# jinPrelude/simple-es

Measured on AMD Instinct MI355X. Metric: env-steps/sec (whole node), CartPole openai_es pop=4096 at 1/2/4/8 GPUs, higher is better.
Workload: dtype f32

## Files before the change

include/ses.h:

```cpp
#ifndef SES_H_
#define SES_H_

#include <stdint.h>

#ifdef __cplusplus
extern "C" {
#endif

#define SES_OK 0
#define SES_ERR_INVALID_ARG (-1)
#define SES_ERR_UNSUPPORTED (-2)
#define SES_ERR_HIP (-3)
#define SES_ERR_NO_DEVICE (-4)
#define SES_ERR_COMM (-5)

#define SES_HIDDEN 32

#define SES_ENV_NONE (-1)
#define SES_ENV_CARTPOLE 0
#define SES_ENV_LUNARLANDER 1
#define SES_ENV_SIMPLE_SPREAD 2
#define SES_ENV_BIPEDALWALKER 3
#define SES_ENV_ACROBOT 4
#define SES_ENV_MOUNTAINCAR 5
#define SES_ENV_PENDULUM 6
#define SES_ENV_MOUNTAINCAR_CONT 7

#define SES_MODE_EPISODIC 0
#define SES_MODE_FIXED_LENGTH 1

typedef struct ses_handle ses_handle;

typedef struct ses_config {
    int32_t env_id;
    int32_t num_state;
    int32_t num_action;
    int32_t discrete_action;
    int32_t gru;
    int32_t pomdp;
    int32_t max_step;
    int32_t eval_ep_num;
    int32_t device;
    int32_t lanes_per_env;
    int32_t n_agents;
    int32_t physics64;
} ses_config;

int ses_create(const ses_config *cfg, void *stream, ses_handle **out);
int ses_destroy(ses_handle *h);
int ses_sync(ses_handle *h);
int ses_set_tuning(ses_handle *h, const char *name, int32_t value);
int ses_launch_counts(ses_handle *h, int64_t *pair_rollouts, int64_t *perturb_rollouts, int64_t *apply_perturb);
int ses_set_stamp(ses_handle *h, uint64_t *dst);
const char *ses_last_error(void);
const char *ses_version(void);
int ses_param_count(int32_t num_state, int32_t num_action, int32_t gru);
int ses_device_count(void);

int ses_perturb(ses_handle *h, const float *parents, const int32_t *parent_idx, const int32_t *row_ids,
                float sigma, uint64_t seed, uint64_t gen, int64_t first_row, int32_t n_rows, float *theta);
int ses_noise(ses_handle *h, uint64_t seed, uint64_t gen, int64_t first_row, int32_t n_rows, float *eps);
int ses_perturb_host_noise(ses_handle *h, const float *parents, const int32_t *parent_idx,
                           const double *eps64, double sigma, int32_t n_rows, float *theta,
                           float *eps_store);
int ses_init_states_uniform(ses_handle *h, uint64_t seed, uint64_t gen, int64_t first_row, int32_t n_rows,
                            int32_t shared, int32_t width, float lo, float hi, float *out);
int ses_init_states_uniform_gens(ses_handle *h, uint64_t seed, uint64_t gen0, int32_t gens, int64_t first_row,
                                 int32_t n_rows, int32_t shared, int32_t width, float lo, float hi, float *out);

int ses_policy_forward(ses_handle *h, const float *theta, const float *obs, float *hidden, int32_t n,
                       float *logits, float *act, int32_t *action);

int ses_env_step(ses_handle *h, int32_t n, int32_t mode, float *x, float *xd, float *th, float *thd,
                 const int32_t *action, float *ret, uint32_t *status);

int ses_env_state_bytes(ses_handle *h);
int ses_env_obs_width(ses_handle *h);
int ses_env_reset(ses_handle *h, const float *init, int32_t n, void *state, float *obs);
int ses_env_step_generic(ses_handle *h, void *state, const void *action, int32_t n, float *obs, float *reward,
                         int32_t *done);

int ses_env_step_shape(ses_handle *h, int32_t *block, int32_t *lds_bytes, int32_t *waves_per_cu, int32_t *lds_per_cu);

int ses_stream_probe(ses_handle *h, int32_t n, float *x, float *xd, float *th, float *thd, const int32_t *action,
                     float *ret, uint32_t *status);

int ses_rollout(ses_handle *h, const float *theta, const float *init, int32_t init_per_offspring,
                int32_t n_rows, int32_t mode, float *fitness, double *ep_return, int32_t *ep_steps);

int ses_rank_center(ses_handle *h, const float *fitness, int32_t n, int32_t *rank, double *weights, float *best);

int ses_openai_generation(ses_handle *h, const float *fitness, int32_t n, uint64_t seed, uint64_t gen, double lr,
                          double sigma, double adam_a, const float *mu_in, const float *m_in, const float *v_in,
                          float *mu_out, float *m_out, float *v_out, float next_sigma, uint64_t next_gen,
                          int64_t first_row, int32_t n_rows, float *theta_next, float *best);
int ses_openai_sharded_ok(ses_handle *h, ses_handle *comm, int32_t n, int32_t per_rank, int32_t world);
int ses_openai_generation_sharded(ses_handle *h, ses_handle *comm, const float *fitness, int32_t n, uint64_t seed, uint64_t gen,
                                  double lr, double sigma, double adam_a, const float *mu_in, const float *m_in,
                                  const float *v_in, float *mu_out, float *m_out, float *v_out, float next_sigma,
                                  uint64_t next_gen, int64_t first_row, int32_t n_rows, int32_t per_rank, int32_t world,
                                  float *theta_next, float *best);
int ses_es_update_philox(ses_handle *h, const double *weights, int32_t n, int32_t skip_row0, uint64_t seed,
                         uint64_t gen, double lr, double sigma, double adam_a, float *mu, float *m, float *v,
                         float *grad_out);
int ses_es_update_stored(ses_handle *h, const double *weights, int32_t n, const float *eps_store, double lr,
                         double sigma, double adam_a, float *mu, float *m, float *v, float *grad_out);

int ses_perturb_mirrored(ses_handle *h, const float *mu, const float *scale, float sigma, uint64_t seed, uint64_t gen,
                         int64_t first_row, int32_t n_rows, float *theta);
int ses_pgpe_generation(ses_handle *h, const float *fitness, int32_t n, uint64_t seed, uint64_t gen, double sigma, double adam_a,
                        double sigma_learning_rate, double sigma_max_change, float scale_lo, float scale_hi, const float *mu_in,
                        const float *m_in, const float *v_in, const float *scale_in, float *mu_out, float *m_out, float *v_out,
                        float *scale_out, float next_sigma, uint64_t next_gen, int64_t first_row, int32_t n_rows,
                        float *theta_next, float *best, float *gmu_out, float *gs_out);

typedef struct ses_sepcma_params {
    int32_t mu, reserved;
    double mueff, c_sigma, d_sigma, c_c, c_1, c_mu, chi;
    float scale_lo, scale_hi, step_lo, step_hi;
} ses_sepcma_params;
int ses_perturb_sepcma(ses_handle *h, const float *mu, const float *C, const float *step, float sigma, uint64_t seed, uint64_t gen,
                       int64_t first_row, int32_t n_rows, float *theta);
int ses_sepcma_generation(ses_handle *h, const float *fitness, int32_t n, uint64_t seed, uint64_t gen, double sigma, double hsig_scale,
                          const ses_sepcma_params *p, const float *weights, const float *mu_in, const float *C_in,
                          const float *ps_in, const float *pc_in, const float *step_in, float *mu_out, float *C_out, float *ps_out,
                          float *pc_out, float *step_out, float next_sigma, uint64_t next_gen, int64_t first_row, int32_t n_rows,
                          float *theta_next, float *best, float *sz_out, float *szz_out, double *norm2_out);

#define SES_LMMA_MAX_MEMORY 32
#define SES_LMMA_MAX_P 16384
typedef struct ses_lmma_params {
    int32_t mu, m;
    double mueff, c_sigma, d_sigma, chi;
    float step_lo, step_hi;
    float cd[SES_LMMA_MAX_MEMORY], ad[SES_LMMA_MAX_MEMORY], ac[SES_LMMA_MAX_MEMORY], bc[SES_LMMA_MAX_MEMORY];
} ses_lmma_params;
int ses_perturb_lmma(ses_handle *h, const float *mu, const float *M, const float *step, const ses_lmma_params *p, int32_t m_active,
                     float sigma, uint64_t seed, uint64_t gen, int64_t first_row, int32_t n_rows, float *theta, float *dots_out);
int ses_lmma_generation(ses_handle *h, const float *fitness, int32_t n, uint64_t seed, uint64_t gen, double sigma,
                        const ses_lmma_params *p, const float *weights, int32_t m_active, int32_t m_active_next, const float *mu_in,
                        const float *ps_in, const float *M_in, const float *step_in, float *mu_out, float *ps_out, float *M_out,
                        float *step_out, float next_sigma, uint64_t next_gen, int64_t first_row, int32_t n_rows, float *theta_next,
                        float *best, float *sz_out, float *sd_out, float *sdots_out, double *norm2_out, float *dots_next_out);

int ses_elite_ids(ses_handle *h, const int32_t *rank, int32_t n, int32_t k, int32_t *elite_ids);
int ses_elite_select(ses_handle *h, const int32_t *rank, int32_t n, int32_t k, const int32_t *parent_map,
                     int32_t *alias_state, int32_t *elite_ids, int32_t *elite_parent_idx, int32_t *alias_first);
int ses_elite_mean(ses_handle *h, const float *rows, const int32_t *alias_first, int32_t k, float *mean);
int ses_gather_rows(ses_handle *h, const float *src, const int32_t *ids, int32_t n_ids, float *dst);

#define SES_STRATEGY_OPENAI_ES 0
#define SES_STRATEGY_SIMPLE_EVOLUTION 1
#define SES_STRATEGY_SIMPLE_GENETIC 2
#define SES_STRATEGY_PGPE 3
#define SES_STRATEGY_SEP_CMA_ES 4
#define SES_STRATEGY_LM_MA_ES 5
typedef struct ses_gen_state {
    int32_t strategy, n, elite_num, mode, shared_init, init_width;
    float init_lo, init_hi;
    uint64_t seed, env_seed;
    double learning_rate, sigma_decay;
    double sigma, pop_sigma;
    uint64_t pop_gen;
    int64_t adam_t;
    int32_t cur, world;
    float *theta[2];
    float *parents[2];
    float *adam_m[2];
    float *adam_v[2];
    int32_t *parent_map;
    int32_t *alias_state;
    float *fitness;
    float *init;
    int32_t *work_i32;
    float *work_f32;
    int64_t first_row;
    int32_t n_local, per_rank;
    ses_handle *comm;
    float *fit_local;
    float *scale[2];
    double sigma_learning_rate, sigma_max_change;
    float scale_lo, scale_hi;
    float *cma_C[2];
    float *cma_ps[2];
    float *cma_pc[2];
    float *cma_step[2];
    const float *cma_weights;
    ses_sepcma_params cma;
    float *lm_ps[2];
    float *lm_M[2];
    float *lm_step[2];
    const float *lm_weights;
    ses_lmma_params lm;
} ses_gen_state;
int ses_run_generations(ses_handle *h, ses_gen_state *st, int32_t k, float *best, uint64_t *stamps);

#define SES_COMM_ID_BYTES 128
int ses_comm_unique_id(void *id);
int ses_comm_init(ses_handle *h, int32_t rank, int32_t world, const void *id);
int ses_comm_info(ses_handle *h, int32_t *rank, int32_t *world, int32_t *rccl_version);
int ses_comm_destroy(ses_handle *h);
int ses_allgather_fitness(ses_handle *h, const float *local, int32_t n_per_rank, float *all);
#define SES_COMM_P2P_HANDLE_BYTES 64
int ses_comm_p2p_export(ses_handle *h, int32_t rank, int32_t world, int32_t max_per_rank, void *handle);
int ses_comm_p2p_attach(ses_handle *h, const void *handles);
int ses_comm_p2p_attach_local(ses_handle *h, ses_handle *const *peers);
int ses_stream_create_exclusive(int32_t device, void **stream);
int ses_stream_destroy(void *stream);
int ses_comm_p2p_info(ses_handle *h, int32_t *world, int32_t *max_per_rank, int32_t *exchanges);
int ses_comm_p2p_counts(ses_handle *h, int32_t *flag_exchanges, int32_t *granule_exchanges);
int ses_comm_p2p_status(ses_handle *h, uint32_t *timed_out_mask);
int ses_comm_p2p_reset_status(ses_handle *h);
int ses_comm_p2p_detach(ses_handle *h);

#ifdef __cplusplus
}
#endif
#endif
```

simple-es_amd/csrc/ses_core.hip:

```cpp
#include <cstring>
#include <string>

#include "ses_internal.h"

namespace ses {

static thread_local char g_err[512] = "";

int set_error(int code, const char *fmt, ...)
{
    va_list ap;
    va_start(ap, fmt);
    vsnprintf(g_err, sizeof g_err, fmt, ap);
    va_end(ap);
    return code;
}

int ensure_episode_scratch(ses_handle *h, size_t episodes)
{
    if (episodes <= h->ep_cap) return SES_OK;
    if (h->ep_return || h->ep_steps) SES_HIP_TRY(hipStreamSynchronize(h->stream));
    if (h->ep_return) SES_HIP_TRY(hipFree(h->ep_return));
    if (h->ep_steps) SES_HIP_TRY(hipFree(h->ep_steps));
    h->ep_return = nullptr;
    h->ep_steps = nullptr;
    h->ep_cap = 0;
    SES_HIP_TRY(hipMalloc(&h->ep_return, episodes * sizeof(double)));
    SES_HIP_TRY(hipMalloc(&h->ep_steps, episodes * sizeof(int32_t)));
    h->ep_cap = episodes;
    return SES_OK;
}

int ensure_reduce_scratch(ses_handle *h, size_t bytes)
{
    if (bytes <= h->red_cap) return SES_OK;
    size_t want = bytes < (1u << 20) ? (1u << 20) : bytes * 2;
    if (h->red_scratch) {
        SES_HIP_TRY(hipStreamSynchronize(h->stream));
        SES_HIP_TRY(hipFree(h->red_scratch));
    }
    h->red_scratch = nullptr;
    h->red_cap = 0;
    h->rank_zeroed = nullptr;
    h->counter_armed = nullptr;
    SES_HIP_TRY(hipMalloc(&h->red_scratch, want));
    h->red_cap = want;
    return SES_OK;
}

}

extern "C" {

const char *ses_last_error(void) { return ses::g_err; }

const char *ses_version(void) { return "ses-hip 0.1 (gfx950)"; }

int ses_param_count(int32_t S, int32_t A, int32_t gru)
{
    int p = SES_HIDDEN * S + SES_HIDDEN + A * SES_HIDDEN + A;
    if (gru) p += 2 * (3 * SES_HIDDEN * SES_HIDDEN) + 2 * (3 * SES_HIDDEN);
    return p;
}

int ses_device_count(void)
{
    int n = 0;
    hipError_t e = hipGetDeviceCount(&n);
    if (e != hipSuccess) return ses::set_error(SES_ERR_NO_DEVICE, "hipGetDeviceCount: %s", hipGetErrorString(e));
    return n;
}

int ses_create(const ses_config *cfg, void *stream, ses_handle **out)
{
    SES_REQUIRE(cfg && out, "ses_create: null argument");
    SES_REQUIRE(cfg->env_id == SES_ENV_CARTPOLE || cfg->env_id == SES_ENV_NONE || cfg->env_id == SES_ENV_SIMPLE_SPREAD ||
                    cfg->env_id == SES_ENV_LUNARLANDER || cfg->env_id == SES_ENV_BIPEDALWALKER || ses::is_classic_env(cfg->env_id),
                "ses_create: unknown env_id %d", cfg->env_id);
    SES_REQUIRE(cfg->num_state >= 1 && cfg->num_state <= 32, "ses_create: num_state %d out of range", cfg->num_state);
    SES_REQUIRE(cfg->num_action >= 1 && cfg->num_action <= 8, "ses_create: num_action %d out of range", cfg->num_action);
    SES_REQUIRE(cfg->eval_ep_num >= 1, "ses_create: eval_ep_num must be >= 1");
    SES_REQUIRE(cfg->max_step >= 1 && cfg->max_step < (1 << 30), "ses_create: max_step must be in [1, 2^30)");
    SES_REQUIRE(cfg->lanes_per_env == 0 || cfg->lanes_per_env == 1 || cfg->lanes_per_env == 2 ||
                    cfg->lanes_per_env == 4 || cfg->lanes_per_env == 8 || cfg->lanes_per_env == 16 || cfg->lanes_per_env == 32,
                "ses_create: lanes_per_env must be 0, 1, 2, 4, 8, 16 or 32");
    if (cfg->env_id == SES_ENV_CARTPOLE)
        SES_REQUIRE(cfg->num_state == 4 && cfg->num_action == 2 && cfg->discrete_action,
                    "ses_create: CartPole needs num_state=4 num_action=2 discrete_action=1");
    if (cfg->env_id == SES_ENV_LUNARLANDER)
        SES_REQUIRE(cfg->num_state == 8 && cfg->num_action == 4,
                    "ses_create: LunarLander needs num_state=8 num_action=4 (discrete_action=0: LunarLanderContinuous-v2, 1: LunarLander-v2)");
    if (cfg->env_id == SES_ENV_BIPEDALWALKER)
        SES_REQUIRE(cfg->num_state == 24 && cfg->num_action == 4 && !cfg->discrete_action && !cfg->gru && !cfg->pomdp,
                    "ses_create: BipedalWalker needs num_state=24 num_action=4 discrete_action=0 gru=0 pomdp=0");
    if (cfg->env_id == SES_ENV_SIMPLE_SPREAD)
        SES_REQUIRE((cfg->n_agents == 2 || cfg->n_agents == 3) && cfg->num_state == 6 * cfg->n_agents &&
                        cfg->num_action == 5 && cfg->discrete_action && (cfg->gru == 0 || cfg->gru == 1),
                    "ses_create: simple_spread needs n_agents in {2,3}, num_state=6*n_agents, num_action=5, "
                    "discrete_action=1, gru in {0,1}");
    static const struct {
        int env_id;
        const char *name;
        int S, A, discrete;
    } classic[] = {{SES_ENV_ACROBOT, "Acrobot-v1", 6, 3, 1}, {SES_ENV_MOUNTAINCAR, "MountainCar-v0", 2, 3, 1},
                   {SES_ENV_PENDULUM, "Pendulum-v1", 3, 1, 0}, {SES_ENV_MOUNTAINCAR_CONT, "MountainCarContinuous-v0", 2, 1, 0}};
    for (const auto &e : classic)
        if (cfg->env_id == e.env_id)
            SES_REQUIRE(cfg->num_state == e.S && cfg->num_action == e.A && (cfg->discrete_action != 0) == e.discrete &&
                            (cfg->gru == 0 || cfg->gru == 1) && !cfg->pomdp && !cfg->physics64,
                        "ses_create: %s needs num_state=%d num_action=%d discrete_action=%d gru in {0,1} pomdp=0 physics64=0 "
                        "(its physics is float64 regardless)",
                        e.name, e.S, e.A, e.discrete);
    SES_REQUIRE(cfg->physics64 == 0 || (cfg->physics64 == 1 && cfg->env_id == SES_ENV_CARTPOLE),
                "ses_create: physics64 is a CartPole rollout option");
    int ndev = ses_device_count();
    if (ndev <= 0) return ses::set_error(SES_ERR_NO_DEVICE, "ses_create: no HIP device visible");
    SES_REQUIRE(cfg->device >= 0 && cfg->device < ndev, "ses_create: device %d not in [0,%d)", cfg->device, ndev);
    SES_HIP_TRY(hipSetDevice(cfg->device));
    ses_handle *h = new ses_handle();
    std::memset(h, 0, sizeof *h);
    h->cfg = *cfg;
    h->stream = (hipStream_t)stream;
    h->P = ses_param_count(cfg->num_state, cfg->num_action, cfg->gru);
    h->obs_mask = 0u;
    if (cfg->pomdp && cfg->env_id == SES_ENV_CARTPOLE) h->obs_mask = 0xAu;
    if (cfg->pomdp && cfg->env_id == SES_ENV_LUNARLANDER) h->obs_mask = 0x2Cu;
    h->tune_rollout_block = 64;
    h->tune_gru_mfma_min_e = 12;
    h->tune_gru_mfma4_min_e = 7;
    h->tune_gru_ep_parallel_max = 4096;
    h->tune_gru_sequential = 0;
    h->tune_rollout_mix = 1;
    h->tune_rollout_waves8 = 1024;
    h->tune_rollout_packed = -1;
    h->tune_rollout_heavy_packed = -1;
    h->tune_rollout_mix_8_16 = 1;
    h->tune_rollout_handover_step = 1 << 30;
    h->tune_rollout_heavy_prio_steps = 1 << 30;
    h->tune_lander_per_wave = 0;
    h->tune_box2d_lpe = 0;
    h->tune_box2d_epw = 0;
    h->tune_env_step_block = 64;
    h->tune_env_step_lds = -1;
    h->tune_env_step_waves = 7;
    h->env_step_key[0] = -2;
    {
        int lds = 0;
        const hipError_t e = hipDeviceGetAttribute(&lds, hipDeviceAttributeMaxSharedMemoryPerMultiprocessor, cfg->device);
        if (e != hipSuccess) {
            delete h;
            return ses::set_error(SES_ERR_HIP, "ses_create: hipDeviceGetAttribute: %s", hipGetErrorString(e));
        }
        h->lds_per_cu = lds;
    }
    h->tune_openai_sharded_tail = 1;
    h->tune_openai_sharded_min_rows = 8192;
    h->tune_openai_granules = 1;
    h->tune_comm_granules_enabled = 1;
    h->tune_fused_fitness = 1;
    h->tune_fused_mean = 1;
    h->tune_fused_elite = 1;
    h->tune_fused_apply_perturb = 1;
    h->tune_fused_perturb_rollout = 1;
    h->tune_pgpe_fused_apply_perturb = 1;
    h->tune_spread_gru_wave_per_batch = -1;
    h->tune_comm_granules = 0;
    h->tune_es_final_max_chunks = 0;
    h->tune_es_tail_wide = 1;
    *out = h;
    return SES_OK;
}

int ses_set_tuning(ses_handle *h, const char *name, int32_t value)
{
    SES_REQUIRE(h && name, "ses_set_tuning: null argument");
    struct Knob {
        const char *name;
        int ses_handle::*field;
        int lo, hi;
    };
    static const Knob knobs[] = {{"rollout_block", &ses_handle::tune_rollout_block, 64, 256},
                                 {"gru_mfma_min_e", &ses_handle::tune_gru_mfma_min_e, 1, 1 << 30},
                                 {"gru_mfma4_min_e", &ses_handle::tune_gru_mfma4_min_e, 0, 8},
                                 {"gru_ep_parallel_max", &ses_handle::tune_gru_ep_parallel_max, 0, 1 << 30},
                                 {"gru_sequential", &ses_handle::tune_gru_sequential, 0, 1},
                                 {"rollout_mix", &ses_handle::tune_rollout_mix, 0, 1},
                                 {"rollout_waves8", &ses_handle::tune_rollout_waves8, 1, 1 << 20},
                                 {"rollout_mix_light", &ses_handle::tune_rollout_mix_light, 0, 16},
                                 {"rollout_lpe32_max_envs", &ses_handle::tune_rollout_lpe32_max, 0, 1 << 30},
                                 {"rollout_packed", &ses_handle::tune_rollout_packed, -1, 1},
                                 {"rollout_heavy_packed", &ses_handle::tune_rollout_heavy_packed, -1, 1},
                                 {"rollout_mix_8_16", &ses_handle::tune_rollout_mix_8_16, 0, 1},
                                 {"rollout_handover_step", &ses_handle::tune_rollout_handover_step, 0, 1 << 30},
                                 {"rollout_heavy_prio_steps", &ses_handle::tune_rollout_heavy_prio_steps, 0, 1 << 30},
                                 {"lander_offspring_per_wave", &ses_handle::tune_lander_per_wave, 0, 4},
                                 {"box2d_lanes_per_env", &ses_handle::tune_box2d_lpe, 0, 64},
                                 {"box2d_envs_per_wave", &ses_handle::tune_box2d_epw, 0, 64},
                                 {"pendulum_generic_step", &ses_handle::tune_pendulum_generic, 0, 1},
                                 {"env_step_block", &ses_handle::tune_env_step_block, 64, 256},
                                 {"env_step_lds_bytes", &ses_handle::tune_env_step_lds, -1, 65536},
                                 {"env_step_waves_per_cu", &ses_handle::tune_env_step_waves, 1, 32},
                                 {"es_final_max_chunks", &ses_handle::tune_es_final_max_chunks, 0, 1 << 20},
                                 {"es_tail_wide", &ses_handle::tune_es_tail_wide, 0, 1},
                                 {"comm_force_rccl", &ses_handle::tune_comm_force_rccl, 0, 1},
                                 {"comm_p2p_timeout_ms", &ses_handle::tune_comm_p2p_timeout_ms, 0, 1 << 30},
                                 {"comm_p2p_keep_going", &ses_handle::tune_comm_p2p_keep_going, 0, 1},
                                 {"openai_sharded_tail", &ses_handle::tune_openai_sharded_tail, 0, 1},
                                 {"openai_sharded_min_rows", &ses_handle::tune_openai_sharded_min_rows, 0, 1 << 30},
                                 {"openai_granule_exchange", &ses_handle::tune_openai_granules, 0, 1},
                                 {"comm_granule_allgather", &ses_handle::tune_comm_granules, 0, 1},
                                 {"comm_granules_enabled", &ses_handle::tune_comm_granules_enabled, 0, 1},
                                 {"fused_fitness_exchange", &ses_handle::tune_fused_fitness, 0, 1},
                                 {"fused_episode_mean", &ses_handle::tune_fused_mean, 0, 1},
                                 {"fused_elite_tail", &ses_handle::tune_fused_elite, 0, 1},
                                 {"fused_apply_perturb", &ses_handle::tune_fused_apply_perturb, 0, 1},
                                 {"fused_perturb_rollout", &ses_handle::tune_fused_perturb_rollout, 0, 1},
                                 {"pgpe_fused_apply_perturb", &ses_handle::tune_pgpe_fused_apply_perturb, 0, 1},
                                 {"spread_gru_wave_per_batch", &ses_handle::tune_spread_gru_wave_per_batch, -1, 1}};
    for (const Knob &k : knobs) {
        if (std::strcmp(k.name, name) == 0) {
            SES_REQUIRE(value >= k.lo && value <= k.hi, "ses_set_tuning: %s = %d outside [%d, %d]", name, value, k.lo, k.hi);
            SES_REQUIRE(k.field != &ses_handle::tune_rollout_block || value == 64 || value == 256,
                        "ses_set_tuning: rollout_block must be 64 or 256");
            SES_REQUIRE(k.field != &ses_handle::tune_env_step_block || value == 64 || value == 128 || value == 256,
                        "ses_set_tuning: env_step_block must be 64, 128 or 256");
            SES_REQUIRE(k.field != &ses_handle::tune_lander_per_wave || value != 3,
                        "ses_set_tuning: lander_offspring_per_wave must be 0, 1, 2 or 4");
            SES_REQUIRE(k.field != &ses_handle::tune_box2d_lpe || (value & (value - 1)) == 0,
                        "ses_set_tuning: box2d_lanes_per_env must be 0 or a power of two up to 64");
            SES_REQUIRE(k.field != &ses_handle::tune_rollout_mix_light || value == 0 || value == 8 || value == 16,
                        "ses_set_tuning: rollout_mix_light must be 0, 8 or 16");
            h->*(k.field) = value;
            if (k.field == &ses_handle::tune_comm_p2p_timeout_ms) ses::comm_p2p_set_timeout(h);
            return SES_OK;
        }
    }
    return ses::set_error(SES_ERR_INVALID_ARG, "ses_set_tuning: unknown knob '%s'", name);
}

int ses_launch_counts(ses_handle *h, int64_t *pair_rollouts, int64_t *perturb_rollouts, int64_t *apply_perturb)
{
    SES_REQUIRE(h, "ses_launch_counts: null handle");
    if (pair_rollouts) *pair_rollouts = h->count_pair_rollouts;
    if (perturb_rollouts) *perturb_rollouts = h->count_perturb_rollouts;
    if (apply_perturb) *apply_perturb = h->count_apply_perturb;
    return SES_OK;
}

int ses_set_stamp(ses_handle *h, uint64_t *dst)
{
    SES_REQUIRE(h, "ses_set_stamp: null handle");
    h->stamp = (unsigned long long *)dst;
    return SES_OK;
}

int ses_destroy(ses_handle *h)
{
    if (!h) return SES_OK;
    (void)hipSetDevice(h->cfg.device);
    (void)ses::comm_release(h);
    if (h->ep_return) (void)hipFree(h->ep_return);
    if (h->ep_steps) (void)hipFree(h->ep_steps);
    if (h->red_scratch) (void)hipFree(h->red_scratch);
    if (h->gen_init) (void)hipFree(h->gen_init);
    delete h;
    return SES_OK;
}

int ses_sync(ses_handle *h)
{
    SES_REQUIRE(h, "ses_sync: null handle");
    SES_HIP_TRY(hipStreamSynchronize(h->stream));
    return SES_OK;
}

}
```

simple-es_amd/csrc/ses_internal.h:

```cpp
#pragma once
#include <hip/hip_runtime.h>

#include <cstdarg>
#include <cstdio>
#include <type_traits>

#include "../../include/ses.h"

namespace ses {
struct P2pGranuleView;
struct PerturbUpdate {
    const float *partial;
    int chunks, P4;
    float update_factor;
    double adam_a;
    const float *mu_in, *m_in, *v_in;
    float *mu_out, *m_out, *v_out;
    float sigma;
    uint64_t seed, gen;
    long long first_row;
    int n_rows, P, quads;
    float *theta;
    unsigned long long *stamp;
    int32_t *rank_to_clear;
    int n_clear;
};
}
struct ses_handle {
    ses_config cfg;
    hipStream_t stream;
    int P;
    uint32_t obs_mask;
    double *ep_return;
    int32_t *ep_steps;
    size_t ep_cap;
    void *red_scratch;
    size_t red_cap;
    float *gen_init;
    size_t gen_init_cap;
    void *comm;
    int comm_rank, comm_world;
    struct ses_p2p *p2p;
    int tune_rollout_block;
    int tune_gru_mfma_min_e;
    int tune_gru_mfma4_min_e;
    int tune_gru_ep_parallel_max;
    int tune_gru_sequential;
    int tune_rollout_mix;
    int tune_rollout_waves8;
    int tune_rollout_mix_light;
    int tune_rollout_lpe32_max;
    int tune_rollout_mix_8_16;
    int tune_rollout_handover_step;
    int tune_rollout_heavy_prio_steps;
    int tune_rollout_packed;
    int tune_rollout_heavy_packed;
    unsigned long long *stamp;
    int32_t *rank_zeroed;
    int rank_zeroed_n;
    unsigned int *counter_armed;
    int tune_comm_force_rccl;
    int tune_es_final_max_chunks;
    int tune_es_tail_wide;
    int tune_box2d_lpe;
    int tune_env_step_block;
    int tune_env_step_lds;
    int tune_env_step_waves;
    const ses::P2pGranuleView *fit_gv;
    const float *fit_own;
    int fit_per_rank;
    int skip_mean;
    const double *mean_src;
    unsigned long long *mean_stamp;
    int tune_fused_elite;
    int tune_fused_apply_perturb;
    int tune_fused_mean;
    int lds_per_cu;
    int env_step_key[3];
    int env_step_lds_resolved;
    int env_step_wpc;
    int tune_box2d_epw;
    int tune_lander_per_wave;
    int tune_comm_p2p_timeout_ms;
    int tune_comm_p2p_keep_going;
    int tune_fused_fitness;
    int tune_comm_granules_enabled;
    int tune_comm_granules;
    int tune_openai_granules;
    int tune_openai_sharded_tail;
    int tune_openai_sharded_min_rows;
    int tune_fused_perturb_rollout;
    int defer_perturb, defer_mode;
    int perturb_pending;
    ses::PerturbUpdate pending;
    long long count_pair_rollouts;
    long long count_perturb_rollouts;
    long long count_apply_perturb;
    int tune_pendulum_generic;
    int tune_pgpe_fused_apply_perturb;
    int tune_spread_gru_wave_per_batch;
};

namespace ses {

__device__ __forceinline__ unsigned long long real_time() { return wall_clock64(); }

int set_error(int code, const char *fmt, ...);

#define SES_HIP_TRY(expr)                                                                          \
    do {                                                                                           \
        hipError_t e_ = (expr);                                                                    \
        if (e_ != hipSuccess)                                                                      \
            return ::ses::set_error(SES_ERR_HIP, "%s failed: %s (%s:%d)", #expr, hipGetErrorString(e_), \
                                    __FILE__, __LINE__);                                           \
    } while (0)

#define SES_REQUIRE(cond, ...)                                             \
    do {                                                                   \
        if (!(cond)) return ::ses::set_error(SES_ERR_INVALID_ARG, __VA_ARGS__); \
    } while (0)

inline int ceil_div(long long a, long long b) { return (int)((a + b - 1) / b); }

template <int L>
using lanes_c = std::integral_constant<int, L>;

template <class F>
inline void with_fixed_length(int mode, F &&f)
{
    if (mode == SES_MODE_FIXED_LENGTH) f(std::true_type{});
    else f(std::false_type{});
}

template <int... Ls, class F>
inline bool with_lanes(int lanes, F &&f)
{
    return (... || (lanes == Ls && (f(lanes_c<Ls>{}), true)));
}

template <int S_, int A_>
struct PolicyShape {
    static constexpr int S = S_, A = A_;
};
template <class... Shapes, class F>
inline bool with_policy_shape(int S, int A, F &&f)
{
    return (... || (S == Shapes::S && A == Shapes::A && (f(Shapes{}), true)));
}

struct RolloutArgs {
    const float *theta, *init;
    int per;
    int n_rows, E, P, max_step;
    uint32_t obs_mask;
    double *epr;
    int32_t *ep_steps;
    long long episodes() const { return (long long)n_rows * E; }
};

template <class K, class... X>
inline void launch_rollout_kernel(const ses_handle *h, K kernel, dim3 grid, dim3 block, const RolloutArgs &a, X... extra)
{
    hipLaunchKernelGGL(kernel, grid, block, 0, h->stream, a.theta, a.init, a.per, a.n_rows, a.E, a.P, a.max_step, a.obs_mask,
                       extra..., a.epr, a.ep_steps);
}

constexpr int P2P_GRANULE_MAX_WORLD = 16;
struct P2pGranuleView {
    unsigned long long *dst[P2P_GRANULE_MAX_WORLD];
    const unsigned long long *src;
    int section;
    int rank, world;
    uint32_t seq;
    unsigned long long timeout_ticks;
    uint32_t *err, *err_seen;
};
int comm_p2p_granules_begin(ses_handle *comm, int granules, P2pGranuleView *view);

#if defined(__HIPCC__)
__device__ __forceinline__ void granule_store(unsigned long long *dst, uint32_t seq, uint32_t value_bits)
{
    __hip_atomic_store(dst, ((unsigned long long)value_bits << 32) | (unsigned long long)seq, __ATOMIC_RELAXED, __HIP_MEMORY_SCOPE_SYSTEM);
}

__device__ __forceinline__ uint32_t granule_wait(const unsigned long long *src, const P2pGranuleView &v, int from)
{
    const unsigned long long t0 = real_time();
    unsigned long long limit = v.timeout_ticks;
    bool known_late = false;
    for (;;) {
        const unsigned long long g = __hip_atomic_load(src, __ATOMIC_RELAXED, __HIP_MEMORY_SCOPE_SYSTEM);
        const uint32_t tag = (uint32_t)g;
        if (tag == v.seq) return (uint32_t)(g >> 32);
        if (!known_late) {
            known_late = true;
            const uint32_t seen = __hip_atomic_load(v.err_seen, __ATOMIC_RELAXED, __HIP_MEMORY_SCOPE_AGENT);
            if (((seen >> (from & 31)) & 1u) && limit > 200000ull) limit = 200000ull;
        }
        if ((int32_t)(tag - v.seq) > 0 || real_time() - t0 > limit) {
            atomicOr_system(v.err, 1u << (from & 31));
            atomicOr(v.err_seen, 1u << (from & 31));
            return 0x7FC00000u;
        }
        __builtin_amdgcn_s_sleep(2);
    }
}

#endif

int openai_fused_fitness_ok(const ses_handle *h, int32_t n, int32_t per_rank, int32_t n_ranked);
int elite_tail_small(ses_handle *h, const double *ep_return, int32_t n, int32_t k, const int32_t *parent_map, int32_t *alias_state,
                     int32_t *rank, float *fitness, float *best, int32_t *ids, int32_t *pidx, int32_t *alias,
                     unsigned long long *stamp, const float *parents, float sigma, uint64_t seed, uint64_t gen, float *mean_out);

inline bool is_classic_env(int env_id)
{
    return env_id == SES_ENV_ACROBOT || env_id == SES_ENV_MOUNTAINCAR || env_id == SES_ENV_PENDULUM || env_id == SES_ENV_MOUNTAINCAR_CONT;
}
int classic_env_state_bytes(const ses_handle *h);
int classic_env_obs_width(const ses_handle *h);
int classic_env_reset(ses_handle *h, const float *init, int n, void *state, float *obs);
int classic_env_step(ses_handle *h, void *state, const void *action, int n, float *obs, float *reward, int32_t *done);
int classic_lanes_per_env(const ses_handle *h, long long episodes);
int classic_rollout(const ses_handle *h, const RolloutArgs &a, int mode);
inline bool is_classic_policy_shape(int S, int A) { return (A == 3 && (S == 6 || S == 2)) || (A == 1 && (S == 3 || S == 2)); }
int classic_policy_forward(ses_handle *h, const float *theta, const float *obs, float *hidden, int n, float *logits, float *act,
                           int32_t *action);

int spread_gru_rollout(const ses_handle *h, const RolloutArgs &a);
inline bool is_spread_policy_shape(int S, int A) { return A == 5 && (S == 12 || S == 18); }
int spread_gru_policy_forward(ses_handle *h, const float *theta, const float *obs, float *hidden, int n, float *logits, float *act,
                              int32_t *action);

enum class GruForm { Sequential, EpisodeParallel, Mfma4, Mfma, LockstepMulti4, LockstepMulti2, Lockstep };

int lander_discrete_rollout(const ses_handle *h, const RolloutArgs &a, GruForm form, int lpe, int epw);
int lander_discrete_env_step(ses_handle *h, void *state, const int32_t *action, int n, float *obs, float *reward, int32_t *done);

bool cartpole_perturb_rollout_ok(const ses_handle *h, int n_rows, int mode);
int flush_pending_perturb(ses_handle *h);

int ensure_episode_scratch(ses_handle *h, size_t episodes);
int ensure_reduce_scratch(ses_handle *h, size_t bytes);
int comm_release(ses_handle *h);
void comm_p2p_set_timeout(ses_handle *h);


}
```

simple-es_amd/csrc/ses_perturb_prologue.h:

```cpp
#pragma once
#include "ses_internal.h"
#include "ses_rng.h"

namespace ses {

__device__ __forceinline__ void adam_apply(float g, double adam_a, float &mu, float &m, float &v)
{
    const float b1 = 0.99f, b2 = 0.999f;
    const float omb1 = (float)(1.0 - 0.99), omb2 = (float)(1.0 - 0.999);
    const float mn = (b1 * m) + (omb1 * g);
    const float vn = (b2 * v) + (omb2 * (g * g));
    const double num = (-adam_a) * (double)mn;
    const float den = __builtin_sqrtf(vn) + 1e-08f;
    const double step = num / (double)den;
    m = mn;
    v = vn;
    mu = (float)((double)mu + step);
}

constexpr int UPDATE_PRELOAD = 4;
struct UpdateOperands {
    float part[UPDATE_PRELOAD];
    float mu, m, v;
};
__device__ __forceinline__ UpdateOperands es_update_load(const PerturbUpdate &u, int p)
{
    UpdateOperands o;
#pragma unroll
    for (int c = 0; c < UPDATE_PRELOAD; ++c) o.part[c] = c < u.chunks ? u.partial[(size_t)c * u.P4 + p] : 0.0f;
    o.mu = u.mu_in[p]; o.m = u.m_in[p]; o.v = u.v_in[p];
    return o;
}
__device__ __forceinline__ void es_update_finish(const PerturbUpdate &u, int p, UpdateOperands &o)
{
    float sum = o.part[0];
#pragma unroll
    for (int c = 1; c < UPDATE_PRELOAD; ++c)
        if (c < u.chunks) sum = sum + o.part[c];
    for (int c = UPDATE_PRELOAD; c < u.chunks; ++c) sum = sum + u.partial[(size_t)c * u.P4 + p];
    const float g = sum * u.update_factor;
    adam_apply(g, u.adam_a, o.mu, o.m, o.v);
}

__device__ __forceinline__ void perturb_update_mean(const PerturbUpdate &u, float *mu_new, UpdateOperands *first = nullptr)
{
    const int block = (int)blockDim.x;
    const long long t = (long long)blockIdx.x * block + threadIdx.x;
    if (u.stamp && t == 0) *u.stamp = real_time();
    for (int p = threadIdx.x; p < u.P; p += block) {
        UpdateOperands o = (first && p == (int)threadIdx.x) ? *first : es_update_load(u, p);
        es_update_finish(u, p, o);
        mu_new[p] = o.mu;
        if (blockIdx.x == 0) { u.mu_out[p] = o.mu; u.m_out[p] = o.m; u.v_out[p] = o.v; }
    }
    for (long long i = t; i < u.n_clear; i += (long long)gridDim.x * block) u.rank_to_clear[i] = 0;
}

__device__ __forceinline__ int perturb_row_quad(const PerturbUpdate &u, const float *mu_new, int i, int q, float (&out)[4])
{
    const int lim = u.P - 4 * q < 4 ? u.P - 4 * q : 4;
    const long long row = u.first_row + i;
    if (row == 0) {
        for (int l = 0; l < lim; ++l) out[l] = mu_new[4 * q + l];
        return lim;
    }
    float z[4];
    normal4(u.seed, u.gen, (uint32_t)row, (uint32_t)q, z);
    for (int l = 0; l < lim; ++l) out[l] = fma_(u.sigma, z[l], mu_new[4 * q + l]);
    return lim;
}

struct RowSpan {
    int row0, rows;
};
__device__ __forceinline__ RowSpan rows_of_envs(int env0, int env1, int E)
{
    if (env1 <= env0) return RowSpan{0, 0};
    const int r0 = env0 / E;
    return RowSpan{r0, (env1 - 1) / E - r0 + 1};
}
inline int max_rows_of_envs(int n, int E) { return n <= 1 ? n : (n - 2) / E + 2; }

constexpr int PERTURB_BATCH = 3;
struct PerturbItems {
    float z[PERTURB_BATCH][4];
    int i[PERTURB_BATCH], q[PERTURB_BATCH], s[PERTURB_BATCH];
};
template <int K>
__device__ __forceinline__ void perturb_draw(const PerturbUpdate &u, RowSpan a, RowSpan b, int base, int items, PerturbItems &it)
{
#pragma unroll
    for (int k = 0; k < K; ++k) {
        int w = base + k * (int)blockDim.x + (int)threadIdx.x;
        w = w < items ? w : items - 1;
        const int s = w / u.quads;
        it.s[k] = s;
        it.q[k] = w - s * u.quads;
        it.i[k] = s < a.rows ? a.row0 + s : b.row0 + (s - a.rows);
        normal4(u.seed, u.gen, (uint32_t)(u.first_row + it.i[k]), (uint32_t)it.q[k], it.z[k]);
    }
}
__device__ __forceinline__ int perturb_batch_count(int base, int items)
{
    const int left = items - (base + ((int)threadIdx.x & ~63));
    const int n = left <= 0 ? 0 : (left + (int)blockDim.x - 1) / (int)blockDim.x;
    return __builtin_amdgcn_readfirstlane(n < PERTURB_BATCH ? n : PERTURB_BATCH);
}
__device__ __forceinline__ void perturb_draw_n(const PerturbUpdate &u, RowSpan a, RowSpan b, int base, int items, int n, PerturbItems &it)
{
    if (n >= 3) perturb_draw<3>(u, a, b, base, items, it);
    else if (n == 2) perturb_draw<2>(u, a, b, base, items, it);
    else if (n == 1) perturb_draw<1>(u, a, b, base, items, it);
}
__device__ __forceinline__ void perturb_store(const PerturbUpdate &u, const float *mu_new, float *lds_rows, int base, int items, int n,
                                              const PerturbItems &it)
{
#pragma unroll
    for (int k = 0; k < PERTURB_BATCH; ++k) {
        if (k >= n || base + k * (int)blockDim.x + (int)threadIdx.x >= items) continue;
        const int q = it.q[k];
        const int lim = u.P - 4 * q < 4 ? u.P - 4 * q : 4;
        const bool mean_row = u.first_row + it.i[k] == 0;
        float *dst = u.theta + (size_t)it.i[k] * u.P + 4 * q, *row = lds_rows + (size_t)it.s[k] * u.P + 4 * q;
        for (int l = 0; l < lim; ++l) {
            const float m = mu_new[4 * q + l];
            const float v = mean_row ? m : fma_(u.sigma, it.z[k][l], m);
            dst[l] = v;
            row[l] = v;
        }
    }
}

__device__ __forceinline__ void perturb_prologue(const PerturbUpdate &u, RowSpan a, RowSpan b, float *mu_new, float *lds_rows,
                                                 TanhEntry *tanh_lds)
{
    const int tid = (int)threadIdx.x, block = (int)blockDim.x;
    const int items = (a.rows + b.rows) * u.quads;
    UpdateOperands first{};
    if (tid < u.P) first = es_update_load(u, tid);
    const float4 *tanh_src = reinterpret_cast<const float4 *>(&SES_TANH_TABLE[0][0]);
    float4 tv{};
    if (tanh_lds && tid < SES_TANH_N) tv = tanh_src[tid];
    PerturbItems it;
    int n = perturb_batch_count(0, items);
    perturb_draw_n(u, a, b, 0, items, n, it);
    if (tanh_lds) {
        if (tid < SES_TANH_N) tanh_lds[tid] = TanhEntry{tv.x, tv.y, tv.z, tv.w};
        for (int i = tid + block; i < SES_TANH_N; i += block) {
            const float4 v = tanh_src[i];
            tanh_lds[i] = TanhEntry{v.x, v.y, v.z, v.w};
        }
    }
    perturb_update_mean(u, mu_new, &first);
    __syncthreads();
    perturb_store(u, mu_new, lds_rows, 0, items, n, it);
    for (int base = PERTURB_BATCH * block; base < items; base += PERTURB_BATCH * block) {
        n = perturb_batch_count(base, items);
        perturb_draw_n(u, a, b, base, items, n, it);
        perturb_store(u, mu_new, lds_rows, base, items, n, it);
    }
    __syncthreads();
}

}
```

simple-es_amd/csrc/ses_policy.h:

```cpp
#pragma once
#include <hip/hip_runtime.h>

#include "ses_math.h"

namespace ses {

constexpr int H = 32;

template <int CTRL>
__device__ __forceinline__ float dpp_mov(float v)
{
    return __builtin_bit_cast(float, __builtin_amdgcn_update_dpp(0, __builtin_bit_cast(int, v), CTRL, 0xF, 0xF, true));
}
constexpr int DPP_QUAD_XOR1 = 0xB1;
constexpr int DPP_QUAD_XOR2 = 0x4E;
constexpr int DPP_ROW_HALF_MIRROR = 0x141;
constexpr int DPP_ROW_ROR8 = 0x128;
constexpr int DPP_ROW_ROR12 = 0x12C;
constexpr int DPP_QUAD_00_22 = 0xA0;
constexpr int DPP_ROW_BCAST1 = 0x151;
constexpr int DPP_ROW_NEWBCAST15 = 0x15F;
constexpr int DPP_ROW_ROR4 = 0x124;
constexpr int DPP_QUAD_BCAST0 = 0x00;
constexpr int DPP_QUAD_BCAST1 = 0x55;
constexpr int DPP_QUAD_BCAST2 = 0xAA;
constexpr int DPP_QUAD_BCAST3 = 0xFF;

template <int LPE>
__device__ __forceinline__ float lanes_sum(float v)
{
    if constexpr (LPE >= 2) v = v + dpp_mov<DPP_QUAD_XOR1>(v);
    if constexpr (LPE >= 4) v = v + dpp_mov<DPP_QUAD_XOR2>(v);
    if constexpr (LPE >= 8) v = v + dpp_mov<DPP_ROW_HALF_MIRROR>(v);
    return v;
}

template <int S, int A, int LPE>
struct MlpSlice {
    static constexpr int U = H / LPE;
    static constexpr int G = U / 4;
    static_assert(U % 4 == 0 || U == 2 || U == 1, "a lane owns whole fc2 groups, or a lane pair / quad owns one");
    static constexpr int W2N = U <= 2 ? 4 : U;
    float w1[U][S];
    float b1[U];
    float w2[A][W2N];
    float b2[A];

    __device__ __forceinline__ void load(const float *__restrict__ theta, int sub)
    {
        const int j0 = sub * U;
        const float *pw1 = theta;
        const float *pb1 = theta + H * S;
        const float *pw2 = pb1 + H;
        const float *pb2 = pw2 + A * H;
#pragma unroll
        for (int u = 0; u < U; ++u) {
#pragma unroll
            for (int k = 0; k < S; ++k) w1[u][k] = SES_TANH_H_INV * pw1[(j0 + u) * S + k];
            b1[u] = SES_TANH_H_INV * pb1[j0 + u];
        }
#pragma unroll
        for (int a = 0; a < A; ++a) {
            if constexpr (U == 1) {
#pragma unroll
                for (int u = 0; u < 4; ++u) w2[a][u] = pw2[a * H + (j0 & ~3) + u];
            } else if constexpr (U == 2) {
#pragma unroll
                for (int u = 0; u < 2; ++u) {
                    w2[a][u] = pw2[a * H + j0 + u];
                    w2[a][2 + u] = pw2[a * H + (j0 & ~3) + u];
                }
            } else {
#pragma unroll
                for (int u = 0; u < U; ++u) w2[a][u] = pw2[a * H + j0 + u];
            }
            b2[a] = pb2[a];
        }
    }

    struct Pending {
        float pre[U], frac[U];
        TanhEntry ent[U];
    };

    __device__ __forceinline__ void begin(const TanhEntry *tab, const float (&obs)[S], Pending &pd) const
    {
        int32_t idx[U];
#pragma unroll
        for (int u = 0; u < U; ++u) {
            float acc = b1[u];
#pragma unroll
            for (int k = 0; k < S; ++k) acc = fma_(w1[u][k], obs[k], acc);
            pd.pre[u] = acc;
            idx[u] = tanh_index_scaled(acc, pd.frac[u]);
        }
        __builtin_amdgcn_sched_barrier(0);
#pragma unroll
        for (int u = 0; u < U; ++u) pd.ent[u] = tab[idx[u]];
    }

    __device__ __forceinline__ void finish(const Pending &pd, float (&logits)[A]) const
    {
        float a[U];
#pragma unroll
        for (int u = 0; u < U; ++u) a[u] = tanh_eval(pd.ent[u], pd.frac[u], pd.pre[u]);
        if constexpr (U == 1) {
#pragma unroll
            for (int o = 0; o < A; ++o) {
                float q = dpp_mov<DPP_QUAD_BCAST0>(a[0]) * w2[o][0];
                q = fma_(dpp_mov<DPP_QUAD_BCAST1>(a[0]), w2[o][1], q);
                q = fma_(dpp_mov<DPP_QUAD_BCAST2>(a[0]), w2[o][2], q);
                q = fma_(dpp_mov<DPP_QUAD_BCAST3>(a[0]), w2[o][3], q);
                q = q + dpp_mov<DPP_ROW_ROR4>(q);
                q = q + dpp_mov<DPP_ROW_ROR8>(q);
                float lo = q, hi = q;
                asm volatile("s_nop 1\n\tv_permlane16_swap_b32 %0, %1\n\ts_nop 1" : "+v"(lo), "+v"(hi));
                q = lo + hi;
                logits[o] = dpp_mov<DPP_ROW_NEWBCAST15>(q + b2[o]);
            }
            return;
        }
        if constexpr (U == 2) {
#pragma unroll
            for (int o = 0; o < A; ++o) {
                float q = dpp_mov<DPP_QUAD_00_22>(a[0]) * w2[o][2];
                q = fma_(dpp_mov<DPP_QUAD_00_22>(a[1]), w2[o][3], q);
                q = fma_(w2[o][0], a[0], q);
                q = fma_(w2[o][1], a[1], q);
                q = q + dpp_mov<DPP_QUAD_XOR2>(q);
                q = q + dpp_mov<DPP_ROW_ROR12>(q);
                q = q + dpp_mov<DPP_ROW_ROR8>(q);
                logits[o] = dpp_mov<DPP_ROW_BCAST1>(q + b2[o]);
            }
            return;
        }
#pragma unroll
        for (int o = 0; o < A; ++o) {
            float p[G > 0 ? G : 1];
#pragma unroll
            for (int g = 0; g < G; ++g) {
                float acc = w2[o][4 * g] * a[4 * g];
                acc = fma_(w2[o][4 * g + 1], a[4 * g + 1], acc);
                acc = fma_(w2[o][4 * g + 2], a[4 * g + 2], acc);
                acc = fma_(w2[o][4 * g + 3], a[4 * g + 3], acc);
                p[g] = acc;
            }
            float s;
            if constexpr (G == 8) {
                s = ((p[0] + p[1]) + (p[2] + p[3])) + ((p[4] + p[5]) + (p[6] + p[7]));
            } else if constexpr (G == 4) {
                s = (p[0] + p[1]) + (p[2] + p[3]);
            } else if constexpr (G == 2) {
                s = p[0] + p[1];
            } else {
                s = p[0];
            }
            logits[o] = lanes_sum<LPE>(s) + b2[o];
        }
    }

    __device__ __forceinline__ void forward(const TanhEntry *tab, const float (&obs)[S], float (&logits)[A]) const
    {
        Pending pd;
        begin(tab, obs, pd);
        finish(pd, logits);
    }
};

template <int S, int A, int LPE>
__device__ __forceinline__ void mlp_forward_streamed(const float *__restrict__ theta, int sub, const TanhEntry *tab,
                                                     const float (&obs)[S], float (&logits)[A])
{
    constexpr int U = H / LPE, G = U / 4;
    static_assert(U % 4 == 0, "a lane owns whole fc2 groups");
    const int j0 = sub * U;
    const float *pw1 = theta;
    const float *pb1 = theta + H * S;
    const float *pw2 = pb1 + H;
    const float *pb2 = pw2 + A * H;
    float p[A][G];
#pragma unroll
    for (int g = 0; g < G; ++g) {
        float a[4];
#pragma unroll
        for (int u = 0; u < 4; ++u) {
            const int j = j0 + 4 * g + u;
            float acc = SES_TANH_H_INV * pb1[j];
#pragma unroll
            for (int k = 0; k < S; ++k) acc = fma_(SES_TANH_H_INV * pw1[j * S + k], obs[k], acc);
            float frac;
            const int32_t idx = tanh_index_scaled(acc, frac);
            a[u] = tanh_eval(tab[idx], frac, acc);
        }
#pragma unroll
        for (int o = 0; o < A; ++o) {
            const float *w = pw2 + o * H + j0 + 4 * g;
            float acc = w[0] * a[0];
            acc = fma_(w[1], a[1], acc);
            acc = fma_(w[2], a[2], acc);
            acc = fma_(w[3], a[3], acc);
            p[o][g] = acc;
        }
        __builtin_amdgcn_sched_barrier(0);
    }
#pragma unroll
    for (int o = 0; o < A; ++o) {
        float s;
        if constexpr (G == 8) {
            s = ((p[o][0] + p[o][1]) + (p[o][2] + p[o][3])) + ((p[o][4] + p[o][5]) + (p[o][6] + p[o][7]));
        } else if constexpr (G == 4) {
            s = (p[o][0] + p[o][1]) + (p[o][2] + p[o][3]);
        } else if constexpr (G == 2) {
            s = p[o][0] + p[o][1];
        } else {
            s = p[o][0];
        }
        logits[o] = lanes_sum<LPE>(s) + pb2[o];
    }
}

__device__ __forceinline__ void stage_tanh_table(TanhEntry *lds)
{
    const float4 *src = reinterpret_cast<const float4 *>(&SES_TANH_TABLE[0][0]);
    for (int i = threadIdx.x; i < SES_TANH_N; i += blockDim.x) {
        const float4 v = src[i];
        lds[i] = TanhEntry{v.x, v.y, v.z, v.w};
    }
    __syncthreads();
}

__device__ __forceinline__ int add_mask_bit(int v, unsigned long long mask)
{
    asm("v_addc_co_u32_e64 %0, vcc, %0, 0, %1" : "+v"(v) : "s"(mask) : "vcc");
    return v;
}

template <int A>
__device__ __forceinline__ int argmax_first(const float (&logits)[A])
{
    int best = 0;
    float bv = logits[0];
#pragma unroll
    for (int k = 1; k < A; ++k) {
        const bool gt = logits[k] > bv;
        best = gt ? k : best;
        bv = gt ? logits[k] : bv;
    }
    return best;
}

}
```

simple-es_amd/csrc/ses_policy_pk.h:

```cpp
#pragma once
#include "ses_cartpole.h"
#include "ses_policy.h"

namespace ses {

typedef float pk2 __attribute__((ext_vector_type(2)));

__device__ __forceinline__ pk2 pk_fma(pk2 a, pk2 b, pk2 c) { return __builtin_elementwise_fma(a, b, c); }
__device__ __forceinline__ pk2 pk_splat(float v) { return pk2{v, v}; }

template <int LPE>
struct MlpSlicePk {
    static constexpr int S = 4, A = 2;
    static constexpr int U = H / LPE;
    static constexpr int UP = U / 2;
    static constexpr int G = U / 4;
    static_assert(U == 2 || U == 4 || U == 8, "4, 8 or 16 lanes per env");
    pk2 w1[UP][S];
    pk2 b1[UP];
    pk2 w2[U];
    pk2 w2e[2];
    pk2 b2;

    __device__ __forceinline__ void load(const float *__restrict__ theta, int sub)
    {
        const int j0 = sub * U;
        const float *pw1 = theta, *pb1 = theta + H * S, *pw2 = pb1 + H, *pb2 = pw2 + A * H;
#pragma unroll
        for (int p = 0; p < UP; ++p) {
#pragma unroll
            for (int k = 0; k < S; ++k)
                w1[p][k] = pk2{SES_TANH_H_INV * pw1[(j0 + 2 * p) * S + k], SES_TANH_H_INV * pw1[(j0 + 2 * p + 1) * S + k]};
            b1[p] = pk2{SES_TANH_H_INV * pb1[j0 + 2 * p], SES_TANH_H_INV * pb1[j0 + 2 * p + 1]};
        }
#pragma unroll
        for (int u = 0; u < U; ++u) w2[u] = pk2{pw2[j0 + u], pw2[H + j0 + u]};
#pragma unroll
        for (int u = 0; u < 2; ++u) w2e[u] = pk2{pw2[(j0 & ~3) + u], pw2[H + (j0 & ~3) + u]};
        b2 = pk2{pb2[0], pb2[1]};
    }

    struct Pending {
        float pre[U], frac[U];
        TanhEntry ent[U];
    };

    __device__ __forceinline__ void begin(const TanhEntry *tab, const float (&obs)[S], Pending &pd) const
    {
        int32_t idx[U];
        pk2 acc[UP];
#pragma unroll
        for (int p = 0; p < UP; ++p) acc[p] = b1[p];
#pragma unroll
        for (int k = 0; k < S; ++k) {
#pragma unroll
            for (int p = 0; p < UP; ++p) acc[p] = pk_fma(w1[p][k], pk_splat(obs[k]), acc[p]);
        }
#pragma unroll
        for (int p = 0; p < UP; ++p) {
            pd.pre[2 * p] = acc[p].x;
            pd.pre[2 * p + 1] = acc[p].y;
            idx[2 * p] = tanh_index_scaled(acc[p].x, pd.frac[2 * p]);
            idx[2 * p + 1] = tanh_index_scaled(acc[p].y, pd.frac[2 * p + 1]);
        }
        __builtin_amdgcn_sched_barrier(0);
#pragma unroll
        for (int u = 0; u < U; ++u) pd.ent[u] = tab[idx[u]];
    }

    __device__ __forceinline__ pk2 finish(const Pending &pd) const
    {
        float a[U];
        if constexpr (U == 8) {
            constexpr int order[8] = {2, 0, 1, 5, 3, 4, 7, 6};
#pragma unroll
            for (int i = 0; i < 8; ++i) a[order[i]] = tanh_eval(pd.ent[order[i]], pd.frac[order[i]], pd.pre[order[i]]);
        } else {
#pragma unroll
            for (int u = 0; u < U; ++u) a[u] = tanh_eval(pd.ent[u], pd.frac[u], pd.pre[u]);
        }
        pk2 q;
        if constexpr (U == 2) {
            const float e0 = dpp_mov<DPP_QUAD_00_22>(a[0]), e1 = dpp_mov<DPP_QUAD_00_22>(a[1]);
            q = w2e[0] * pk_splat(e0);
            q = pk_fma(w2e[1], pk_splat(e1), q);
            q = pk_fma(w2[0], pk_splat(a[0]), q);
            q = pk_fma(w2[1], pk_splat(a[1]), q);
            float q0 = q.x, q1 = q.y;
            q0 = q0 + dpp_mov<DPP_QUAD_XOR2>(q0);
            q1 = q1 + dpp_mov<DPP_QUAD_XOR2>(q1);
            q0 = q0 + dpp_mov<DPP_ROW_ROR12>(q0);
            q1 = q1 + dpp_mov<DPP_ROW_ROR12>(q1);
            q0 = q0 + dpp_mov<DPP_ROW_ROR8>(q0);
            q1 = q1 + dpp_mov<DPP_ROW_ROR8>(q1);
            const pk2 lg = pk2{q0, q1} + b2;
            return pk2{dpp_mov<DPP_ROW_BCAST1>(lg.x), dpp_mov<DPP_ROW_BCAST1>(lg.y)};
        } else {
            pk2 p[G];
#pragma unroll
            for (int g = 0; g < G; ++g) {
                p[g] = w2[4 * g] * pk_splat(a[4 * g]);
                p[g] = pk_fma(w2[4 * g + 1], pk_splat(a[4 * g + 1]), p[g]);
                p[g] = pk_fma(w2[4 * g + 2], pk_splat(a[4 * g + 2]), p[g]);
                p[g] = pk_fma(w2[4 * g + 3], pk_splat(a[4 * g + 3]), p[g]);
            }
            if constexpr (G == 2) q = p[0] + p[1];
            else q = p[0];
            const float q0 = lanes_sum<LPE>(q.x), q1 = lanes_sum<LPE>(q.y);
            return pk2{q0, q1} + b2;
        }
    }
};

struct CartPoleSimPk {
    pk2 P, V;
    __device__ __forceinline__ void init(const float *s0)
    {
        P = pk2{s0[0], s0[2]};
        V = pk2{s0[1], s0[3]};
    }
};

template <int LPE, bool FIXED_LENGTH, bool MASKED>
__device__ __forceinline__ void rollout_cartpole_mlp_loop_pk(const TanhEntry *tanh_tab, const MlpSlicePk<LPE> &net,
                                                             CartPoleSimPk &sim, int max_step, uint32_t obs_mask, int &steps,
                                                             unsigned long long &alive_mask)
{
    pk2 P = sim.P;
    pk2 V = sim.V;
    const float th_clamp = register_constant(CP_TH_CLAMP), lim_clamp = register_constant(CP_CLAMP);
    const pk2 tau2 = pk_splat(register_constant(CP_TAU));
    const pk2 k0 = {register_constant(2.443315711809948e-5f), register_constant(-1.9515295891e-4f)};
    const pk2 k1 = {register_constant(-1.388731625493765e-3f), register_constant(8.3321608736e-3f)};
    const pk2 k2 = {register_constant(4.166664568298827e-2f), register_constant(-1.6666654611e-1f)};
    asm volatile("" ::"v"(net.b2));
    bool alive = true;
    for (int t = 0; t < max_step; ++t) {
        if constexpr (!FIXED_LENGTH) {
            if (__ballot(alive) == 0ull) break;
        }
        float obs[4] = {P.x, V.x, P.y, V.y};
        if constexpr (MASKED) {
#pragma unroll
            for (int k = 0; k < 4; ++k) obs[k] = ((obs_mask >> k) & 1u) ? 0.0f : obs[k];
        }
        typename MlpSlicePk<LPE>::Pending pending;
        net.begin(tanh_tab, obs, pending);
        const float th = P.y, thd = V.y;
        const float z = th * th;
        const pk2 zz = pk_splat(z);
        pk2 pz = pk_fma(k0, zz, k1);
        pz = pk_fma(pz, zz, k2);
        pz = pz * zz;
        CartPolePre pre;
        pre.sn = fma_(pz.y, th, th);
        pre.cs = fma_(pz.x, z, fma_(-0.5f, z, 1.0f));
        pre.q = CP_PML_OVER_MASS * (thd * thd);
        pre.gsn = CP_GRAVITY * pre.sn;
        pre.den = fma_(CP_DEN_C1, pre.cs * pre.cs, CP_DEN_C0);
        {
            const float r0 = __builtin_amdgcn_rcpf(pre.den);
            pre.rden = fma_(fma_(-pre.den, r0, 1.0f), r0, r0);
        }
        const pk2 lg = net.finish(pending);
        const bool one = lg.y > lg.x;
        const float fom = one ? CP_FORCE_OVER_MASS : -CP_FORCE_OVER_MASS;
        const float temp = fma_(pre.q, pre.sn, fom);
        const float num = fma_(-pre.cs, temp, pre.gsn);
        const float thacc = cartpole_quotient(num, pre);
        const float xacc = fma_(-CP_PML_OVER_MASS * thacc, pre.cs, temp);
        const pk2 Pn = pk_fma(tau2, V, P);
        const pk2 Vn = pk_fma(tau2, pk2{xacc, thacc}, V);
        const float nx = clamp_sym_reg(Pn.x, lim_clamp);
        const float nth = __builtin_amdgcn_fmed3f(Pn.y, -th_clamp, th_clamp);
        const float nxd = clamp_sym_reg(Vn.x, lim_clamp);
        const float nthd = clamp_sym_reg(Vn.y, lim_clamp);
        if constexpr (FIXED_LENGTH) {
            P = pk2{nx, nth};
            V = pk2{nxd, nthd};
            steps = add_mask_bit(steps, alive_mask);
            alive_mask &= ~(__builtin_amdgcn_ballot_w64(__builtin_fabsf(nx) > CP_X_LIMIT) |
                            __builtin_amdgcn_ballot_w64(__builtin_fabsf(nth) > CP_THETA_LIMIT));
        } else {
            const bool term = (nx < -CP_X_LIMIT) || (nx > CP_X_LIMIT) || (nth < -CP_THETA_LIMIT) || (nth > CP_THETA_LIMIT);
            P = pk2{alive ? nx : P.x, alive ? nth : P.y};
            V = pk2{alive ? nxd : V.x, alive ? nthd : V.y};
            steps += (int)alive;
            alive = alive & !term;
        }
    }
    sim.P = P;
    sim.V = V;
}

}
```

simple-es_amd/csrc/ses_rollout.hip:

```cpp
#include "ses_cartpole.h"
#include "ses_gru.h"
#include "ses_gru_lockstep.h"
#include "ses_gru_mfma.h"
#include "ses_gru_mfma4.h"
#include "ses_lander.h"
#include "ses_walker.h"
#include "ses_internal.h"
#include "ses_policy.h"
#include "ses_policy_pk.h"
#include "ses_policy_forward.h"
#include "ses_rollout_bodies.h"
#include "ses_perturb_prologue.h"
#include "ses_spread.h"

namespace ses {

template <bool PHYS64>
struct CartPoleSim;

template <>
struct CartPoleSim<false> {
    CartPoleState st;
    CartPolePre pre;
    float th_clamp, lim_clamp;
    __device__ __forceinline__ void init(const float *s0)
    {
        st = CartPoleState{s0[0], s0[1], s0[2], s0[3]};
        th_clamp = register_constant(CP_TH_CLAMP);
        lim_clamp = register_constant(CP_CLAMP);
    }
    __device__ __forceinline__ void observe(float (&o)[4]) const { o[0] = st.x; o[1] = st.xd; o[2] = st.th; o[3] = st.thd; }
    __device__ __forceinline__ bool small_angle() const { return __builtin_fabsf(st.th) <= SINCOS_SMALL_MAX; }
    template <bool SMALL>
    __device__ __forceinline__ void prepare()
    {
        pre = SMALL ? cartpole_pre_small(st) : cartpole_pre(st);
    }
    __device__ __forceinline__ unsigned long long terminal_mask() const
    {
        return __builtin_amdgcn_ballot_w64(__builtin_fabsf(st.x) > CP_X_LIMIT) |
               __builtin_amdgcn_ballot_w64(__builtin_fabsf(st.th) > CP_THETA_LIMIT);
    }
    __device__ __forceinline__ bool advance(int action, bool keep_old)
    {
        CartPoleState ns = st;
        const bool term = cartpole_post(ns, pre, action, th_clamp, lim_clamp);
        st.x = keep_old ? st.x : ns.x;
        st.xd = keep_old ? st.xd : ns.xd;
        st.th = keep_old ? st.th : ns.th;
        st.thd = keep_old ? st.thd : ns.thd;
        return term;
    }
};

template <>
struct CartPoleSim<true> {
    CartPoleState64 st;
    __device__ __forceinline__ void init(const float *s0) { st = CartPoleState64{s0[0], s0[1], s0[2], s0[3]}; }
    __device__ __forceinline__ void observe(float (&o)[4]) const
    {
        o[0] = (float)st.x; o[1] = (float)st.xd; o[2] = (float)st.th; o[3] = (float)st.thd;
    }
    __device__ __forceinline__ bool small_angle() const { return false; }
    template <bool SMALL>
    __device__ __forceinline__ void prepare() {}
    __device__ __forceinline__ unsigned long long terminal_mask() const
    {
        const double thr = 12 * 2 * 3.141592653589793 / 360;
        return __builtin_amdgcn_ballot_w64(__builtin_fabs(st.x) > 2.4) |
               __builtin_amdgcn_ballot_w64(__builtin_fabs(st.th) > thr);
    }
    __device__ __forceinline__ bool advance(int action, bool keep_old)
    {
        CartPoleState64 ns = st;
        const bool term = cartpole_step64(ns, action);
        st.x = keep_old ? st.x : ns.x;
        st.xd = keep_old ? st.xd : ns.xd;
        st.th = keep_old ? st.th : ns.th;
        st.thd = keep_old ? st.thd : ns.thd;
        return term;
    }
};

template <int LPE, bool FIXED_LENGTH, bool PHYS64, bool MASKED, bool SMALL>
__device__ __forceinline__ void rollout_cartpole_mlp_loop(const TanhEntry *tanh_tab, const MlpSlice<4, 2, LPE> &net,
                                                          CartPoleSim<PHYS64> &sim, int max_step, uint32_t obs_mask,
                                                          int &steps, unsigned long long &alive_mask)
{
    bool alive = true;
    for (int t = 0; t < max_step; ++t) {
        if constexpr (!FIXED_LENGTH) {
            if (__ballot(alive) == 0ull) break;
        }
        float obs[4];
        sim.observe(obs);
        if constexpr (MASKED) {
#pragma unroll
            for (int k = 0; k < 4; ++k) obs[k] = ((obs_mask >> k) & 1u) ? 0.0f : obs[k];
        }
        float logits[2];
        typename MlpSlice<4, 2, LPE>::Pending pending;
        net.begin(tanh_tab, obs, pending);
        sim.template prepare<SMALL>();
        net.finish(pending, logits);
        const int action = argmax_first<2>(logits);
        const bool term = sim.advance(action, FIXED_LENGTH ? false : !alive);
        if constexpr (FIXED_LENGTH) {
            steps = add_mask_bit(steps, alive_mask);
            alive_mask &= ~sim.terminal_mask();
        } else {
            steps += (int)alive;
            alive = alive & !term;
        }
    }
}

template <int LPE, bool FIXED_LENGTH, bool PHYS64>
__device__ __forceinline__ void rollout_cartpole_mlp_run(const TanhEntry *tanh_tab, const MlpSlice<4, 2, LPE> &net,
                                                         CartPoleSim<PHYS64> &sim, int n_steps, uint32_t obs_mask, bool small,
                                                         int &steps, unsigned long long &alive_mask)
{
    if (obs_mask == 0u && small)
        rollout_cartpole_mlp_loop<LPE, FIXED_LENGTH, PHYS64, false, true>(tanh_tab, net, sim, n_steps, obs_mask, steps, alive_mask);
    else if (small)
        rollout_cartpole_mlp_loop<LPE, FIXED_LENGTH, PHYS64, true, true>(tanh_tab, net, sim, n_steps, obs_mask, steps, alive_mask);
    else
        rollout_cartpole_mlp_loop<LPE, FIXED_LENGTH, PHYS64, true, false>(tanh_tab, net, sim, n_steps, obs_mask, steps, alive_mask);
}

template <int LPE, bool FIXED_LENGTH, bool PHYS64 = false, bool PK = false>
__device__ __forceinline__ void rollout_cartpole_mlp_body(const TanhEntry *tanh_tab, long long lane_index, int env0,
                                                          const float *__restrict__ theta,
                                                          const float *__restrict__ init, int init_per_offspring,
                                                          int n_env, int E, int P, int max_step, uint32_t obs_mask,
                                                          double *__restrict__ ep_return,
                                                          int32_t *__restrict__ ep_steps, int row_base = 0)
{
    static_assert(!PK || (!PHYS64 && (LPE == 8 || LPE == 16)), "the packed step exists for 8 / 16 lanes per env, fp32 dynamics");
    int env = env0 + (int)(lane_index / LPE);
    const int sub = (int)(lane_index % LPE);
    const bool valid = env < n_env;
    env = valid ? env : n_env - 1;
    const int row = env / E;
    const int ep = env - row * E;
    const float *s0 = init + ((size_t)(init_per_offspring ? row : 0) * E + ep) * 4;
    int steps = 0;
    const bool small = !PHYS64 && __ballot(!(__builtin_fabsf(s0[2]) <= SINCOS_SMALL_MAX)) == 0ull;
    bool done = false;
    if constexpr (PK) {
        if (small) {
            MlpSlicePk<LPE> netp;
            netp.load(theta + (size_t)(row - row_base) * P, sub);
            CartPoleSimPk simp;
            simp.init(s0);
            unsigned long long alive_mask = ~0ull;
            if (obs_mask == 0u)
                rollout_cartpole_mlp_loop_pk<LPE, FIXED_LENGTH, false>(tanh_tab, netp, simp, max_step, obs_mask, steps, alive_mask);
            else
                rollout_cartpole_mlp_loop_pk<LPE, FIXED_LENGTH, true>(tanh_tab, netp, simp, max_step, obs_mask, steps, alive_mask);
            done = true;
        }
    }
    if (!done) {
        MlpSlice<4, 2, LPE> net;
        net.load(theta + (size_t)(row - row_base) * P, sub);
        CartPoleSim<PHYS64> sim;
        sim.init(s0);
        unsigned long long alive_mask = ~0ull;
        rollout_cartpole_mlp_run<LPE, FIXED_LENGTH, PHYS64>(tanh_tab, net, sim, max_step, obs_mask, small, steps, alive_mask);
    }
    if (valid && sub == 0) {
        if (ep_return) ep_return[env] = (double)steps;
        if (ep_steps) ep_steps[env] = steps;
    }
}

template <int LPE, bool FIXED_LENGTH, int BLOCK, bool PHYS64 = false, bool PK = false>
__global__ __launch_bounds__(BLOCK) void k_rollout_cartpole_mlp(const float *__restrict__ theta,
                                                             const float *__restrict__ init, int init_per_offspring,
                                                             int n_rows, int E, int P, int max_step,
                                                             uint32_t obs_mask, double *__restrict__ ep_return,
                                                             int32_t *__restrict__ ep_steps)
{
    __shared__ TanhEntry tanh_tab[SES_TANH_N];
    stage_tanh_table(tanh_tab);
    rollout_cartpole_mlp_body<LPE, FIXED_LENGTH, PHYS64, PK>(tanh_tab, (long long)blockIdx.x * BLOCK + threadIdx.x, 0, theta, init,
                                                 init_per_offspring, n_rows * E, E, P, max_step, obs_mask, ep_return,
                                                 ep_steps);
}

template <bool FIXED_LENGTH, int LIGHT, int REST = 4>
__global__ __launch_bounds__(64) void k_rollout_cartpole_mlp_mix(const float *__restrict__ theta,
                                                                 const float *__restrict__ init,
                                                                 int init_per_offspring, int n_rows, int E, int P,
                                                                 int max_step, uint32_t obs_mask, int waves_light,
                                                                 double *__restrict__ ep_return,
                                                                 int32_t *__restrict__ ep_steps)
{
    constexpr int EPW = 64 / LIGHT;
    __shared__ TanhEntry tanh_tab[SES_TANH_N];
    stage_tanh_table(tanh_tab);
    const int n_env = n_rows * E;
    if ((int)blockIdx.x < waves_light) {
        rollout_cartpole_mlp_body<LIGHT, FIXED_LENGTH>(tanh_tab, (long long)blockIdx.x * 64 + threadIdx.x, 0, theta, init,
                                                       init_per_offspring, n_env < waves_light * EPW ? n_env : waves_light * EPW,
                                                       E, P, max_step, obs_mask, ep_return, ep_steps);
    } else {
        rollout_cartpole_mlp_body<REST, FIXED_LENGTH>(tanh_tab, (long long)(blockIdx.x - waves_light) * 64 + threadIdx.x,
                                                      waves_light * EPW, theta, init, init_per_offspring, n_env, E, P, max_step,
                                                      obs_mask, ep_return, ep_steps);
    }
}

constexpr int HANDOVER_PAIRS = 4;
struct HandoverSlot {
    float x, xd, th, thd;
    int steps, alive;
};
template <bool FIXED_LENGTH, bool OWN_ROWS, bool HEAVY_PK>
__device__ __forceinline__ void rollout_cartpole_mlp_pairs(
    const TanhEntry *tanh_tab, HandoverSlot (*slots)[64 / 4], int *small_of, const float *__restrict__ theta,
    const float *__restrict__ init, int init_per_offspring, int n_rows, int E, int P, int max_step, uint32_t obs_mask,
    int waves_light, int waves_heavy, int handover, int prio_steps, double *__restrict__ ep_return,
    int32_t *__restrict__ ep_steps, const float *rows_l = nullptr, int row0_l = 0, const float *rows_h = nullptr, int row0_h = 0)
{
    static_assert(FIXED_LENGTH, "the hand-over needs every env to run max_step steps");
    constexpr int LIGHT = 16, HEAVY = 4, SPLIT = 8;
    constexpr int EPW_L = 64 / LIGHT, EPW_H = 64 / HEAVY, EPW_S = 64 / SPLIT;
    static_assert(EPW_H == 2 * EPW_S, "the heavy wave's envs are split evenly");
    using Slot = HandoverSlot;
    const int wave = (int)threadIdx.x / 64, lane = (int)threadIdx.x % 64;
    const int slot = wave % HANDOVER_PAIRS;
    const int pair = (int)blockIdx.x * HANDOVER_PAIRS + slot;
    const bool heavy = wave >= HANDOVER_PAIRS;
    const int n_env = n_rows * E;
    const int n_light = n_env < waves_light * EPW_L ? n_env : waves_light * EPW_L;
    const int env0_h = waves_light * EPW_L + pair * EPW_H;
    const bool has_heavy = pair < waves_heavy && env0_h < n_env;
    const bool split = handover < max_step;
    const int n_heavy = split ? handover : max_step;
    if (!heavy) {
        if (pair * EPW_L < n_light)
            rollout_cartpole_mlp_body<LIGHT, FIXED_LENGTH>(tanh_tab, (long long)pair * 64 + lane, 0, OWN_ROWS ? rows_l : theta, init,
                                                           init_per_offspring, n_light, E, P, max_step, obs_mask, ep_return,
                                                           ep_steps, OWN_ROWS ? row0_l : 0);
    } else if (has_heavy) {
        int env = env0_h + lane / HEAVY;
        const int sub = lane % HEAVY;
        const bool valid = env < n_env;
        env = valid ? env : n_env - 1;
        const int row = env / E;
        const int ep = env - row * E;
        const float *s0 = init + ((size_t)(init_per_offspring ? row : 0) * E + ep) * 4;
        const bool small = __ballot(!(__builtin_fabsf(s0[2]) <= SINCOS_SMALL_MAX)) == 0ull;
        const float *const row_theta = OWN_ROWS ? rows_h + (size_t)(row - row0_h) * P : theta + (size_t)row * P;
        CartPoleSim<false> sim;
        sim.init(s0);
        int steps = 0;
        unsigned long long alive_mask = ~0ull;
        const int n1 = prio_steps < n_heavy ? prio_steps : n_heavy;
        bool done = false;
        if constexpr (HEAVY_PK) if (small) {
            MlpSlicePk<HEAVY> netp;
            netp.load(row_theta, sub);
            CartPoleSimPk simp;
            simp.init(s0);
#pragma unroll 1
            for (int seg = 0; seg < 2; ++seg) {
                if (seg == 0) __builtin_amdgcn_s_setprio(1);
                else __builtin_amdgcn_s_setprio(0);
                const int n_seg = seg == 0 ? n1 : n_heavy - n1;
                if (obs_mask == 0u)
                    rollout_cartpole_mlp_loop_pk<HEAVY, FIXED_LENGTH, false>(tanh_tab, netp, simp, n_seg, obs_mask, steps, alive_mask);
                else
                    rollout_cartpole_mlp_loop_pk<HEAVY, FIXED_LENGTH, true>(tanh_tab, netp, simp, n_seg, obs_mask, steps, alive_mask);
            }
            sim.st = CartPoleState{simp.P.x, simp.V.x, simp.P.y, simp.V.y};
            done = true;
        }
        if (!done) {
            MlpSlice<4, 2, HEAVY> net;
            net.load(row_theta, sub);
#pragma unroll 1
            for (int seg = 0; seg < 2; ++seg) {
                if (seg == 0) __builtin_amdgcn_s_setprio(1);
                else __builtin_amdgcn_s_setprio(0);
                rollout_cartpole_mlp_run<HEAVY, FIXED_LENGTH, false>(tanh_tab, net, sim, seg == 0 ? n1 : n_heavy - n1, obs_mask,
                                                                     small, steps, alive_mask);
            }
        }
        if (!split) {
            if (valid && sub == 0) {
                if (ep_return) ep_return[env] = (double)steps;
                if (ep_steps) ep_steps[env] = steps;
            }
        } else if (sub == 0) {
            slots[slot][lane / HEAVY] = Slot{sim.st.x, sim.st.xd, sim.st.th, sim.st.thd, steps, (int)((alive_mask >> lane) & 1ull)};
            if (lane == 0) small_of[slot] = small ? 1 : 0;
        }
    }
    if (!split) return;
    __syncthreads();
    if (!has_heavy) return;
    const int k = (heavy ? 0 : EPW_S) + lane / SPLIT;
    const int sub = lane % SPLIT;
    int env = env0_h + k;
    const bool valid = env < n_env;
    env = valid ? env : n_env - 1;
    const int row = env / E;
    const Slot st = slots[slot][k];
    const bool small = small_of[slot] != 0;
    MlpSlice<4, 2, SPLIT> net;
    net.load(OWN_ROWS ? rows_h + (size_t)(row - row0_h) * P : theta + (size_t)row * P, sub);
    const float s1[4] = {st.x, st.xd, st.th, st.thd};
    CartPoleSim<false> sim;
    sim.init(s1);
    int steps = st.steps;
    unsigned long long alive_mask = __ballot(st.alive != 0);
    rollout_cartpole_mlp_run<SPLIT, FIXED_LENGTH, false>(tanh_tab, net, sim, max_step - handover, obs_mask, small, steps,
                                                         alive_mask);
    if (valid && sub == 0) {
        if (ep_return) ep_return[env] = (double)steps;
        if (ep_steps) ep_steps[env] = steps;
    }
}

template <bool FIXED_LENGTH, bool HEAVY_PK = false>
__global__ __launch_bounds__(64 * 2 * HANDOVER_PAIRS) void k_rollout_cartpole_mlp_handover(
    const float *__restrict__ theta, const float *__restrict__ init, int init_per_offspring, int n_rows, int E, int P,
    int max_step, uint32_t obs_mask, int waves_light, int waves_heavy, int handover, int prio_steps,
    double *__restrict__ ep_return, int32_t *__restrict__ ep_steps)
{
    __shared__ TanhEntry tanh_tab[SES_TANH_N];
    __shared__ HandoverSlot slots[HANDOVER_PAIRS][64 / 4];
    __shared__ int small_of[HANDOVER_PAIRS];
    stage_tanh_table(tanh_tab);
    rollout_cartpole_mlp_pairs<FIXED_LENGTH, false, HEAVY_PK>(tanh_tab, slots, small_of, theta, init, init_per_offspring, n_rows, E, P,
                                                              max_step, obs_mask, waves_light, waves_heavy, handover, prio_steps,
                                                              ep_return, ep_steps);
}

template <bool FIXED_LENGTH, bool HEAVY_PK = false>
__global__ __launch_bounds__(64 * 2 * HANDOVER_PAIRS) void k_rollout_cartpole_mlp_handover_perturb(
    const float *__restrict__ init, int init_per_offspring, int n_rows, int E, int P, int max_step, uint32_t obs_mask,
    int waves_light, int waves_heavy, int handover, int prio_steps, double *__restrict__ ep_return,
    int32_t *__restrict__ ep_steps, PerturbUpdate u)
{
    __shared__ TanhEntry tanh_tab[SES_TANH_N];
    __shared__ HandoverSlot slots[HANDOVER_PAIRS][64 / 4];
    __shared__ int small_of[HANDOVER_PAIRS];
    extern __shared__ float own_rows_lds[];
    constexpr int ENVS_L = HANDOVER_PAIRS * (64 / 16), ENVS_H = HANDOVER_PAIRS * (64 / 4);
    const int n_env = n_rows * E;
    const int n_light = n_env < waves_light * (64 / 16) ? n_env : waves_light * (64 / 16);
    const int l0 = (int)blockIdx.x * ENVS_L, h0 = waves_light * (64 / 16) + (int)blockIdx.x * ENVS_H;
    const RowSpan span_l = rows_of_envs(l0, l0 + ENVS_L < n_light ? l0 + ENVS_L : n_light, E);
    const RowSpan span_h = rows_of_envs(h0, h0 + ENVS_H < n_env ? h0 + ENVS_H : n_env, E);
    float *const mu_new = own_rows_lds, *const rows = own_rows_lds + u.P4;
    perturb_prologue(u, span_l, span_h, mu_new, rows, tanh_tab);
    rollout_cartpole_mlp_pairs<FIXED_LENGTH, true, HEAVY_PK>(tanh_tab, slots, small_of, nullptr, init, init_per_offspring, n_rows, E, P,
                                                             max_step, obs_mask, waves_light, waves_heavy, handover, prio_steps, ep_return,
                                                             ep_steps, rows, span_l.row0, rows + (size_t)span_l.rows * P, span_h.row0);
}
inline int pair_own_rows(int E) { return max_rows_of_envs(HANDOVER_PAIRS * (64 / 16), E) + max_rows_of_envs(HANDOVER_PAIRS * (64 / 4), E); }

template <bool FIXED_LENGTH>
__global__ __launch_bounds__(256) void k_rollout_cartpole_gru(const float *__restrict__ theta,
                                                              const float *__restrict__ init, int init_per_offspring,
                                                              int n_rows, int E, int P, int max_step,
                                                              uint32_t obs_mask, double *__restrict__ ep_return,
                                                              int32_t *__restrict__ ep_steps, int ep_parallel)
{
    __shared__ TanhEntry tanh_tab[SES_TANH_N];
    __shared__ __attribute__((aligned(16))) float vecs[4][64];
    stage_tanh_table(tanh_tab);
    const int wave = threadIdx.x >> 6, lane = threadIdx.x & 63;
    const int unit = blockIdx.x * 4 + wave, n_units = ep_parallel ? n_rows * E : n_rows;
    const bool valid = unit < n_units;
    const int u = valid ? unit : n_units - 1;
    const int row = ep_parallel ? u / E : u;
    const int ep_begin = ep_parallel ? u - row * E : 0, ep_end = ep_parallel ? ep_begin + 1 : E;
    GruSlice<4, 2> net;
    net.load(theta + (size_t)row * P, lane);
    float *vec = vecs[wave];
    for (int ep = ep_begin; ep < ep_end; ++ep) {
        const float *s0 = init + ((size_t)(init_per_offspring ? row : 0) * E + ep) * 4;
        CartPoleState st{s0[0], s0[1], s0[2], s0[3]};
        float h = 0.0f;
        wave_lds_sync();
        if (lane < 32) vec[2 * lane + 1] = 0.0f;
        wave_lds_sync();
        int steps = 0;
        bool alive = true;
        for (int t = 0; t < max_step; ++t) {
            if constexpr (!FIXED_LENGTH) {
                if (__builtin_amdgcn_readfirstlane((int)alive) == 0) break;
            }
            float obs[4];
            obs[0] = (obs_mask & 1u) ? 0.0f : st.x;
            obs[1] = (obs_mask & 2u) ? 0.0f : st.xd;
            obs[2] = (obs_mask & 4u) ? 0.0f : st.th;
            obs[3] = (obs_mask & 8u) ? 0.0f : st.thd;
            float logits[2];
            net.forward(tanh_tab, obs, h, vec, lane, logits);
            const int action = argmax_first<2>(logits);
            CartPoleState ns = st;
            const bool term = cartpole_step_general(ns, action);
            const bool advance = FIXED_LENGTH ? true : alive;
            st.x = advance ? ns.x : st.x;
            st.xd = advance ? ns.xd : st.xd;
            st.th = advance ? ns.th : st.th;
            st.thd = advance ? ns.thd : st.thd;
            const int nsteps = steps + 1;
            const bool finished = term | (nsteps >= max_step);
            steps = alive ? nsteps : steps;
            alive = alive & !finished;
        }
        if (valid && lane == 0) {
            if (ep_return) ep_return[(size_t)row * E + ep] = (double)steps;
            if (ep_steps) ep_steps[(size_t)row * E + ep] = steps;
        }
    }
}

struct CartPoleLs {
    static constexpr int S = 4, A = 2, INIT_W = 4;
    struct State {
        CartPoleState st;
    };
    __device__ static __forceinline__ void reset(State &s, const float *__restrict__ u, int)
    {
        s.st = CartPoleState{u[0], u[1], u[2], u[3]};
    }
    __device__ static __forceinline__ void observe(const State &s, float (&obs)[S])
    {
        obs[0] = s.st.x; obs[1] = s.st.xd; obs[2] = s.st.th; obs[3] = s.st.thd;
    }
    __device__ static __forceinline__ float step(State &s, const float (&logits)[A], const TanhEntry *, bool freeze,
                                                 bool &done)
    {
        const int action = argmax_first<A>(logits);
        CartPoleState ns = s.st;
        done = cartpole_step_general(ns, action);
        s.st.x = freeze ? s.st.x : ns.x;
        s.st.xd = freeze ? s.st.xd : ns.xd;
        s.st.th = freeze ? s.st.th : ns.th;
        s.st.thd = freeze ? s.st.thd : ns.thd;
        return 1.0f;
    }
};

struct CartPoleLs64 {
    static constexpr int S = 4, A = 2, INIT_W = 4;
    struct State {
        CartPoleState64 st;
    };
    __device__ static __forceinline__ void reset(State &s, const float *__restrict__ u, int)
    {
        s.st = CartPoleState64{u[0], u[1], u[2], u[3]};
    }
    __device__ static __forceinline__ void observe(const State &s, float (&obs)[S])
    {
        obs[0] = (float)s.st.x; obs[1] = (float)s.st.xd; obs[2] = (float)s.st.th; obs[3] = (float)s.st.thd;
    }
    __device__ static __forceinline__ float step(State &s, const float (&logits)[A], const TanhEntry *, bool freeze,
                                                 bool &done)
    {
        const int action = argmax_first<A>(logits);
        CartPoleState64 ns = s.st;
        done = cartpole_step64(ns, action);
        s.st.x = freeze ? s.st.x : ns.x;
        s.st.xd = freeze ? s.st.xd : ns.xd;
        s.st.th = freeze ? s.st.th : ns.th;
        s.st.thd = freeze ? s.st.thd : ns.thd;
        return 1.0f;
    }
};

struct LanderLs {
    static constexpr int S = 8, A = 4, INIT_W = 16;
    struct State {
        LanderState st;
    };
    __device__ static __forceinline__ void reset(State &s, const float *__restrict__ u, int slot)
    {
        __shared__ float terrain[4][32][LL_TERRAIN_ROW];
        ll_reset(s.st, u, terrain[threadIdx.x >> 6][slot]);
    }
    __device__ static __forceinline__ void observe(const State &s, float (&obs)[S]) { ll_obs(s.st, obs); }
    __device__ static __forceinline__ float step(State &s, const float (&logits)[A], const TanhEntry *tab, bool freeze,
                                                 bool &done)
    {
        const float a0 = tanh_(tab, logits[0]), a1 = tanh_(tab, logits[1]);
        float r = 0.0f;
        done = true;
        if (!freeze) r = ll_step(s.st, a0, a1, done);
        return r;
    }
};

template <typename EnvT, bool FIXED_LENGTH>
__device__ __forceinline__ void gru_mfma4_batch(const TanhEntry *tanh_tab, GruMfma4Lds<EnvT::S, EnvT::A> &lds,
                                                const GruMfma4<EnvT::S, EnvT::A> &net, int lane, int nb,
                                                const float *__restrict__ init_rows, int max_step, uint32_t obs_mask,
                                                double *__restrict__ ret_out, int32_t *__restrict__ steps_out, bool valid_row)
{
    constexpr int S = EnvT::S, A = EnvT::A;
    const int slot = lane & 7;
    const bool owner_valid = slot < nb;
    typename EnvT::State st;
    EnvT::reset(st, init_rows + (size_t)(owner_valid ? slot : 0) * EnvT::INIT_W, slot);
    float hreg[4] = {0.0f, 0.0f, 0.0f, 0.0f};
    wave_lds_sync();
    if (lane < 32) {
#pragma unroll
        for (int e = 0; e < G4_EB; ++e) lds.ah[e][lane][1] = 0.0f;
    }
    double ret = 0.0;
    int steps = 0;
    bool alive = true;
    for (int t = 0; t < max_step; ++t) {
        if constexpr (!FIXED_LENGTH) {
            if (__ballot(alive & owner_valid) == 0ull) break;
        }
        float obs[S];
        EnvT::observe(st, obs);
        if (lane < G4_EB) {
#pragma unroll
            for (int k = 0; k < S; ++k) lds.obs[lane][k] = ((obs_mask >> k) & 1u) ? 0.0f : obs[k];
        }
        wave_lds_sync();
        net.step(tanh_tab, lds, hreg, lane);
        float logits[A];
        GruMfma4<S, A>::logits_of(lds, lane, logits);
        bool term;
        const bool freeze = FIXED_LENGTH ? false : !alive;
        const float r = EnvT::step(st, logits, tanh_tab, freeze, term);
        const int nsteps = steps + 1;
        const bool finished = term | (nsteps >= max_step);
        ret = alive ? ret + (double)r : ret;
        steps = alive ? nsteps : steps;
        alive = alive & !finished;
    }
    if (valid_row && lane < G4_EB && owner_valid) {
        if (ret_out) ret_out[slot] = ret;
        if (steps_out) steps_out[slot] = steps;
    }
}

template <typename EnvT, bool FIXED_LENGTH>
__global__ __launch_bounds__(256, 2) void k_rollout_gru_mfma4(const float *__restrict__ theta, const float *__restrict__ init,
                                                              int init_per_offspring, int n_rows, int E, int P, int max_step,
                                                              uint32_t obs_mask, double *__restrict__ ep_return,
                                                              int32_t *__restrict__ ep_steps)
{
    __shared__ TanhEntry tanh_tab[SES_TANH_N];
    __shared__ __attribute__((aligned(16))) GruMfma4Lds<EnvT::S, EnvT::A> ldsv[4];
    stage_tanh_table(tanh_tab);
    const int wave = threadIdx.x >> 6, lane = threadIdx.x & 63;
    int row = blockIdx.x * 4 + wave;
    const bool valid = row < n_rows;
    row = valid ? row : n_rows - 1;
    GruMfma4Lds<EnvT::S, EnvT::A> &lds = ldsv[wave];
    GruMfma4<EnvT::S, EnvT::A> net;
    net.load(theta + (size_t)row * P, lane, lds);
    wave_lds_sync();
    for (int e0 = 0; e0 < E; e0 += G4_EB) {
        const int nb = E - e0 < G4_EB ? E - e0 : G4_EB;
        const float *rows = init + ((size_t)(init_per_offspring ? row : 0) * E + e0) * EnvT::INIT_W;
        double *ro = ep_return ? ep_return + (size_t)row * E + e0 : nullptr;
        int32_t *so = ep_steps ? ep_steps + (size_t)row * E + e0 : nullptr;
        gru_mfma4_batch<EnvT, FIXED_LENGTH>(tanh_tab, lds, net, lane, nb, rows, max_step, obs_mask, ro, so, valid);
    }
}

template <typename EnvT, int G>
__global__ __launch_bounds__(256, 2) void k_rollout_gru_lockstep_multi(const float *__restrict__ theta,
                                                                    const float *__restrict__ init, int init_per_offspring,
                                                                    int n_rows, int E, int P, int max_step,
                                                                    uint32_t obs_mask, double *__restrict__ ep_return,
                                                                    int32_t *__restrict__ ep_steps)
{
    __shared__ TanhEntry tanh_tab[SES_TANH_N];
    __shared__ __attribute__((aligned(16))) GruLockstepLds<EnvT::S, EnvT::A> ldsv[4][G];
    stage_tanh_table(tanh_tab);
    const int wave = threadIdx.x >> 6, lane = threadIdx.x & 63;
    const int row0 = (blockIdx.x * 4 + wave) * G;
    if (row0 >= n_rows) return;
#define SES_LSM_CASE(NP_, ODD_)                                                                                          \
    gru_lockstep_multi_batch<EnvT, G, NP_, ODD_>(tanh_tab, ldsv[wave], theta, P, row0, n_rows, lane, E, init,              \
                                                 init_per_offspring, E, max_step, obs_mask, ep_return, ep_steps)
    switch (E) {
        case 1: SES_LSM_CASE(1, true); break;
        case 2: SES_LSM_CASE(1, false); break;
        case 3: SES_LSM_CASE(2, true); break;
        case 4: SES_LSM_CASE(2, false); break;
        case 5: SES_LSM_CASE(3, true); break;
        case 6: SES_LSM_CASE(3, false); break;
        case 7: SES_LSM_CASE(4, true); break;
        default: SES_LSM_CASE(4, false); break;
    }
#undef SES_LSM_CASE
}

template <typename EnvT, bool FIXED_LENGTH>
__global__ __launch_bounds__(256, 2) void k_rollout_gru_mfma(const float *__restrict__ theta,
                                                          const float *__restrict__ init, int init_per_offspring,
                                                          int n_rows, int E, int P, int max_step, uint32_t obs_mask,
                                                          double *__restrict__ ep_return,
                                                          int32_t *__restrict__ ep_steps)
{
    __shared__ TanhEntry tanh_tab[SES_TANH_N];
    __shared__ __attribute__((aligned(16))) GruMfmaLds<EnvT::S, EnvT::A> ldsv[4];
    stage_tanh_table(tanh_tab);
    const int wave = threadIdx.x >> 6, lane = threadIdx.x & 63;
    int row = blockIdx.x * 4 + wave;
    const bool valid = row < n_rows;
    row = valid ? row : n_rows - 1;
    GruMfmaLds<EnvT::S, EnvT::A> &lds = ldsv[wave];
    GruMfma<EnvT::S, EnvT::A> net;
    net.load(theta + (size_t)row * P, lane, lds);
    wave_lds_sync();
    for (int e0 = 0; e0 < E; e0 += GM_EB) {
        const int nb = E - e0 < GM_EB ? E - e0 : GM_EB;
        const float *rows = init + ((size_t)(init_per_offspring ? row : 0) * E + e0) * EnvT::INIT_W;
        double *ro = ep_return ? ep_return + (size_t)row * E + e0 : nullptr;
        int32_t *so = ep_steps ? ep_steps + (size_t)row * E + e0 : nullptr;
        gru_mfma_batch<EnvT, FIXED_LENGTH>(tanh_tab, lds, net, lane, nb, rows, max_step, obs_mask, ro, so, valid);
    }
}

__global__ __launch_bounds__(256, 2) void k_rollout_lander_gru(const float *__restrict__ theta,
                                                        const float *__restrict__ init, int init_per_offspring,
                                                        int n_rows, int E, int P, int max_step, uint32_t obs_mask,
                                                        double *__restrict__ ep_return, int32_t *__restrict__ ep_steps,
                                                        int ep_parallel)
{
    constexpr int S = 8, A = 4;
    __shared__ TanhEntry tanh_tab[SES_TANH_N];
    __shared__ __attribute__((aligned(16))) float vecs[4][64];
    __shared__ float terrain[4][LL_TERRAIN_ROW];
    stage_tanh_table(tanh_tab);
    const int wave = threadIdx.x >> 6, lane = threadIdx.x & 63;
    {
        const int unit = blockIdx.x * 4 + wave, n_units = ep_parallel ? n_rows * E : n_rows;
        const bool valid = unit < n_units;
        const int u = valid ? unit : n_units - 1;
        const int row = ep_parallel ? u / E : u;
        const int ep_begin = ep_parallel ? u - row * E : 0, ep_end = ep_parallel ? ep_begin + 1 : E;
        GruSlice<S, A> net;
        net.load(theta + (size_t)row * P, lane);
        float *vec = vecs[wave];
        for (int ep = ep_begin; ep < ep_end; ++ep) {
            LanderState st;
            ll_reset(st, init + ((size_t)(init_per_offspring ? row : 0) * E + ep) * 16, terrain[wave]);
            float h = 0.0f;
            wave_lds_sync();
            if (lane < 32) vec[2 * lane + 1] = 0.0f;
            wave_lds_sync();
            double ret = 0.0;
            int steps = 0;
            bool done = false;
            while (steps < max_step) {
                if (__builtin_amdgcn_readfirstlane((int)done)) break;
                float obs[S], logits[A];
                ll_obs(st, obs);
#pragma unroll
                for (int k = 0; k < S; ++k) obs[k] = ((obs_mask >> k) & 1u) ? 0.0f : obs[k];
                net.forward(tanh_tab, obs, h, vec, lane, logits);
                const float a0 = tanh_(tanh_tab, logits[0]), a1 = tanh_(tanh_tab, logits[1]);
                ret += (double)ll_step(st, a0, a1, done);
                steps += 1;
            }
            if (valid && lane == 0) {
                ep_return[(size_t)row * E + ep] = ret;
                if (ep_steps) ep_steps[(size_t)row * E + ep] = steps;
            }
        }
    }
}

struct LanderMlpEnv {
    static constexpr int S = 8, A = 4, INIT_W = 16, ROW = LL_TERRAIN_ROW;
    static constexpr int WAVES_PER_SIMD = 2;
    using State = LanderState;
    __device__ static __forceinline__ void reset(State &s, const float *__restrict__ u, float *row) { ll_reset(s, u, row); }
    __device__ static __forceinline__ void observe(const State &s, float (&obs)[S]) { ll_obs(s, obs); }
    __device__ static __forceinline__ float step(State &s, const float (&act)[A], bool &done) { return ll_step(s, act[0], act[1], done); }
};

struct WalkerMlpEnv {
    static constexpr int S = 24, A = 4, INIT_W = 4, ROW = BW_TERRAIN_ROW;
    static constexpr int WAVES_PER_SIMD = 1;
    using State = WalkerState;
    __device__ static __forceinline__ void reset(State &s, const float *__restrict__ u, float *row) { bw_reset(s, u, row); }
    __device__ static __forceinline__ void observe(const State &s, float (&obs)[S]) { bw_obs(s, obs); }
    __device__ static __forceinline__ float step(State &s, const float (&act)[A], bool &done)
    {
        return bw_step(s, act[0], act[1], act[2], act[3], done);
    }
};

template <class EnvB, int LPE>
__global__ __launch_bounds__(64, EnvB::WAVES_PER_SIMD) void k_rollout_box2d_mlp(const float *__restrict__ theta,
                                                           const float *__restrict__ init, int init_per_offspring,
                                                           int n_rows, int E, int P, int max_step, uint32_t obs_mask,
                                                           int envs_per_wave, double *__restrict__ ep_return,
                                                           int32_t *__restrict__ ep_steps)
{
    constexpr int S = EnvB::S, A = EnvB::A;
    __shared__ TanhEntry tanh_tab[SES_TANH_N];
    __shared__ float terrain[64 / LPE][EnvB::ROW];
    stage_tanh_table(tanh_tab);
    const int n_env = n_rows * E;
    const int group = (int)threadIdx.x / LPE;
    const int slot = group < envs_per_wave ? group : envs_per_wave - 1;
    int env = (int)blockIdx.x * envs_per_wave + slot;
    const int sub = (int)(threadIdx.x % LPE);
    const bool valid = env < n_env && group < envs_per_wave;
    env = env < n_env ? env : n_env - 1;
    const int row = env / E, ep = env - row * E;
    typename EnvB::State st;
    EnvB::reset(st, init + ((size_t)(init_per_offspring ? row : 0) * E + ep) * EnvB::INIT_W, terrain[slot]);
#ifdef SES_PHASE_TIMERS
    phase_mark(-1);
#endif
    double ret = 0.0;
    int steps = 0;
    bool done = false;
    for (int t = 0; t < max_step; ++t) {
        if (__ballot(!done) == 0ull) break;
        float obs[S], logits[A], act[A];
#ifdef SES_PHASE_TIMERS
        phase_mark(10);
#endif
        EnvB::observe(st, obs);
#pragma unroll
        for (int k = 0; k < S; ++k) obs[k] = ((obs_mask >> k) & 1u) ? 0.0f : obs[k];
        if constexpr (LPE > 8) {
            MlpSlice<S, A, 16> net;
            net.load(theta + (size_t)row * P, (int)(threadIdx.x & 15));
            net.forward(tanh_tab, obs, logits);
        } else if constexpr (LPE >= 4) {
            MlpSlice<S, A, LPE> net;
            net.load(theta + (size_t)row * P, sub);
            net.forward(tanh_tab, obs, logits);
        } else {
            mlp_forward_streamed<S, A, LPE>(theta + (size_t)row * P, sub, tanh_tab, obs, logits);
        }
#pragma unroll
        for (int k = 0; k < A; ++k) act[k] = tanh_(tanh_tab, logits[k]);
#ifdef SES_PHASE_TIMERS
#pragma unroll
        for (int k = 0; k < A; ++k) asm volatile("" : "+v"(act[k]));
        phase_mark(11);
#endif
        if (!done) {
            ret += (double)EnvB::step(st, act, done);
            steps += 1;
        }
    }
    if (valid && sub == 0) {
        ep_return[env] = ret;
        if (ep_steps) ep_steps[env] = steps;
    }
#ifdef SES_PHASE_TIMERS
    phase_flush();
#endif
}

template <int NA>
__global__ __launch_bounds__(64) void k_rollout_spread_mlp(const float *__restrict__ theta,
                                                           const float *__restrict__ init, int init_per_offspring,
                                                           int n_rows, int E, int P, int max_cycles,
                                                           double *__restrict__ ep_return)
{
    constexpr int LPE = 8, S = 6 * NA, A = 5;
    __shared__ TanhEntry tanh_tab[SES_TANH_N];
    stage_tanh_table(tanh_tab);
    const long long gtid = (long long)blockIdx.x * 64 + threadIdx.x;
    const int n_env = n_rows * E;
    int env = (int)(gtid / LPE);
    const int sub = (int)(threadIdx.x % LPE);
    const bool valid = env < n_env;
    env = valid ? env : n_env - 1;
    const int row = env / E;
    const int ep = env - row * E;
    MlpSlice<S, A, LPE> net;
    net.load(theta + (size_t)row * P, sub);
    const float *s0 = init + ((size_t)(init_per_offspring ? row : 0) * E + ep) * (4 * NA);
    SpreadState<NA> st;
#pragma unroll
    for (int i = 0; i < NA; ++i) {
        st.ax[i] = s0[2 * i]; st.ay[i] = s0[2 * i + 1];
        st.vx[i] = 0.0f; st.vy[i] = 0.0f;
        st.lx[i] = s0[2 * NA + 2 * i]; st.ly[i] = s0[2 * NA + 2 * i + 1];
    }
    double ret = 0.0;
    for (int t = 0; t < max_cycles; ++t) {
        int action[NA];
#pragma unroll
        for (int a = 0; a < NA; ++a) {
            float obs[S], logits[A];
            spread_obs<NA>(st, a, obs);
            net.forward(tanh_tab, obs, logits);
            action[a] = argmax_first<A>(logits);
        }
        ret += (double)spread_step<NA, true>(st, action, sub & 3);
    }
    if (valid && sub == 0) ep_return[env] = ret;
}

__global__ void k_fitness_mean(const double *__restrict__ ep_return, int n_rows, int E, float *__restrict__ fitness,
                               unsigned long long *__restrict__ stamp)
{
    const int i = blockIdx.x * blockDim.x + threadIdx.x;
    if (stamp && i == 0) *stamp = real_time();
    if (i >= n_rows) return;
    double total = 0.0;
    for (int e = 0; e < E; ++e) total += ep_return[(size_t)i * E + e];
    fitness[i] = (float)(total / (double)E);
}

__global__ void k_fitness_mean_granules(const double *__restrict__ ep_return, int n_rows, int E, float *__restrict__ fitness,
                                        unsigned long long *__restrict__ stamp, P2pGranuleView gv)
{
    const int i = blockIdx.x * blockDim.x + threadIdx.x;
    if (stamp && i == 0) *stamp = real_time();
    if (i >= n_rows) return;
    double total = 0.0;
    for (int e = 0; e < E; ++e) total += ep_return[(size_t)i * E + e];
    const float f = (float)(total / (double)E);
    fitness[i] = f;
    for (int r = 0; r < gv.world; ++r) granule_store(gv.dst[r] + i, gv.seq, f2u(f));
}

template <bool FIXED_LENGTH>
__device__ __forceinline__ void env_step_one(float &x, float &xd, float &th, float &thd, int action, float &ret,
                                             uint32_t &status, int max_step)
{
    const bool done = (status >> 31) != 0u;
    const uint32_t steps = status & 0x7fffffffu;
    CartPoleState s{x, xd, th, thd};
    const bool term = cartpole_step(s, action);
    const bool advance = FIXED_LENGTH ? true : !done;
    x = advance ? s.x : x;
    xd = advance ? s.xd : xd;
    th = advance ? s.th : th;
    thd = advance ? s.thd : thd;
    const uint32_t nsteps = steps + 1u;
    const bool now_done = term | (max_step > 0 && (int)nsteps >= max_step);
    ret = done ? ret : ret + 1.0f;
    status = done ? status : (nsteps | ((uint32_t)now_done << 31));
}

typedef float f32x4 __attribute__((ext_vector_type(4)));
typedef uint32_t u32x4 __attribute__((ext_vector_type(4)));
typedef int32_t i32x4 __attribute__((ext_vector_type(4)));

template <bool FIXED_LENGTH>
__global__ __launch_bounds__(256) void k_env_step_cartpole_v4(int n4, int max_step, f32x4 *__restrict__ x,
                                                              f32x4 *__restrict__ xd, f32x4 *__restrict__ th,
                                                              f32x4 *__restrict__ thd,
                                                              const i32x4 *__restrict__ action,
                                                              f32x4 *__restrict__ ret, u32x4 *__restrict__ status)
{
    const int stride = gridDim.x * blockDim.x;
    for (int i = blockIdx.x * blockDim.x + threadIdx.x; i < n4; i += stride) {
        f32x4 vx = __builtin_nontemporal_load(x + i), vxd = __builtin_nontemporal_load(xd + i),
              vth = __builtin_nontemporal_load(th + i), vthd = __builtin_nontemporal_load(thd + i),
              vr = __builtin_nontemporal_load(ret + i);
        const i32x4 va = __builtin_nontemporal_load(action + i);
        u32x4 vs = __builtin_nontemporal_load(status + i);
#pragma unroll
        for (int l = 0; l < 4; ++l) {
            float ex = vx[l], exd = vxd[l], eth = vth[l], ethd = vthd[l], er = vr[l];
            uint32_t es = vs[l];
            env_step_one<FIXED_LENGTH>(ex, exd, eth, ethd, va[l], er, es, max_step);
            vx[l] = ex; vxd[l] = exd; vth[l] = eth; vthd[l] = ethd; vr[l] = er; vs[l] = es;
        }
        __builtin_nontemporal_store(vx, x + i);
        __builtin_nontemporal_store(vxd, xd + i);
        __builtin_nontemporal_store(vth, th + i);
        __builtin_nontemporal_store(vthd, thd + i);
        __builtin_nontemporal_store(vr, ret + i);
        __builtin_nontemporal_store(vs, status + i);
    }
}

__global__ __launch_bounds__(256) void k_stream_probe13(int n4, f32x4 *__restrict__ x, f32x4 *__restrict__ xd,
                                                        f32x4 *__restrict__ th, f32x4 *__restrict__ thd,
                                                        const i32x4 *__restrict__ action, f32x4 *__restrict__ ret,
                                                        u32x4 *__restrict__ status)
{
    const int stride = gridDim.x * blockDim.x;
    for (int i = blockIdx.x * blockDim.x + threadIdx.x; i < n4; i += stride) {
        f32x4 vx = __builtin_nontemporal_load(x + i);
        const f32x4 vxd = __builtin_nontemporal_load(xd + i), vth = __builtin_nontemporal_load(th + i),
                    vthd = __builtin_nontemporal_load(thd + i), vr = __builtin_nontemporal_load(ret + i);
        const i32x4 va = __builtin_nontemporal_load(action + i);
        const u32x4 vs = __builtin_nontemporal_load(status + i);
        asm volatile("" ::"v"(va));
        f32x4 wxd = vxd, wth = vth, wthd = vthd, wr = vr;
        u32x4 ws = vs;
        asm volatile("" : "+v"(vx), "+v"(wxd), "+v"(wth), "+v"(wthd), "+v"(wr), "+v"(ws));
        __builtin_nontemporal_store(vx, x + i);
        __builtin_nontemporal_store(wxd, xd + i);
        __builtin_nontemporal_store(wth, th + i);
        __builtin_nontemporal_store(wthd, thd + i);
        __builtin_nontemporal_store(wr, ret + i);
        __builtin_nontemporal_store(ws, status + i);
    }
}

template <bool FIXED_LENGTH>
__global__ void k_env_step_cartpole_scalar(int first, int n, int max_step, float *x, float *xd, float *th, float *thd,
                                           const int32_t *action, float *ret, uint32_t *status)
{
    const int i = first + blockIdx.x * blockDim.x + threadIdx.x;
    if (i >= n) return;
    float vx = x[i], vxd = xd[i], vth = th[i], vthd = thd[i], vr = ret[i];
    uint32_t vs = status[i];
    env_step_one<FIXED_LENGTH>(vx, vxd, vth, vthd, action[i], vr, vs, max_step);
    x[i] = vx; xd[i] = vxd; th[i] = vth; thd[i] = vthd; ret[i] = vr; status[i] = vs;
}

static int pick_lanes_per_env(const ses_handle *h, long long n_env)
{
    if (h->cfg.lanes_per_env) return h->cfg.lanes_per_env;
    if (n_env * 4 / 64 >= 640) return 4;
    return n_env <= 4096 ? 16 : 8;
}

template <int LPE, int BLOCK, bool PK = false, bool PHYS64 = false>
static void launch_rollout_b(const ses_handle *h, const RolloutArgs &a, int mode)
{
    const dim3 grid(ceil_div(a.episodes() * LPE, BLOCK)), block(BLOCK);
    with_fixed_length(mode, [&](auto fixed) {
        launch_rollout_kernel(h, k_rollout_cartpole_mlp<LPE, fixed(), BLOCK, PHYS64, PK>, grid, block, a);
    });
}

static bool cartpole_mlp_packed(const ses_handle *h, int lpe, long long episodes)
{
    if (lpe != 8 && lpe != 16) return false;
    if (h->tune_rollout_packed >= 0) return h->tune_rollout_packed != 0;
    return ceil_div(episodes * lpe, 64) <= h->tune_rollout_waves8;
}

template <int LPE>
static void launch_rollout(const ses_handle *h, const RolloutArgs &a, int mode)
{
    if constexpr (LPE == 8 || LPE == 16) {
        if (h->tune_rollout_block != 256 && cartpole_mlp_packed(h, LPE, a.episodes())) {
            launch_rollout_b<LPE, 64, true>(h, a, mode);
            return;
        }
    }
    if (h->tune_rollout_block == 256) launch_rollout_b<LPE, 256>(h, a, mode);
    else launch_rollout_b<LPE, 64>(h, a, mode);
}

static void box2d_wave_shape(const ses_handle *h, long long episodes, int waves_per_simd, int &lpe, int &epw)
{
    if (h->tune_box2d_lpe) {
        lpe = h->tune_box2d_lpe;
        epw = h->tune_box2d_epw ? h->tune_box2d_epw : 64 / lpe;
        if (epw > 64 / lpe) epw = 64 / lpe;
        return;
    }
    const long long slots = 1024ll * waves_per_simd;
    long long need = h->tune_box2d_epw ? h->tune_box2d_epw : (episodes + slots - 1) / slots;
    epw = (int)(need < 1 ? 1 : need > 64 ? 64 : need);
    lpe = 64;
    while (lpe > 1 && epw * lpe > 64) lpe >>= 1;
}

template <class EnvB>
static void launch_box2d_mlp(const ses_handle *h, const RolloutArgs &a)
{
    int lpe, epw;
    box2d_wave_shape(h, a.episodes(), EnvB::WAVES_PER_SIMD, lpe, epw);
    const dim3 grid(ceil_div(a.episodes(), epw)), block(64);
    const auto launch = [&](auto lanes) { launch_rollout_kernel(h, k_rollout_box2d_mlp<EnvB, lanes()>, grid, block, a, epw); };
    if (!with_lanes<64, 32, 16, 8, 4, 2, 1>(lpe, launch)) with_lanes<1>(1, launch);
}

static int lander_offspring_per_wave(const ses_handle *h, int n_rows)
{
    if (h->tune_lander_per_wave) return h->tune_lander_per_wave;
    return n_rows >= 3072 ? 4 : (n_rows >= 1536 ? 2 : 1);
}

static GruForm gru_form(const ses_handle *h, const RolloutArgs &a)
{
    const bool lander = h->cfg.env_id == SES_ENV_LUNARLANDER;
    const int E = h->cfg.eval_ep_num;
    if (h->tune_gru_sequential != 0) return GruForm::Sequential;
    if (a.episodes() <= h->tune_gru_ep_parallel_max && E > 1) return GruForm::EpisodeParallel;
    if (!lander && h->tune_gru_mfma4_min_e > 0 && E >= h->tune_gru_mfma4_min_e && E <= G4_EB) return GruForm::Mfma4;
    if (E >= h->tune_gru_mfma_min_e) return GruForm::Mfma;
    const int per_wave = lander && E <= GL_EB ? lander_offspring_per_wave(h, a.n_rows) : 1;
    return per_wave == 4 ? GruForm::LockstepMulti4 : (per_wave == 2 ? GruForm::LockstepMulti2 : GruForm::Lockstep);
}

struct MlpSplit {
    int light;
    int lpe;
};

static MlpSplit choose_cartpole_mlp_split(const ses_handle *h, long long episodes)
{
    if (h->cfg.lanes_per_env) return MlpSplit{0, h->cfg.lanes_per_env};
    if (h->tune_rollout_lpe32_max > 0 && episodes <= h->tune_rollout_lpe32_max) return MlpSplit{0, 32};
    if (episodes > 49152) return MlpSplit{0, 4};
    const int simds = h->tune_rollout_waves8;
    auto instr = [](int lpe) { return lpe == 4 ? 160.0 : (lpe == 8 ? 104.0 : 84.0); };
    auto cadence = [](long long k) { return k <= 1 ? 5.0 : (k == 2 ? 3.45 : (k == 3 ? 3.1 : 2.95)); };
    MlpSplit best{0, 8};
    double best_cost = -1.0;
    auto consider = [&](MlpSplit sp, double cost) {
        if (best_cost < 0.0 || cost < best_cost) { best_cost = cost; best = sp; }
    };
    const bool mix_only = h->tune_rollout_mix_light != 0;
    if (!mix_only) {
        for (int lpe : {16, 8, 4}) {
            const long long k = ceil_div(ceil_div(episodes * lpe, 64), simds);
            consider(MlpSplit{0, lpe}, k * instr(lpe) * cadence(k));
        }
    }
    if ((h->tune_rollout_mix || mix_only) && episodes > 8192) {
        for (int light : {16, 8}) {
            if (mix_only && light != h->tune_rollout_mix_light) continue;
            const long long envs_light = (long long)simds * (64 / light);
            if (episodes <= envs_light) continue;
            const long long kh = ceil_div(ceil_div(episodes - envs_light, 16), simds);
            consider(MlpSplit{light, 4}, (instr(light) + 160.0 * kh) * cadence(1 + kh));
        }
        const long long envs8 = (long long)simds * 8;
        if (h->tune_rollout_mix_8_16 && !mix_only && episodes > envs8) {
            const long long k16 = ceil_div(ceil_div(episodes - envs8, 4), simds);
            consider(MlpSplit{8, 16}, (104.0 + 84.0 * k16) * cadence(1 + k16));
        }
    }
    return best;
}

struct PairShape {
    int waves_light, waves_rest, handover;
};
static bool cartpole_mlp_pair_shape(const ses_handle *h, long long episodes, int mode, PairShape &ps)
{
    const MlpSplit sp = choose_cartpole_mlp_split(h, episodes);
    if (!sp.light) return false;
    const int epw = 64 / sp.light, knob = h->tune_rollout_waves8, epw_rest = 64 / sp.lpe;
    ps.waves_light = (long long)knob * epw < episodes ? knob : (int)(episodes / epw);
    ps.waves_rest = ceil_div(episodes - (long long)epw * ps.waves_light, epw_rest);
    ps.handover = h->tune_rollout_handover_step;
    return mode == SES_MODE_FIXED_LENGTH && sp.light == 16 && sp.lpe == 4 && ps.waves_rest <= ps.waves_light &&
           (ps.handover < h->cfg.max_step || h->tune_rollout_heavy_prio_steps > 0);
}

constexpr int HEAVY_PACKED_DEFAULT = 1;
static int cartpole_mlp_heavy_packed(const ses_handle *h)
{
    return h->tune_rollout_heavy_packed >= 0 ? h->tune_rollout_heavy_packed : HEAVY_PACKED_DEFAULT;
}

constexpr size_t PERTURB_ROLLOUT_LDS_MAX = 56u << 10;
static size_t perturb_rollout_lds(int P, int E) { return sizeof(float) * ((size_t)(P + 3) / 4 * 4 + (size_t)pair_own_rows(E) * P); }

bool cartpole_perturb_rollout_ok(const ses_handle *h, int n_rows, int mode)
{
    if (!h->tune_fused_perturb_rollout || h->cfg.env_id != SES_ENV_CARTPOLE || h->cfg.gru || h->cfg.physics64 || n_rows < 1) return false;
    PairShape ps;
    return cartpole_mlp_pair_shape(h, (long long)n_rows * h->cfg.eval_ep_num, mode, ps) &&
           perturb_rollout_lds(h->P, h->cfg.eval_ep_num) <= PERTURB_ROLLOUT_LDS_MAX;
}

static void launch_cartpole_mlp_pairs_perturb(ses_handle *h, const RolloutArgs &a, const PairShape &ps);
static void launch_cartpole_mlp_pairs_packed(ses_handle *h, const RolloutArgs &a, const PairShape &ps);

static void launch_cartpole_mlp(ses_handle *h, const RolloutArgs &a, int mode)
{
    const long long episodes = a.episodes();
    const MlpSplit sp = choose_cartpole_mlp_split(h, episodes);
    if (sp.light) {
        PairShape ps;
        const bool pairs = cartpole_mlp_pair_shape(h, episodes, mode, ps);
        const int waves_light = ps.waves_light, waves_rest = ps.waves_rest, handover = ps.handover;
        const dim3 grid(waves_light + waves_rest), block(64);
        if (pairs) {
            h->count_pair_rollouts += 1;
            if (h->perturb_pending) {
                launch_cartpole_mlp_pairs_perturb(h, a, ps);
                return;
            }
            if (cartpole_mlp_heavy_packed(h)) {
                launch_cartpole_mlp_pairs_packed(h, a, ps);
                return;
            }
            launch_rollout_kernel(h, k_rollout_cartpole_mlp_handover<true>, dim3(ceil_div(waves_light, HANDOVER_PAIRS)),
                                  dim3(64 * 2 * HANDOVER_PAIRS), a, waves_light, waves_rest, handover, h->tune_rollout_heavy_prio_steps);
            return;
        }
        with_fixed_length(mode, [&](auto fixed) {
            constexpr bool FIXED = fixed();
            const auto mix = [&](auto light, auto rest) {
                launch_rollout_kernel(h, k_rollout_cartpole_mlp_mix<FIXED, light(), rest()>, grid, block, a, waves_light);
            };
            if (sp.lpe == 16) mix(lanes_c<8>{}, lanes_c<16>{});
            else if (sp.light == 16) mix(lanes_c<16>{}, lanes_c<4>{});
            else mix(lanes_c<8>{}, lanes_c<4>{});
        });
        return;
    }
    const auto launch = [&](auto lanes) { launch_rollout<lanes()>(h, a, mode); };
    if (!with_lanes<1, 2, 4, 16, 32, 8>(sp.lpe, launch)) with_lanes<8>(8, launch);
}

struct EnvStepShape {
    int blocks, block, lds;
};
static void env_step_resolve(ses_handle *h)
{
    const int block = h->tune_env_step_block;
    if (h->env_step_key[0] == block && h->env_step_key[1] == h->tune_env_step_lds && h->env_step_key[2] == h->tune_env_step_waves) return;
    auto occupancy = [&](int lds) {
        int nb = 0;
        if (hipOccupancyMaxActiveBlocksPerMultiprocessor(&nb, k_env_step_cartpole_v4<true>, block, (size_t)lds) != hipSuccess) {
            (void)hipGetLastError();
            nb = 0;
        }
        return nb;
    };
    int lds = h->tune_env_step_lds;
    if (lds < 0) {
        int wgs = h->tune_env_step_waves * 64 / block;
        if (wgs < 1) wgs = 1;
        lds = h->lds_per_cu > 0 ? h->lds_per_cu / wgs / 256 * 256 : 0;
        if (lds > 65536) lds = 65536;
        for (int tries = 0; tries < 16 && lds > 256; ++tries) {
            const int nb = occupancy(lds);
            if (nb == 0 || nb == wgs) break;
            if (nb < wgs) lds -= 256;
            else if (lds + 256 <= 65536 && occupancy(lds + 256) >= wgs) lds += 256;
            else break;
        }
    }
    h->env_step_lds_resolved = lds;
    h->env_step_wpc = occupancy(lds) * block / 64;
    h->env_step_key[0] = block; h->env_step_key[1] = h->tune_env_step_lds; h->env_step_key[2] = h->tune_env_step_waves;
}

static EnvStepShape env_step_shape(ses_handle *h, int n4)
{
    EnvStepShape sh;
    env_step_resolve(h);
    sh.block = h->tune_env_step_block;
    sh.lds = h->env_step_lds_resolved;
    const long long want = ceil_div((long long)n4, sh.block);
    sh.blocks = want < (1 << 20) ? (int)want : (1 << 20);
    return sh;
}

static int rollout_lander(const ses_handle *h, const RolloutArgs &a, int mode)
{
    SES_REQUIRE(mode == SES_MODE_EPISODIC, "ses_rollout: LunarLander has no fixed-length mode");
    if (h->cfg.discrete_action) {
        int lpe = 0, epw = 0;
        if (!h->cfg.gru) box2d_wave_shape(h, a.episodes(), LanderMlpEnv::WAVES_PER_SIMD, lpe, epw);
        return lander_discrete_rollout(h, a, h->cfg.gru ? gru_form(h, a) : GruForm::Lockstep, lpe, epw);
    }
    const dim3 block(256);
    if (h->cfg.gru) {
        switch (const GruForm form = gru_form(h, a)) {
            case GruForm::EpisodeParallel:
            case GruForm::Sequential: {
                const bool epp = form == GruForm::EpisodeParallel;
                hipLaunchKernelGGL(k_rollout_lander_gru, dim3(ceil_div(epp ? a.episodes() : a.n_rows, 4)), block, 0, h->stream, a.theta,
                                   a.init, a.per, a.n_rows, a.E, a.P, a.max_step, a.obs_mask, a.epr, a.ep_steps, epp ? 1 : 0);
                break;
            }
            case GruForm::Mfma:
                launch_rollout_kernel(h, k_rollout_gru_mfma<LanderLs, false>, dim3(ceil_div(a.n_rows, 4)), block, a);
                break;
            case GruForm::LockstepMulti4:
                launch_rollout_kernel(h, k_rollout_gru_lockstep_multi<LanderLs, 4>, dim3(ceil_div(a.n_rows, 16)), block, a);
                break;
            case GruForm::LockstepMulti2:
                launch_rollout_kernel(h, k_rollout_gru_lockstep_multi<LanderLs, 2>, dim3(ceil_div(a.n_rows, 8)), block, a);
                break;
            default:
                launch_rollout_kernel(h, k_rollout_gru_lockstep<LanderLs, false, 1>, dim3(a.n_rows), dim3(64), a);
                break;
        }
    } else {
        launch_box2d_mlp<LanderMlpEnv>(h, a);
    }
    return SES_OK;
}

static int rollout_walker(const ses_handle *h, const RolloutArgs &a, int mode)
{
    SES_REQUIRE(mode == SES_MODE_EPISODIC, "ses_rollout: BipedalWalker has no fixed-length mode");
    SES_REQUIRE(!h->cfg.gru, "ses_rollout: BipedalWalker has an MLP-policy kernel only (conf/bipedalwalker.yaml: gru False)");
    launch_box2d_mlp<WalkerMlpEnv>(h, a);
    return SES_OK;
}

static int rollout_spread(const ses_handle *h, const RolloutArgs &a)
{
    SES_REQUIRE(a.ep_steps == nullptr, "ses_rollout: simple_spread episodes have a fixed length, no ep_steps");
    if (h->cfg.gru) return spread_gru_rollout(h, a);
    const dim3 grid(ceil_div(a.episodes() * 8, 64)), block(64);
    with_lanes<2, 3>(h->cfg.n_agents == 2 ? 2 : 3, [&](auto agents) {
        hipLaunchKernelGGL(k_rollout_spread_mlp<agents()>, grid, block, 0, h->stream, a.theta, a.init, a.per, a.n_rows, a.E, a.P,
                           a.max_step, a.epr);
    });
    return SES_OK;
}

static int rollout_cartpole(ses_handle *h, const RolloutArgs &a, int mode)
{
    const dim3 rows4(ceil_div(a.n_rows, 4)), block(256);
    if (h->cfg.physics64) {
        if (h->cfg.gru)
            with_fixed_length(mode, [&](auto fixed) {
                launch_rollout_kernel(h, k_rollout_gru_lockstep<CartPoleLs64, fixed(), 4>, rows4, block, a);
            });
        else if (pick_lanes_per_env(h, a.episodes()) >= 8) launch_rollout_b<8, 64, false, true>(h, a, mode);
        else launch_rollout_b<4, 64, false, true>(h, a, mode);
    } else if (h->cfg.gru) {
        switch (const GruForm form = gru_form(h, a)) {
            case GruForm::EpisodeParallel:
            case GruForm::Sequential: {
                const bool epp = form == GruForm::EpisodeParallel;
                const dim3 grid(ceil_div(epp ? a.episodes() : a.n_rows, 4));
                with_fixed_length(mode, [&](auto fixed) {
                    hipLaunchKernelGGL(k_rollout_cartpole_gru<fixed()>, grid, block, 0, h->stream, a.theta, a.init, a.per, a.n_rows, a.E,
                                       a.P, a.max_step, a.obs_mask, a.epr, a.ep_steps, epp ? 1 : 0);
                });
                break;
            }
            case GruForm::Mfma4:
                with_fixed_length(mode, [&](auto fixed) {
                    launch_rollout_kernel(h, k_rollout_gru_mfma4<CartPoleLs, fixed()>, rows4, block, a);
                });
                break;
            case GruForm::Mfma:
                with_fixed_length(mode, [&](auto fixed) {
                    launch_rollout_kernel(h, k_rollout_gru_mfma<CartPoleLs, fixed()>, rows4, block, a);
                });
                break;
            default:
                with_fixed_length(mode, [&](auto fixed) {
                    launch_rollout_kernel(h, k_rollout_gru_lockstep<CartPoleLs, fixed(), 4>, rows4, block, a);
                });
                break;
        }
    } else {
        launch_cartpole_mlp(h, a, mode);
    }
    return SES_OK;
}

}

extern "C" {

int ses_rollout(ses_handle *h, const float *theta, const float *init, int32_t init_per_offspring, int32_t n_rows,
                int32_t mode, float *fitness, double *ep_return, int32_t *ep_steps)
{
    using namespace ses;
    SES_REQUIRE(h && theta && init && fitness, "ses_rollout: null argument");
    SES_REQUIRE(n_rows >= 1, "ses_rollout: n_rows must be >= 1");
    SES_REQUIRE(mode == SES_MODE_EPISODIC || mode == SES_MODE_FIXED_LENGTH, "ses_rollout: bad mode %d", mode);
    SES_REQUIRE((long long)n_rows * h->cfg.eval_ep_num * 16 < (1ll << 31), "ses_rollout: shard too large");
    SES_REQUIRE(h->cfg.env_id == SES_ENV_CARTPOLE || h->cfg.env_id == SES_ENV_SIMPLE_SPREAD ||
                    h->cfg.env_id == SES_ENV_LUNARLANDER || h->cfg.env_id == SES_ENV_BIPEDALWALKER || is_classic_env(h->cfg.env_id),
                "ses_rollout: handle has no env");
    SES_HIP_TRY(hipSetDevice(h->cfg.device));
    const size_t episodes = (size_t)n_rows * h->cfg.eval_ep_num;
    double *epr = ep_return;
    if (!epr) {
        int rc = ensure_episode_scratch(h, episodes);
        if (rc != SES_OK) return rc;
        epr = h->ep_return;
    }
    const RolloutArgs a{theta, init, init_per_offspring, n_rows, h->cfg.eval_ep_num, h->P, h->cfg.max_step, h->obs_mask, epr, ep_steps};
    int rc;
    if (h->perturb_pending && !(theta == h->pending.theta && n_rows == h->pending.n_rows && mode == h->defer_mode &&
                                cartpole_perturb_rollout_ok(h, n_rows, mode))) {
        rc = flush_pending_perturb(h);
        if (rc != SES_OK) return rc;
    }
    switch (h->cfg.env_id) {
        case SES_ENV_CARTPOLE: rc = rollout_cartpole(h, a, mode); break;
        case SES_ENV_LUNARLANDER: rc = rollout_lander(h, a, mode); break;
        case SES_ENV_BIPEDALWALKER: rc = rollout_walker(h, a, mode); break;
        case SES_ENV_SIMPLE_SPREAD: rc = rollout_spread(h, a); break;
        default: rc = classic_rollout(h, a, mode); break;
    }
    if (rc != SES_OK) return rc;
    if (h->skip_mean) {
        SES_REQUIRE(epr == h->ep_return, "ses_rollout: the fused episode mean works on the handle's own episode scratch");
    } else if (h->fit_gv)
        hipLaunchKernelGGL(k_fitness_mean_granules, dim3(ceil_div(n_rows, 256)), dim3(256), 0, h->stream, epr, n_rows,
                           h->cfg.eval_ep_num, fitness, h->stamp, *h->fit_gv);
    else
        hipLaunchKernelGGL(k_fitness_mean, dim3(ceil_div(n_rows, 256)), dim3(256), 0, h->stream, epr, n_rows,
                           h->cfg.eval_ep_num, fitness, h->stamp);
    SES_HIP_TRY(hipGetLastError());
    return SES_OK;
}

int ses_env_step(ses_handle *h, int32_t n, int32_t mode, float *x, float *xd, float *th, float *thd,
                 const int32_t *action, float *ret, uint32_t *status)
{
    using namespace ses;
    SES_REQUIRE(h && x && xd && th && thd && action && ret && status, "ses_env_step: null argument");
    SES_REQUIRE(n >= 1, "ses_env_step: n must be >= 1");
    SES_REQUIRE(mode == SES_MODE_EPISODIC || mode == SES_MODE_FIXED_LENGTH, "ses_env_step: bad mode %d", mode);
    SES_REQUIRE(h->cfg.env_id == SES_ENV_CARTPOLE, "ses_env_step: handle has no env");
    SES_HIP_TRY(hipSetDevice(h->cfg.device));
    const uintptr_t align = (uintptr_t)x | (uintptr_t)xd | (uintptr_t)th | (uintptr_t)thd | (uintptr_t)action |
                            (uintptr_t)ret | (uintptr_t)status;
    const int n4 = (align & 15u) ? 0 : n / 4;
    const int max_step = h->cfg.max_step;
    if (n4 > 0) {
        const EnvStepShape sh = env_step_shape(h, n4);
        with_fixed_length(mode, [&](auto fixed) {
            hipLaunchKernelGGL(k_env_step_cartpole_v4<fixed()>, dim3(sh.blocks), dim3(sh.block), sh.lds, h->stream, n4, max_step,
                               (f32x4 *)x, (f32x4 *)xd, (f32x4 *)th, (f32x4 *)thd, (const i32x4 *)action, (f32x4 *)ret,
                               (u32x4 *)status);
        });
    }
    const int first = n4 * 4;
    if (first < n) {
        const int blocks = ceil_div(n - first, 256);
        with_fixed_length(mode, [&](auto fixed) {
            hipLaunchKernelGGL(k_env_step_cartpole_scalar<fixed()>, dim3(blocks), dim3(256), 0, h->stream, first, n, max_step, x, xd,
                               th, thd, action, ret, status);
        });
    }
    SES_HIP_TRY(hipGetLastError());
    return SES_OK;
}

int ses_env_step_shape(ses_handle *h, int32_t *block, int32_t *lds_bytes, int32_t *waves_per_cu, int32_t *lds_per_cu)
{
    using namespace ses;
    SES_REQUIRE(h, "ses_env_step_shape: null handle");
    SES_HIP_TRY(hipSetDevice(h->cfg.device));
    env_step_resolve(h);
    if (block) *block = h->tune_env_step_block;
    if (lds_bytes) *lds_bytes = h->env_step_lds_resolved;
    if (waves_per_cu) *waves_per_cu = h->env_step_wpc;
    if (lds_per_cu) *lds_per_cu = h->lds_per_cu;
    return SES_OK;
}

int ses_stream_probe(ses_handle *h, int32_t n, float *x, float *xd, float *th, float *thd, const int32_t *action, float *ret,
                     uint32_t *status)
{
    using namespace ses;
    SES_REQUIRE(h && x && xd && th && thd && action && ret && status, "ses_stream_probe: null argument");
    const uintptr_t align = (uintptr_t)x | (uintptr_t)xd | (uintptr_t)th | (uintptr_t)thd | (uintptr_t)action |
                            (uintptr_t)ret | (uintptr_t)status;
    SES_REQUIRE(n >= 4 && (n & 3) == 0 && (align & 15u) == 0, "ses_stream_probe: n must be a multiple of 4 and the arrays 16-byte aligned");
    SES_HIP_TRY(hipSetDevice(h->cfg.device));
    const int n4 = n / 4;
    const EnvStepShape sh = env_step_shape(h, n4);
    hipLaunchKernelGGL(k_stream_probe13, dim3(sh.blocks), dim3(sh.block), sh.lds, h->stream, n4, (f32x4 *)x, (f32x4 *)xd, (f32x4 *)th,
                       (f32x4 *)thd, (const i32x4 *)action, (f32x4 *)ret, (u32x4 *)status);
    SES_HIP_TRY(hipGetLastError());
    return SES_OK;
}

int ses_policy_forward(ses_handle *h, const float *theta, const float *obs, float *hidden, int32_t n, float *logits,
                       float *act, int32_t *action)
{
    using namespace ses;
    SES_REQUIRE(h && theta && obs && logits && action, "ses_policy_forward: null argument");
    SES_REQUIRE(n >= 1 && (long long)n * 4 < (1ll << 31), "ses_policy_forward: n out of range");
    SES_HIP_TRY(hipSetDevice(h->cfg.device));
    const int S = h->cfg.num_state, A = h->cfg.num_action;
    bool known;
    if (h->cfg.gru) {
        SES_REQUIRE(hidden, "ses_policy_forward: GRU policy needs the hidden-state array");
        known = with_policy_shape<PolicyShape<4, 2>, PolicyShape<8, 4>>(S, A, [&](auto sh) {
            hipLaunchKernelGGL((k_policy_forward_gru<sh.S, sh.A>), dim3(ceil_div(n, 4)), dim3(256), 0, h->stream, theta, obs, hidden, n,
                               h->P, logits, act, action);
        });
    } else {
        known = with_policy_shape<PolicyShape<4, 2>, PolicyShape<8, 4>, PolicyShape<12, 5>, PolicyShape<18, 5>, PolicyShape<24, 4>>(
            S, A, [&](auto sh) {
                hipLaunchKernelGGL((k_policy_forward_mlp<sh.S, sh.A>), dim3(ceil_div((long long)n * 4, 64)), dim3(64), 0, h->stream,
                                   theta, obs, n, h->P, logits, act, action);
            });
    }
    if (known) {
        SES_HIP_TRY(hipGetLastError());
        return SES_OK;
    }
    if (is_classic_policy_shape(S, A)) return classic_policy_forward(h, theta, obs, hidden, n, logits, act, action);
    if (h->cfg.gru && is_spread_policy_shape(S, A))
        return spread_gru_policy_forward(h, theta, obs, hidden, n, logits, act, action);
    if (h->cfg.gru) return set_error(SES_ERR_UNSUPPORTED, "ses_policy_forward: no GRU kernel instance for num_state=%d num_action=%d", S, A);
    return set_error(SES_ERR_UNSUPPORTED, "ses_policy_forward: no kernel instance for num_state=%d num_action=%d", S, A);
}

}

namespace ses {

static void launch_cartpole_mlp_pairs_perturb(ses_handle *h, const RolloutArgs &a, const PairShape &ps)
{
    h->perturb_pending = 0;
    h->count_perturb_rollouts += 1;
    const auto launch = [&](auto kernel) {
        hipLaunchKernelGGL(kernel, dim3(ceil_div(ps.waves_light, HANDOVER_PAIRS)), dim3(64 * 2 * HANDOVER_PAIRS),
                           perturb_rollout_lds(a.P, a.E), h->stream, a.init, a.per, a.n_rows, a.E, a.P, a.max_step, a.obs_mask,
                           ps.waves_light, ps.waves_rest, ps.handover, h->tune_rollout_heavy_prio_steps, a.epr, a.ep_steps, h->pending);
    };
    if (!cartpole_mlp_heavy_packed(h)) launch(k_rollout_cartpole_mlp_handover_perturb<true>);
    else launch(k_rollout_cartpole_mlp_handover_perturb<true, true>);
}

static void launch_cartpole_mlp_pairs_packed(ses_handle *h, const RolloutArgs &a, const PairShape &ps)
{
    launch_rollout_kernel(h, k_rollout_cartpole_mlp_handover<true, true>, dim3(ceil_div(ps.waves_light, HANDOVER_PAIRS)),
                          dim3(64 * 2 * HANDOVER_PAIRS), a, ps.waves_light, ps.waves_rest, ps.handover, h->tune_rollout_heavy_prio_steps);
}

}

#ifdef SES_PHASE_TIMERS
extern "C" int ses_debug_phase_totals(unsigned long long *out24, int reset)
{
    if (hipMemcpyFromSymbol(out24, HIP_SYMBOL(ses::phase_total), ses::PHASE_SLOTS * sizeof(unsigned long long)) != hipSuccess) return -1;
    if (reset) {
        unsigned long long z[ses::PHASE_SLOTS] = {};
        if (hipMemcpyToSymbol(HIP_SYMBOL(ses::phase_total), z, sizeof z) != hipSuccess) return -1;
    }
    return 0;
}
#endif
```

simple-es_amd/ses/_lib.py:

```python
import ctypes
import os

_HERE = os.path.dirname(os.path.abspath(__file__))
LIB_PATH = os.environ.get("SES_LIB_PATH") or os.path.join(os.path.dirname(_HERE), "libses_hip.so")

SES_OK = 0
ENV_NONE = -1
ENV_CARTPOLE = 0
ENV_LUNARLANDER = 1
ENV_SIMPLE_SPREAD = 2
ENV_BIPEDALWALKER = 3
ENV_ACROBOT = 4
ENV_MOUNTAINCAR = 5
ENV_PENDULUM = 6
ENV_MOUNTAINCAR_CONT = 7
MODE_EPISODIC = 0
MODE_FIXED_LENGTH = 1
HIDDEN = 32


class SesConfig(ctypes.Structure):
    _fields_ = [
        ("env_id", ctypes.c_int32),
        ("num_state", ctypes.c_int32),
        ("num_action", ctypes.c_int32),
        ("discrete_action", ctypes.c_int32),
        ("gru", ctypes.c_int32),
        ("pomdp", ctypes.c_int32),
        ("max_step", ctypes.c_int32),
        ("eval_ep_num", ctypes.c_int32),
        ("device", ctypes.c_int32),
        ("lanes_per_env", ctypes.c_int32),
        ("n_agents", ctypes.c_int32),
        ("physics64", ctypes.c_int32),
    ]


class SesSepcmaParams(ctypes.Structure):
    _fields_ = [
        ("mu", ctypes.c_int32), ("reserved", ctypes.c_int32),
        ("mueff", ctypes.c_double), ("c_sigma", ctypes.c_double), ("d_sigma", ctypes.c_double), ("c_c", ctypes.c_double),
        ("c_1", ctypes.c_double), ("c_mu", ctypes.c_double), ("chi", ctypes.c_double),
        ("scale_lo", ctypes.c_float), ("scale_hi", ctypes.c_float), ("step_lo", ctypes.c_float), ("step_hi", ctypes.c_float),
    ]


class SesLmmaParams(ctypes.Structure):
    _fields_ = [
        ("mu", ctypes.c_int32), ("m", ctypes.c_int32),
        ("mueff", ctypes.c_double), ("c_sigma", ctypes.c_double), ("d_sigma", ctypes.c_double), ("chi", ctypes.c_double),
        ("step_lo", ctypes.c_float), ("step_hi", ctypes.c_float),
        ("cd", ctypes.c_float * 32), ("ad", ctypes.c_float * 32), ("ac", ctypes.c_float * 32), ("bc", ctypes.c_float * 32),
    ]


LMMA_MAX_MEMORY = 32
LMMA_MAX_P = 16384


class SesGenState(ctypes.Structure):
    _fields_ = [
        ("strategy", ctypes.c_int32), ("n", ctypes.c_int32), ("elite_num", ctypes.c_int32), ("mode", ctypes.c_int32),
        ("shared_init", ctypes.c_int32), ("init_width", ctypes.c_int32),
        ("init_lo", ctypes.c_float), ("init_hi", ctypes.c_float),
        ("seed", ctypes.c_uint64), ("env_seed", ctypes.c_uint64),
        ("learning_rate", ctypes.c_double), ("sigma_decay", ctypes.c_double),
        ("sigma", ctypes.c_double), ("pop_sigma", ctypes.c_double),
        ("pop_gen", ctypes.c_uint64), ("adam_t", ctypes.c_int64),
        ("cur", ctypes.c_int32), ("world", ctypes.c_int32),
        ("theta", ctypes.c_void_p * 2), ("parents", ctypes.c_void_p * 2),
        ("adam_m", ctypes.c_void_p * 2), ("adam_v", ctypes.c_void_p * 2),
        ("parent_map", ctypes.c_void_p), ("alias_state", ctypes.c_void_p),
        ("fitness", ctypes.c_void_p), ("init", ctypes.c_void_p),
        ("work_i32", ctypes.c_void_p), ("work_f32", ctypes.c_void_p),
        ("first_row", ctypes.c_int64), ("n_local", ctypes.c_int32), ("per_rank", ctypes.c_int32),
        ("comm", ctypes.c_void_p), ("fit_local", ctypes.c_void_p),
        ("scale", ctypes.c_void_p * 2),
        ("sigma_learning_rate", ctypes.c_double), ("sigma_max_change", ctypes.c_double),
        ("scale_lo", ctypes.c_float), ("scale_hi", ctypes.c_float),
        ("cma_C", ctypes.c_void_p * 2), ("cma_ps", ctypes.c_void_p * 2), ("cma_pc", ctypes.c_void_p * 2),
        ("cma_step", ctypes.c_void_p * 2), ("cma_weights", ctypes.c_void_p), ("cma", SesSepcmaParams),
        ("lm_ps", ctypes.c_void_p * 2), ("lm_M", ctypes.c_void_p * 2), ("lm_step", ctypes.c_void_p * 2),
        ("lm_weights", ctypes.c_void_p), ("lm", SesLmmaParams),
    ]


STRATEGY_OPENAI_ES, STRATEGY_SIMPLE_EVOLUTION, STRATEGY_SIMPLE_GENETIC, STRATEGY_PGPE, STRATEGY_SEP_CMA_ES = 0, 1, 2, 3, 4
STRATEGY_LM_MA_ES = 5

_vp = ctypes.c_void_p
_i32 = ctypes.c_int32
_i64 = ctypes.c_int64
_u64 = ctypes.c_uint64
_f32 = ctypes.c_float
_f64 = ctypes.c_double

SIGNATURES = {
    "ses_create": [ctypes.POINTER(SesConfig), _vp, ctypes.POINTER(_vp)],
    "ses_destroy": [_vp],
    "ses_sync": [_vp],
    "ses_set_tuning": [_vp, ctypes.c_char_p, _i32],
    "ses_launch_counts": [_vp, _vp, _vp, _vp],
    "ses_set_stamp": [_vp, _vp],
    "ses_last_error": [],
    "ses_version": [],
    "ses_param_count": [_i32, _i32, _i32],
    "ses_device_count": [],
    "ses_perturb": [_vp, _vp, _vp, _vp, _f32, _u64, _u64, _i64, _i32, _vp],
    "ses_noise": [_vp, _u64, _u64, _i64, _i32, _vp],
    "ses_perturb_host_noise": [_vp, _vp, _vp, _vp, _f64, _i32, _vp, _vp],
    "ses_init_states_uniform": [_vp, _u64, _u64, _i64, _i32, _i32, _i32, _f32, _f32, _vp],
    "ses_init_states_uniform_gens": [_vp, _u64, _u64, _i32, _i64, _i32, _i32, _i32, _f32, _f32, _vp],
    "ses_policy_forward": [_vp, _vp, _vp, _vp, _i32, _vp, _vp, _vp],
    "ses_env_step": [_vp, _i32, _i32, _vp, _vp, _vp, _vp, _vp, _vp, _vp],
    "ses_env_state_bytes": [_vp],
    "ses_env_obs_width": [_vp],
    "ses_env_reset": [_vp, _vp, _i32, _vp, _vp],
    "ses_env_step_generic": [_vp, _vp, _vp, _i32, _vp, _vp, _vp],
    "ses_env_step_shape": [_vp, _vp, _vp, _vp, _vp],
    "ses_stream_probe": [_vp, _i32, _vp, _vp, _vp, _vp, _vp, _vp, _vp],
    "ses_rollout": [_vp, _vp, _vp, _i32, _i32, _i32, _vp, _vp, _vp],
    "ses_rank_center": [_vp, _vp, _i32, _vp, _vp, _vp],
    "ses_es_update_philox": [_vp, _vp, _i32, _i32, _u64, _u64, _f64, _f64, _f64, _vp, _vp, _vp, _vp],
    "ses_openai_generation": [_vp, _vp, _i32, _u64, _u64, _f64, _f64, _f64, _vp, _vp, _vp, _vp, _vp, _vp, _f32, _u64, _i64, _i32,
                              _vp, _vp],
    "ses_openai_sharded_ok": [_vp, _vp, _i32, _i32, _i32],
    "ses_openai_generation_sharded": [_vp, _vp, _vp, _i32, _u64, _u64, _f64, _f64, _f64, _vp, _vp, _vp, _vp, _vp, _vp, _f32, _u64,
                                      _i64, _i32, _i32, _i32, _vp, _vp],
    "ses_es_update_stored": [_vp, _vp, _i32, _vp, _f64, _f64, _f64, _vp, _vp, _vp, _vp],
    "ses_perturb_mirrored": [_vp, _vp, _vp, _f32, _u64, _u64, _i64, _i32, _vp],
    "ses_pgpe_generation": [_vp, _vp, _i32, _u64, _u64, _f64, _f64, _f64, _f64, _f32, _f32, _vp, _vp, _vp, _vp, _vp, _vp, _vp, _vp,
                            _f32, _u64, _i64, _i32, _vp, _vp, _vp, _vp],
    "ses_perturb_sepcma": [_vp, _vp, _vp, _vp, _f32, _u64, _u64, _i64, _i32, _vp],
    "ses_sepcma_generation": [_vp, _vp, _i32, _u64, _u64, _f64, _f64, ctypes.POINTER(SesSepcmaParams), _vp, _vp, _vp, _vp, _vp, _vp,
                              _vp, _vp, _vp, _vp, _vp, _f32, _u64, _i64, _i32, _vp, _vp, _vp, _vp, _vp],
    "ses_perturb_lmma": [_vp, _vp, _vp, _vp, ctypes.POINTER(SesLmmaParams), _i32, _f32, _u64, _u64, _i64, _i32, _vp, _vp],
    "ses_lmma_generation": [_vp, _vp, _i32, _u64, _u64, _f64, ctypes.POINTER(SesLmmaParams), _vp, _i32, _i32, _vp, _vp, _vp, _vp,
                            _vp, _vp, _vp, _vp, _f32, _u64, _i64, _i32, _vp, _vp, _vp, _vp, _vp, _vp, _vp],
    "ses_elite_ids": [_vp, _vp, _i32, _i32, _vp],
    "ses_elite_select": [_vp, _vp, _i32, _i32, _vp, _vp, _vp, _vp, _vp],
    "ses_elite_mean": [_vp, _vp, _vp, _i32, _vp],
    "ses_gather_rows": [_vp, _vp, _vp, _i32, _vp],
    "ses_run_generations": [_vp, ctypes.POINTER(SesGenState), _i32, _vp, _vp],
    "ses_comm_unique_id": [_vp],
    "ses_comm_init": [_vp, _i32, _i32, _vp],
    "ses_comm_info": [_vp, _vp, _vp, _vp],
    "ses_comm_destroy": [_vp],
    "ses_allgather_fitness": [_vp, _vp, _i32, _vp],
    "ses_comm_p2p_export": [_vp, _i32, _i32, _i32, _vp],
    "ses_comm_p2p_attach": [_vp, _vp],
    "ses_comm_p2p_attach_local": [_vp, _vp],
    "ses_stream_create_exclusive": [_i32, _vp],
    "ses_stream_destroy": [_vp],
    "ses_comm_p2p_info": [_vp, _vp, _vp, _vp],
    "ses_comm_p2p_counts": [_vp, _vp, _vp],
    "ses_comm_p2p_status": [_vp, _vp],
    "ses_comm_p2p_reset_status": [_vp],
    "ses_comm_p2p_detach": [_vp],
}
COMM_ID_BYTES = 128
COMM_P2P_HANDLE_BYTES = 64
_RESTYPE = {"ses_last_error": ctypes.c_char_p, "ses_version": ctypes.c_char_p}

_lib = None


class SesError(RuntimeError):
    pass


def load():
    global _lib
    if _lib is not None:
        return _lib
    if not os.path.exists(LIB_PATH):
        raise SesError(f"{LIB_PATH} not found: build it with simple-es_amd/csrc/build.sh "
                       f"(hipcc --offload-arch=gfx950). There is no CPU fallback.")
    lib = ctypes.CDLL(LIB_PATH)
    for name, argtypes in SIGNATURES.items():
        fn = getattr(lib, name)
        fn.argtypes = argtypes
        fn.restype = _RESTYPE.get(name, ctypes.c_int)
    _lib = lib
    return lib


def check(rc, what=""):
    if rc != SES_OK:
        msg = load().ses_last_error().decode("utf-8", "replace")
        raise SesError(f"{what or 'libses_hip'} failed (code {rc}): {msg}")
    return rc
```

simple-es_amd/ses/device.py:

```python
import contextlib
import ctypes
import os
import sys

import torch

from . import _lib
from ._lib import (ENV_ACROBOT, ENV_BIPEDALWALKER, ENV_CARTPOLE, ENV_LUNARLANDER, ENV_MOUNTAINCAR, ENV_MOUNTAINCAR_CONT, ENV_NONE,
                   ENV_PENDULUM, ENV_SIMPLE_SPREAD, HIDDEN, MODE_EPISODIC, SesConfig, SesError, check)

ENV_IDS = {"CartPole-v1": ENV_CARTPOLE, "CartPole-v0": ENV_CARTPOLE, "simple_spread": ENV_SIMPLE_SPREAD,
           "LunarLanderContinuous-v2": ENV_LUNARLANDER, "LunarLander-v2": ENV_LUNARLANDER, "BipedalWalker-v3": ENV_BIPEDALWALKER, "Acrobot-v1": ENV_ACROBOT,
           "MountainCar-v0": ENV_MOUNTAINCAR, "Pendulum-v1": ENV_PENDULUM, "MountainCarContinuous-v0": ENV_MOUNTAINCAR_CONT,
           None: ENV_NONE}
LANDER_DISCRETE = {"LunarLander-v2": True, "LunarLanderContinuous-v2": False}


def param_count(num_state, num_action, gru):
    return _lib.load().ses_param_count(int(num_state), int(num_action), int(bool(gru)))


def _ptr(t):
    return None if t is None else ctypes.c_void_p(t.data_ptr())


@contextlib.contextmanager
def _stdout_to_stderr():
    sys.stdout.flush()
    saved = os.dup(1)
    try:
        os.dup2(2, 1)
        yield
    finally:
        sys.stdout.flush()
        os.dup2(saved, 1)
        os.close(saved)


def exclusive_stream(device=None):
    if not torch.cuda.is_available():
        raise SesError("no HIP device visible to torch")
    device = torch.cuda.current_device() if device is None else int(device)
    raw = ctypes.c_void_p()
    check(_lib.load().ses_stream_create_exclusive(device, ctypes.byref(raw)), "ses_stream_create_exclusive")
    return torch.cuda.ExternalStream(raw.value, device=torch.device("cuda", device))


def destroy_stream(stream):
    stream.synchronize()
    check(_lib.load().ses_stream_destroy(ctypes.c_void_p(stream.cuda_stream)), "ses_stream_destroy")


class HipES:

    def __init__(self, env_name="CartPole-v1", num_state=4, num_action=2, discrete_action=True, gru=False,
                 pomdp=False, max_step=500, eval_ep_num=5, device=None, lanes_per_env=0, n_agents=1,
                 physics64=False, stream=None):
        if env_name in LANDER_DISCRETE and bool(discrete_action) != LANDER_DISCRETE[env_name]:
            other = next(k for k in LANDER_DISCRETE if k != env_name)
            raise SesError(f"{env_name} takes discrete_action={LANDER_DISCRETE[env_name]} "
                           f"(discrete_action={bool(discrete_action)} is {other})")
        lib = _lib.load()
        if not torch.cuda.is_available():
            raise SesError("no HIP device visible to torch: the simple-es hot path needs an MI355X "
                           "(there is no CPU fallback)")
        if env_name not in ENV_IDS:
            raise SesError(f"env {env_name!r} has no device kernel (available: {sorted(k for k in ENV_IDS if k)})")
        device = torch.cuda.current_device() if device is None else int(device)
        self.device = torch.device("cuda", device)
        self.S, self.A = int(num_state), int(num_action)
        self.discrete, self.gru, self.pomdp = bool(discrete_action), bool(gru), bool(pomdp)
        self.max_step, self.E = int(max_step), int(eval_ep_num)
        self.P = param_count(self.S, self.A, self.gru)
        self.env_id = ENV_IDS[env_name]
        self.n_agents = int(n_agents)
        if self.env_id == ENV_SIMPLE_SPREAD:
            self.init_dim, self.init_range = 4 * self.n_agents, (-1.0, 1.0)
        elif self.env_id == ENV_LUNARLANDER:
            self.init_dim, self.init_range = 16, (0.0, 1.0)
        elif self.env_id == ENV_BIPEDALWALKER:
            self.init_dim, self.init_range = 4, (0.0, 1.0)
        elif self.env_id == ENV_ACROBOT:
            self.init_dim, self.init_range = 4, (-0.1, 0.1)
        elif self.env_id == ENV_MOUNTAINCAR:
            self.init_dim, self.init_range = 1, (-0.6, -0.4)
        elif self.env_id == ENV_PENDULUM:
            self.init_dim, self.init_range = 2, (-1.0, 1.0)
        elif self.env_id == ENV_MOUNTAINCAR_CONT:
            self.init_dim, self.init_range = 1, (-0.6, -0.4)
        else:
            self.init_dim, self.init_range = 4, (-0.05, 0.05)
        cfg = SesConfig(self.env_id, self.S, self.A, int(self.discrete), int(self.gru), int(self.pomdp),
                        self.max_step, self.E, int(device), int(lanes_per_env), self.n_agents, int(bool(physics64)))
        self._lib = lib
        self._h = ctypes.c_void_p()
        with torch.cuda.device(self.device):
            self.stream = torch.cuda.current_stream(self.device) if stream is None else stream
            check(lib.ses_create(ctypes.byref(cfg), ctypes.c_void_p(self.stream.cuda_stream), ctypes.byref(self._h)),
                  "ses_create")
        for item in filter(None, os.environ.get("SES_TUNING", "").split(",")):
            name, _, value = item.partition("=")
            self.set_tuning(name.strip(), int(value))

    def set_tuning(self, name, value):
        check(self._lib.ses_set_tuning(self._h, name.encode(), int(value)), "ses_set_tuning")

    def launch_counts(self):
        out = [ctypes.c_int64(0) for _ in range(3)]
        check(self._lib.ses_launch_counts(self._h, *[ctypes.byref(o) for o in out]), "ses_launch_counts")
        return tuple(int(o.value) for o in out)

    def set_stamp(self, dst):
        if dst is not None and not (isinstance(dst, torch.Tensor) and dst.dtype == torch.int64 and dst.numel() >= 1 and
                                    (dst.is_pinned() if dst.device.type == "cpu" else dst.device == self.device)):
            raise SesError("set_stamp: expected a pinned host or device int64 tensor")
        self._stamp_keepalive = dst
        check(self._lib.ses_set_stamp(self._h, _ptr(dst)), "ses_set_stamp")

    def close(self):
        if getattr(self, "_h", None) is not None and self._h.value:
            self._lib.ses_destroy(self._h)
            self._h = ctypes.c_void_p()

    def __del__(self):
        try:
            self.close()
        except Exception:
            pass

    def _chk(self, t, name, dtype, shape, optional=False):
        if t is None:
            if optional:
                return None
            raise SesError(f"{name}: tensor required")
        if not isinstance(t, torch.Tensor):
            raise SesError(f"{name}: expected a torch tensor, got {type(t).__name__}")
        if t.device != self.device:
            raise SesError(f"{name}: on {t.device}, handle is on {self.device}")
        if t.dtype != dtype:
            raise SesError(f"{name}: dtype {t.dtype}, expected {dtype}")
        if not t.is_contiguous():
            raise SesError(f"{name}: must be contiguous")
        if tuple(t.shape) != tuple(shape):
            raise SesError(f"{name}: shape {tuple(t.shape)}, expected {tuple(shape)}")
        return t

    def _chk_best(self, best):
        if best is None:
            return None
        if isinstance(best, torch.Tensor) and best.device.type == "cpu":
            if not (best.is_pinned() and best.dtype == torch.float32 and best.numel() == 1 and best.is_contiguous()):
                raise SesError("best: a host tensor must be pinned float32[1]")
            return best
        return self._chk(best, "best", torch.float32, (1,))

    def _check_parent_idx(self, parent_idx, K):
        last = getattr(self, "_idx_checked", None)
        if last is not None and last[0] is parent_idx and last[1] == parent_idx._version and last[2] == K:
            return
        lo, hi = int(parent_idx.min()), int(parent_idx.max())
        if hi >= K or lo < -K:
            raise SesError(f"parent_idx outside [-{K}, {K})")
        self._idx_checked = (parent_idx, parent_idx._version, K)

    def empty(self, *shape, dtype=torch.float32):
        return torch.empty(*shape, dtype=dtype, device=self.device)

    def zeros(self, *shape, dtype=torch.float32):
        return torch.zeros(*shape, dtype=dtype, device=self.device)

    def alloc_env_soa(self, n, skew_bytes=4096):
        stride = (n * 4 + skew_bytes + 15) // 16 * 16
        pool = torch.zeros(stride * 7 // 4, dtype=torch.float32, device=self.device)
        views = [pool[k * stride // 4: k * stride // 4 + n] for k in range(7)]
        x, xd, th, thd, action, ret, status = views
        return x, xd, th, thd, action.view(torch.int32), ret, status.view(torch.int32)

    def sync(self):
        check(self._lib.ses_sync(self._h), "ses_sync")

    @staticmethod
    def comm_unique_id():
        buf = ctypes.create_string_buffer(_lib.COMM_ID_BYTES)
        with _stdout_to_stderr():
            check(_lib.load().ses_comm_unique_id(buf), "ses_comm_unique_id")
        return buf.raw

    def comm_init(self, rank, world, unique_id):
        if len(unique_id) != _lib.COMM_ID_BYTES:
            raise SesError(f"comm_init: unique id must be {_lib.COMM_ID_BYTES} bytes")
        buf = ctypes.create_string_buffer(bytes(unique_id), _lib.COMM_ID_BYTES)
        with _stdout_to_stderr():
            check(self._lib.ses_comm_init(self._h, int(rank), int(world), buf), "ses_comm_init")
        self._route = None

    def comm_info(self):
        r, w, v = ctypes.c_int32(), ctypes.c_int32(), ctypes.c_int32()
        check(self._lib.ses_comm_info(self._h, ctypes.byref(r), ctypes.byref(w), ctypes.byref(v)), "ses_comm_info")
        return r.value, w.value, v.value

    def comm_destroy(self):
        check(self._lib.ses_comm_destroy(self._h), "ses_comm_destroy")
        self._route = None

    def comm_p2p_export(self, rank, world, max_per_rank):
        buf = ctypes.create_string_buffer(_lib.COMM_P2P_HANDLE_BYTES)
        check(self._lib.ses_comm_p2p_export(self._h, int(rank), int(world), int(max_per_rank), buf), "ses_comm_p2p_export")
        return buf.raw

    def comm_p2p_attach(self, handles):
        blob = b"".join(bytes(h) for h in handles)
        check(self._lib.ses_comm_p2p_attach(self._h, ctypes.create_string_buffer(blob, len(blob))), "ses_comm_p2p_attach")
        self._route = None

    def comm_p2p_attach_local(self, peers):
        arr = (ctypes.c_void_p * len(peers))(*[p._h.value for p in peers])
        check(self._lib.ses_comm_p2p_attach_local(self._h, arr), "ses_comm_p2p_attach_local")
        self._route = None

    def comm_p2p_info(self):
        w, m, x = ctypes.c_int32(), ctypes.c_int32(), ctypes.c_int32()
        check(self._lib.ses_comm_p2p_info(self._h, ctypes.byref(w), ctypes.byref(m), ctypes.byref(x)), "ses_comm_p2p_info")
        return w.value, m.value, x.value

    def comm_p2p_counts(self):
        f, g = ctypes.c_int32(), ctypes.c_int32()
        check(self._lib.ses_comm_p2p_counts(self._h, ctypes.byref(f), ctypes.byref(g)), "ses_comm_p2p_counts")
        return f.value, g.value

    def comm_p2p_status(self):
        m = ctypes.c_uint32()
        check(self._lib.ses_comm_p2p_status(self._h, ctypes.byref(m)), "ses_comm_p2p_status")
        return m.value

    def comm_p2p_reset_status(self):
        check(self._lib.ses_comm_p2p_reset_status(self._h), "ses_comm_p2p_reset_status")

    def comm_p2p_detach(self):
        check(self._lib.ses_comm_p2p_detach(self._h), "ses_comm_p2p_detach")
        self._route = None

    def comm_route(self):
        r = getattr(self, "_route", None)
        if r is None:
            w, cap, _ = self.comm_p2p_info()
            r = self._route = (w, cap, self.comm_info()[1])
        return r

    def allgather_fitness(self, local, out=None):
        world, cap, rccl_world = self.comm_route()
        if world < 1 or local.shape[0] > cap:
            world = rccl_world
        if world < 1:
            raise SesError("allgather_fitness: the handle has no communicator (comm_init or comm_p2p_attach first)")
        n = local.shape[0]
        self._chk(local, "local", torch.float32, (n,))
        out = self.empty(world * n) if out is None else self._chk(out, "all", torch.float32, (world * n,))
        check(self._lib.ses_allgather_fitness(self._h, _ptr(local), int(n), _ptr(out)), "ses_allgather_fitness")
        return out

    def perturb(self, parents, sigma, seed, gen, first_row, n_rows, parent_idx=None, row_ids=None, out=None,
                idx_in_range=False):
        parents = parents.view(-1, self.P) if parents.dim() == 1 else parents
        K = parents.shape[0]
        self._chk(parents, "parents", torch.float32, (K, self.P))
        self._chk(parent_idx, "parent_idx", torch.int32, (n_rows,), optional=True)
        self._chk(row_ids, "row_ids", torch.int32, (n_rows,), optional=True)
        if parent_idx is not None and not idx_in_range:
            self._check_parent_idx(parent_idx, K)
        theta = self.empty(n_rows, self.P) if out is None else self._chk(out, "theta", torch.float32, (n_rows, self.P))
        check(self._lib.ses_perturb(self._h, _ptr(parents), _ptr(parent_idx), _ptr(row_ids), float(sigma), int(seed),
                                    int(gen), int(first_row), int(n_rows), _ptr(theta)), "ses_perturb")
        return theta

    def noise(self, seed, gen, first_row, n_rows):
        eps = self.empty(n_rows, self.P)
        check(self._lib.ses_noise(self._h, int(seed), int(gen), int(first_row), int(n_rows), _ptr(eps)), "ses_noise")
        return eps

    def perturb_host_noise(self, parents, eps64, sigma, parent_idx=None, want_eps_store=False):
        parents = parents.view(-1, self.P) if parents.dim() == 1 else parents
        K = parents.shape[0]
        n_rows = eps64.shape[0]
        self._chk(parents, "parents", torch.float32, (K, self.P))
        self._chk(eps64, "eps64", torch.float64, (n_rows, self.P))
        self._chk(parent_idx, "parent_idx", torch.int32, (n_rows,), optional=True)
        if parent_idx is not None:
            self._check_parent_idx(parent_idx, K)
        theta = self.empty(n_rows, self.P)
        store = self.empty(n_rows, self.P) if want_eps_store else None
        check(self._lib.ses_perturb_host_noise(self._h, _ptr(parents), _ptr(parent_idx), _ptr(eps64), float(sigma),
                                               int(n_rows), _ptr(theta), _ptr(store)), "ses_perturb_host_noise")
        return (theta, store) if want_eps_store else theta

    def init_states_uniform(self, seed, gen, first_row, n_rows, shared=False, lo=None, hi=None, out=None):
        lo = self.init_range[0] if lo is None else lo
        hi = self.init_range[1] if hi is None else hi
        out = (self.empty(n_rows, self.E, self.init_dim) if out is None else
               self._chk(out, "out", torch.float32, (n_rows, self.E, self.init_dim)))
        check(self._lib.ses_init_states_uniform(self._h, int(seed), int(gen), int(first_row), int(n_rows),
                                                int(bool(shared)), int(self.init_dim), float(lo), float(hi), _ptr(out)),
              "ses_init_states_uniform")
        return out

    def init_states_uniform_gens(self, seed, gen0, gens, first_row, n_rows, shared=False, out=None):
        lo, hi = self.init_range
        out = (self.empty(gens, n_rows, self.E, self.init_dim) if out is None else
               self._chk(out, "out", torch.float32, (gens, n_rows, self.E, self.init_dim)))
        check(self._lib.ses_init_states_uniform_gens(self._h, int(seed), int(gen0), int(gens), int(first_row), int(n_rows),
                                                     int(bool(shared)), int(self.init_dim), float(lo), float(hi), _ptr(out)),
              "ses_init_states_uniform_gens")
        return out

    def policy_forward(self, theta, obs, hidden=None):
        n = obs.shape[0]
        self._chk(theta, "theta", torch.float32, (n, self.P))
        self._chk(obs, "obs", torch.float32, (n, self.S))
        if self.gru:
            self._chk(hidden, "hidden", torch.float32, (n, HIDDEN))
        logits = self.empty(n, self.A)
        act = self.empty(n, self.A)
        action = self.empty(n, dtype=torch.int32)
        check(self._lib.ses_policy_forward(self._h, _ptr(theta), _ptr(obs), _ptr(hidden if self.gru else None), int(n),
                                           _ptr(logits), _ptr(act), _ptr(action)), "ses_policy_forward")
        return action, logits, act

    def env_step(self, x, xd, th, thd, action, ret, status, mode=MODE_EPISODIC):
        n = x.shape[0]
        for name, t in (("x", x), ("xd", xd), ("th", th), ("thd", thd), ("ret", ret)):
            self._chk(t, name, torch.float32, (n,))
        self._chk(action, "action", torch.int32, (n,))
        self._chk(status, "status", torch.int32, (n,))
        check(self._lib.ses_env_step(self._h, int(n), int(mode), _ptr(x), _ptr(xd), _ptr(th), _ptr(thd), _ptr(action),
                                     _ptr(ret), _ptr(status)), "ses_env_step")

    def run_generations(self, state, k, best, stamps=None):
        if not (isinstance(best, torch.Tensor) and best.dtype == torch.float32 and best.numel() >= k and best.is_contiguous()
                and (best.is_pinned() if best.device.type == "cpu" else best.device == self.device)):
            raise SesError("run_generations: best must be a pinned host or device float32 tensor of at least k elements")
        if stamps is not None and not (isinstance(stamps, torch.Tensor) and stamps.dtype == torch.int64 and stamps.numel() >= 2 * k
                                       and stamps.is_contiguous()
                                       and (stamps.is_pinned() if stamps.device.type == "cpu" else stamps.device == self.device)):
            raise SesError("run_generations: stamps must be a pinned host or device int64 tensor of at least 2 k elements")
        check(self._lib.ses_run_generations(self._h, ctypes.byref(state), int(k), _ptr(best), _ptr(stamps)), "ses_run_generations")

    def env_state_bytes(self):
        b = self._lib.ses_env_state_bytes(self._h)
        if b <= 0:
            check(b, "ses_env_state_bytes")
        return b

    def env_obs_width(self):
        w = self._lib.ses_env_obs_width(self._h)
        if w <= 0:
            check(w, "ses_env_obs_width")
        return w

    def env_reset(self, init):
        n = init.shape[0]
        self._chk(init, "init", torch.float32, (n, self.init_dim))
        state = torch.zeros(n, self.env_state_bytes(), dtype=torch.uint8, device=self.device)
        obs = self.empty(n, self.env_obs_width())
        check(self._lib.ses_env_reset(self._h, _ptr(init), int(n), _ptr(state), _ptr(obs)), "ses_env_reset")
        return state, obs

    def env_step_generic(self, state, action):
        n = state.shape[0]
        self._chk(state, "state", torch.uint8, (n, self.env_state_bytes()))
        if self.env_id in (ENV_CARTPOLE, ENV_ACROBOT, ENV_MOUNTAINCAR) or (self.env_id == ENV_LUNARLANDER and self.discrete):
            self._chk(action, "action", torch.int32, (n,))
        elif self.env_id == ENV_SIMPLE_SPREAD:
            self._chk(action, "action", torch.int32, (n, self.n_agents))
        else:
            self._chk(action, "action", torch.float32, (n, self.A))
        obs = self.empty(n, self.env_obs_width())
        reward = self.empty(n)
        done = self.empty(n, dtype=torch.int32)
        check(self._lib.ses_env_step_generic(self._h, _ptr(state), _ptr(action), int(n), _ptr(obs), _ptr(reward), _ptr(done)),
              "ses_env_step_generic")
        return obs, reward, done

    def env_step_shape(self):
        b, l, w, c = ctypes.c_int32(), ctypes.c_int32(), ctypes.c_int32(), ctypes.c_int32()
        check(self._lib.ses_env_step_shape(self._h, ctypes.byref(b), ctypes.byref(l), ctypes.byref(w), ctypes.byref(c)),
              "ses_env_step_shape")
        return b.value, l.value, w.value, c.value

    def stream_probe(self, x, xd, th, thd, action, ret, status):
        n = x.shape[0]
        for name, t in (("x", x), ("xd", xd), ("th", th), ("thd", thd), ("ret", ret)):
            self._chk(t, name, torch.float32, (n,))
        self._chk(action, "action", torch.int32, (n,))
        self._chk(status, "status", torch.int32, (n,))
        check(self._lib.ses_stream_probe(self._h, int(n), _ptr(x), _ptr(xd), _ptr(th), _ptr(thd), _ptr(action), _ptr(ret),
                                         _ptr(status)), "ses_stream_probe")

    def rollout(self, theta, init, mode=MODE_EPISODIC, want_episodes=False, fitness=None):
        n_rows = theta.shape[0]
        self._chk(theta, "theta", torch.float32, (n_rows, self.P))
        if init.dim() == 2:
            self._chk(init, "init", torch.float32, (self.E, self.init_dim))
            per = 0
        else:
            self._chk(init, "init", torch.float32, (n_rows, self.E, self.init_dim))
            per = 1
        fitness = self.empty(n_rows) if fitness is None else self._chk(fitness, "fitness", torch.float32, (n_rows,))
        ep_ret = self.empty(n_rows, self.E, dtype=torch.float64) if want_episodes else None
        ep_steps = self.empty(n_rows, self.E, dtype=torch.int32) if (want_episodes and self.env_id != ENV_SIMPLE_SPREAD) else None
        check(self._lib.ses_rollout(self._h, _ptr(theta), _ptr(init), per, int(n_rows), int(mode), _ptr(fitness),
                                    _ptr(ep_ret), _ptr(ep_steps)), "ses_rollout")
        return (fitness, ep_ret, ep_steps) if want_episodes else fitness

    def rank_center(self, fitness, want_weights=True, best=None):
        n = fitness.shape[0]
        self._chk(fitness, "fitness", torch.float32, (n,))
        self._chk_best(best)
        rank = self.empty(n, dtype=torch.int32)
        weights = self.empty(n, dtype=torch.float64) if want_weights else None
        check(self._lib.ses_rank_center(self._h, _ptr(fitness), int(n), _ptr(rank), _ptr(weights), _ptr(best)),
              "ses_rank_center")
        return rank, weights

    def es_update_philox(self, weights, seed, gen, lr, sigma, adam_a, mu, m, v, skip_row0=True, want_grad=False):
        n = weights.shape[0]
        self._chk(weights, "weights", torch.float64, (n,))
        for name, t in (("mu", mu), ("m", m), ("v", v)):
            self._chk(t, name, torch.float32, (self.P,))
        grad = self.empty(self.P) if want_grad else None
        check(self._lib.ses_es_update_philox(self._h, _ptr(weights), int(n), int(bool(skip_row0)), int(seed), int(gen),
                                             float(lr), float(sigma), float(adam_a), _ptr(mu), _ptr(m), _ptr(v),
                                             _ptr(grad)), "ses_es_update_philox")
        return grad

    def openai_sharded_ok(self, comm, n, per_rank, world):
        rc = self._lib.ses_openai_sharded_ok(self._h, comm._h, int(n), int(per_rank), int(world))
        if rc < 0:
            check(rc, "ses_openai_sharded_ok")
        return rc == 1

    def openai_generation(self, fitness, seed, gen, lr, sigma, adam_a, state_in, state_out, next_sigma, next_gen,
                          first_row, n_rows, theta_next=None, best=None, comm=None, per_rank=0, world=1):
        n = fitness.shape[0]
        self._chk(fitness, "fitness", torch.float32, (n,))
        for name, t in zip(("mu_in", "m_in", "v_in", "mu_out", "m_out", "v_out"), tuple(state_in) + tuple(state_out)):
            self._chk(t, name, torch.float32, (self.P,))
        if any(a.data_ptr() == b.data_ptr() for a, b in zip(state_in, state_out)):
            raise SesError("openai_generation: state_in and state_out must be distinct buffers")
        self._chk_best(best)
        if not (0 <= first_row and first_row + n_rows <= n):
            raise SesError(f"openai_generation: rows [{first_row}, +{n_rows}) outside the population of {n}")
        theta = (self.empty(n_rows, self.P) if theta_next is None else
                 self._chk(theta_next, "theta_next", torch.float32, (n_rows, self.P)))
        if comm is not None:
            check(self._lib.ses_openai_generation_sharded(
                self._h, comm._h, _ptr(fitness), int(n), int(seed), int(gen), float(lr), float(sigma), float(adam_a),
                *[_ptr(t) for t in state_in], *[_ptr(t) for t in state_out], float(next_sigma), int(next_gen), int(first_row),
                int(n_rows), int(per_rank), int(world), _ptr(theta), _ptr(best)), "ses_openai_generation_sharded")
            return theta
        check(self._lib.ses_openai_generation(self._h, _ptr(fitness), int(n), int(seed), int(gen), float(lr), float(sigma),
                                              float(adam_a), *[_ptr(t) for t in state_in], *[_ptr(t) for t in state_out],
                                              float(next_sigma), int(next_gen), int(first_row), int(n_rows),
                                              _ptr(theta) if n_rows else None, _ptr(best)), "ses_openai_generation")
        return theta

    def _chk_vectors(self, names, tensors, shapes):
        for name, t, shape in zip(names, tensors, shapes):
            if shape is not None:
                self._chk(t, name, torch.float32, shape)

    def _chk_state(self, who, names, shapes, state_in, state_out):
        if len(state_in) != len(names) or len(state_out) != len(names):
            raise SesError(f"{who}: state_in / state_out are ({', '.join(names)})")
        for side, state in (("in", state_in), ("out", state_out)):
            self._chk_vectors([f"{name}_{side}" for name in names], state, shapes)
        if any(a.data_ptr() == b.data_ptr() and a.numel() for a, b in zip(state_in, state_out)):
            raise SesError(f"{who}: state_in and state_out must be distinct buffers")

    def _next_rows(self, who, n, first_row, n_rows, theta_next, best):
        self._chk_best(best)
        if not (0 <= first_row and 0 <= n_rows and first_row + n_rows <= n):
            raise SesError(f"{who}: rows [{first_row}, +{n_rows}) outside the population of {n}")
        return (self.empty(n_rows, self.P) if theta_next is None else
                self._chk(theta_next, "theta_next", torch.float32, (n_rows, self.P)))

    def _perturb_rows(self, who, first_row, n_rows, out):
        if not (first_row >= 0 and n_rows >= 1):
            raise SesError(f"{who}: bad row range [{first_row}, +{n_rows})")
        return self.empty(n_rows, self.P) if out is None else self._chk(out, "theta", torch.float32, (n_rows, self.P))

    def perturb_mirrored(self, mu, scale, sigma, seed, gen, first_row, n_rows, out=None):
        self._chk_vectors(("mu", "scale"), (mu, scale), ((self.P,),) * 2)
        theta = self._perturb_rows("perturb_mirrored", first_row, n_rows, out)
        check(self._lib.ses_perturb_mirrored(self._h, _ptr(mu), _ptr(scale), float(sigma), int(seed), int(gen), int(first_row),
                                             int(n_rows), _ptr(theta)), "ses_perturb_mirrored")
        return theta

    def pgpe_generation(self, fitness, seed, gen, sigma, adam_a, sigma_learning_rate, sigma_max_change, scale_limits, state_in,
                        state_out, next_sigma, next_gen, first_row, n_rows, theta_next=None, best=None, want_sums=False):
        n = fitness.shape[0]
        self._chk(fitness, "fitness", torch.float32, (n,))
        if n < 4 or n % 2:
            raise SesError(f"pgpe_generation: the population must be even and >= 4, got {n}")
        self._chk_state("pgpe_generation", ("mu", "m", "v", "scale"), ((self.P,),) * 4, state_in, state_out)
        lo, hi = (float(x) for x in scale_limits)
        if not (0.0 < lo <= hi and 0.0 <= sigma_max_change < 1.0):
            raise SesError("pgpe_generation: need 0 < scale_lo <= scale_hi and 0 <= sigma_max_change < 1")
        theta = self._next_rows("pgpe_generation", n, first_row, n_rows, theta_next, best)
        gmu = self.empty(self.P) if want_sums else None
        gs = self.empty(self.P) if want_sums else None
        check(self._lib.ses_pgpe_generation(self._h, _ptr(fitness), int(n), int(seed), int(gen), float(sigma), float(adam_a),
                                            float(sigma_learning_rate), float(sigma_max_change), lo, hi,
                                            *[_ptr(t) for t in state_in], *[_ptr(t) for t in state_out], float(next_sigma),
                                            int(next_gen), int(first_row), int(n_rows), _ptr(theta) if n_rows else None,
                                            _ptr(best), _ptr(gmu), _ptr(gs)), "ses_pgpe_generation")
        return (theta, gmu, gs) if want_sums else theta

    def perturb_sepcma(self, mu, C, step, sigma, seed, gen, first_row, n_rows, out=None):
        self._chk_vectors(("mu", "C", "step"), (mu, C, step), ((self.P,), (self.P,), (1,)))
        theta = self._perturb_rows("perturb_sepcma", first_row, n_rows, out)
        check(self._lib.ses_perturb_sepcma(self._h, _ptr(mu), _ptr(C), _ptr(step), float(sigma), int(seed), int(gen), int(first_row),
                                           int(n_rows), _ptr(theta)), "ses_perturb_sepcma")
        return theta

    def sepcma_generation(self, fitness, seed, gen, sigma, hsig_scale, params, weights, state_in, state_out, next_sigma, next_gen,
                          first_row, n_rows, theta_next=None, best=None, want_sums=False):
        n = fitness.shape[0]
        self._chk(fitness, "fitness", torch.float32, (n,))
        if n < 4:
            raise SesError(f"sepcma_generation: the population must have at least 4 rows, got {n}")
        if not isinstance(params, _lib.SesSepcmaParams):
            raise SesError("sepcma_generation: params must be a SesSepcmaParams")
        if not 1 <= params.mu <= n:
            raise SesError(f"sepcma_generation: mu = {params.mu} outside [1, {n}]")
        self._chk(weights, "weights", torch.float32, (params.mu,))
        self._chk_state("sepcma_generation", ("mu", "C", "p_sigma", "p_c", "step"), ((self.P,),) * 4 + ((1,),), state_in, state_out)
        if not (0.0 < params.scale_lo <= params.scale_hi and 0.0 < params.step_lo <= params.step_hi):
            raise SesError("sepcma_generation: need 0 < scale_lo <= scale_hi and 0 < step_lo <= step_hi")
        theta = self._next_rows("sepcma_generation", n, first_row, n_rows, theta_next, best)
        sz = self.empty(self.P) if want_sums else None
        szz = self.empty(self.P) if want_sums else None
        norm2 = self.empty(1, dtype=torch.float64) if want_sums else None
        check(self._lib.ses_sepcma_generation(self._h, _ptr(fitness), int(n), int(seed), int(gen), float(sigma), float(hsig_scale),
                                              ctypes.byref(params), _ptr(weights), *[_ptr(t) for t in state_in],
                                              *[_ptr(t) for t in state_out], float(next_sigma), int(next_gen), int(first_row),
                                              int(n_rows), _ptr(theta) if n_rows else None, _ptr(best), _ptr(sz), _ptr(szz),
                                              _ptr(norm2)), "ses_sepcma_generation")
        return (theta, sz, szz, norm2) if want_sums else theta

    def _chk_lmma(self, who, params, M, m_active, name="M"):
        if not isinstance(params, _lib.SesLmmaParams):
            raise SesError(f"{who}: params must be a SesLmmaParams")
        if self.P > _lib.LMMA_MAX_P:
            raise SesError(f"{who}: {self.P} parameters; the lm_ma_es kernels hold at most {_lib.LMMA_MAX_P}")
        if not 0 <= params.m <= _lib.LMMA_MAX_MEMORY:
            raise SesError(f"{who}: memory = {params.m} outside [0, {_lib.LMMA_MAX_MEMORY}]")
        if not 0 <= m_active <= params.m:
            raise SesError(f"{who}: m_active = {m_active} outside [0, memory = {params.m}]")
        self._chk(M, name, torch.float32, (params.m, self.P))

    def perturb_lmma(self, mu, M, step, params, m_active, sigma, seed, gen, first_row, n_rows, out=None, want_dots=False):
        self._chk_vectors(("mu", "step"), (mu, step), ((self.P,), (1,)))
        self._chk_lmma("perturb_lmma", params, M, m_active)
        theta = self._perturb_rows("perturb_lmma", first_row, n_rows, out)
        dots = self.empty(n_rows, m_active) if want_dots else None
        check(self._lib.ses_perturb_lmma(self._h, _ptr(mu), _ptr(M) if params.m else None, _ptr(step), ctypes.byref(params),
                                         int(m_active), float(sigma), int(seed), int(gen), int(first_row), int(n_rows), _ptr(theta),
                                         _ptr(dots) if want_dots and m_active else None), "ses_perturb_lmma")
        return (theta, dots) if want_dots else theta

    def lmma_generation(self, fitness, seed, gen, sigma, params, weights, m_active, m_active_next, state_in, state_out, next_sigma,
                        next_gen, first_row, n_rows, theta_next=None, best=None, want_sums=False):
        n = fitness.shape[0]
        self._chk(fitness, "fitness", torch.float32, (n,))
        if n < 4:
            raise SesError(f"lmma_generation: the population must have at least 4 rows, got {n}")
        self._chk_state("lmma_generation", ("mu", "p_sigma", "M", "step"), ((self.P,), (self.P,), None, (1,)), state_in, state_out)
        self._chk_lmma("lmma_generation", params, state_in[2], m_active, "M_in")
        self._chk_lmma("lmma_generation", params, state_out[2], m_active_next, "M_out")
        if not 1 <= params.mu <= n:
            raise SesError(f"lmma_generation: mu = {params.mu} outside [1, {n}]")
        self._chk(weights, "weights", torch.float32, (params.mu,))
        if not 0.0 < params.step_lo <= params.step_hi:
            raise SesError("lmma_generation: need 0 < step_lo <= step_hi")
        theta = self._next_rows("lmma_generation", n, first_row, n_rows, theta_next, best)
        sz = self.empty(self.P) if want_sums else None
        sd = self.empty(self.P) if want_sums else None
        sdots = self.empty(m_active) if want_sums else None
        norm2 = self.empty(1, dtype=torch.float64) if want_sums else None
        dots = self.empty(n_rows, m_active_next) if want_sums else None

        def opt(t):
            return _ptr(t) if t is not None and t.numel() else None
        M_in, M_out = (opt(state_in[2]), opt(state_out[2]))
        check(self._lib.ses_lmma_generation(self._h, _ptr(fitness), int(n), int(seed), int(gen), float(sigma), ctypes.byref(params),
                                            _ptr(weights), int(m_active), int(m_active_next), _ptr(state_in[0]), _ptr(state_in[1]),
                                            M_in, _ptr(state_in[3]), _ptr(state_out[0]), _ptr(state_out[1]), M_out,
                                            _ptr(state_out[3]), float(next_sigma), int(next_gen), int(first_row), int(n_rows),
                                            _ptr(theta) if n_rows else None, _ptr(best), _ptr(sz), _ptr(sd), opt(sdots), _ptr(norm2),
                                            opt(dots)), "ses_lmma_generation")
        return (theta, sz, sd, sdots, norm2, dots) if want_sums else theta

    def es_update_stored(self, weights, eps_store, lr, sigma, adam_a, mu, m, v, want_grad=False):
        n = weights.shape[0]
        self._chk(weights, "weights", torch.float64, (n,))
        self._chk(eps_store, "eps_store", torch.float32, (n, self.P))
        for name, t in (("mu", mu), ("m", m), ("v", v)):
            self._chk(t, name, torch.float32, (self.P,))
        grad = self.empty(self.P) if want_grad else None
        check(self._lib.ses_es_update_stored(self._h, _ptr(weights), int(n), _ptr(eps_store), float(lr), float(sigma),
                                             float(adam_a), _ptr(mu), _ptr(m), _ptr(v), _ptr(grad)),
              "ses_es_update_stored")
        return grad

    def elite_ids(self, rank, k):
        n = rank.shape[0]
        self._chk(rank, "rank", torch.int32, (n,))
        if not 1 <= k <= n:
            raise SesError(f"elite_ids: need 1 <= k <= n, got k={k} n={n}")
        ids = self.empty(k, dtype=torch.int32)
        check(self._lib.ses_elite_ids(self._h, _ptr(rank), int(n), int(k), _ptr(ids)), "ses_elite_ids")
        return ids

    def elite_select(self, rank, k, parent_map, alias_state=None):
        n = rank.shape[0]
        self._chk(rank, "rank", torch.int32, (n,))
        self._chk(parent_map, "parent_map", torch.int32, (n,))
        self._chk(alias_state, "alias_state", torch.int32, (1,), optional=True)
        if not 1 <= k <= min(n, 1024):
            raise SesError(f"elite_select: need 1 <= k <= min(n, 1024), got k={k} n={n}")
        out = self.empty(3, k, dtype=torch.int32)
        alias = out[2] if alias_state is not None else None
        check(self._lib.ses_elite_select(self._h, _ptr(rank), int(n), int(k), _ptr(parent_map), _ptr(alias_state),
                                         _ptr(out[0]), _ptr(out[1]), _ptr(alias)), "ses_elite_select")
        return out[0], out[1], alias

    def elite_mean(self, rows, alias_first=None):
        k = rows.shape[0]
        self._chk(rows, "rows", torch.float32, (k, self.P))
        self._chk(alias_first, "alias_first", torch.int32, (k,), optional=True)
        mean = self.empty(self.P)
        check(self._lib.ses_elite_mean(self._h, _ptr(rows), _ptr(alias_first), int(k), _ptr(mean)), "ses_elite_mean")
        return mean

    def gather_rows(self, src, ids):
        n_src = src.shape[0]
        k = ids.shape[0]
        self._chk(src, "src", torch.float32, (n_src, self.P))
        self._chk(ids, "ids", torch.int32, (k,))
        lo, hi = int(ids.min()), int(ids.max())
        if lo < 0 or hi >= n_src:
            raise SesError(f"gather_rows: ids outside [0, {n_src})")
        dst = self.empty(k, self.P)
        check(self._lib.ses_gather_rows(self._h, _ptr(src), _ptr(ids), int(k), _ptr(dst)), "ses_gather_rows")
        return dst
```

Measured before the change: 57.62 billion.

## Replicate tanh lookup table across LDS banks to avoid gather conflicts

Adds a banked variant of the CartPole handover rollout kernels that stages 16 copies of the tanh lookup table in dynamic LDS, interleaved so each lane reads its own copy. This is meant to remove LDS bank conflicts on the per-step table gathers in the packed heavy path. The perturb prologue is restructured so the larger table staging overlaps with noise drawing, and the loop is aligned and padded with NOPs. In exchange the kernel uses far more LDS per block, which can lower occupancy. A runtime check falls back to the old kernel if the LDS does not fit.

```diff
diff --git a/include/ses.h b/include/ses.h
--- a/include/ses.h
+++ b/include/ses.h
@@ -51,6 +51,7 @@
 int ses_sync(ses_handle *h);
 int ses_set_tuning(ses_handle *h, const char *name, int32_t value);
 int ses_launch_counts(ses_handle *h, int64_t *pair_rollouts, int64_t *perturb_rollouts, int64_t *apply_perturb);
+int ses_tanh_banked_count(ses_handle *h, int64_t *banked_rollouts);
 int ses_set_stamp(ses_handle *h, uint64_t *dst);
 const char *ses_last_error(void);
 const char *ses_version(void);
diff --git a/simple-es_amd/csrc/ses_core.hip b/simple-es_amd/csrc/ses_core.hip
--- a/simple-es_amd/csrc/ses_core.hip
+++ b/simple-es_amd/csrc/ses_core.hip
@@ -134,6 +134,7 @@
     h->tune_rollout_waves8 = 1024;
     h->tune_rollout_packed = -1;
     h->tune_rollout_heavy_packed = -1;
+    h->tune_rollout_tanh_banked = -1;
     h->tune_rollout_mix_8_16 = 1;
     h->tune_rollout_handover_step = 1 << 30;
     h->tune_rollout_heavy_prio_steps = 1 << 30;
@@ -190,6 +191,7 @@
                                  {"rollout_lpe32_max_envs", &ses_handle::tune_rollout_lpe32_max, 0, 1 << 30},
                                  {"rollout_packed", &ses_handle::tune_rollout_packed, -1, 1},
                                  {"rollout_heavy_packed", &ses_handle::tune_rollout_heavy_packed, -1, 1},
+                                 {"rollout_tanh_banked", &ses_handle::tune_rollout_tanh_banked, -1, 1},
                                  {"rollout_mix_8_16", &ses_handle::tune_rollout_mix_8_16, 0, 1},
                                  {"rollout_handover_step", &ses_handle::tune_rollout_handover_step, 0, 1 << 30},
                                  {"rollout_heavy_prio_steps", &ses_handle::tune_rollout_heavy_prio_steps, 0, 1 << 30},
@@ -247,6 +249,13 @@
     return SES_OK;
 }
 
+int ses_tanh_banked_count(ses_handle *h, int64_t *banked_rollouts)
+{
+    SES_REQUIRE(h && banked_rollouts, "ses_tanh_banked_count: null argument");
+    *banked_rollouts = h->count_tanh_banked;
+    return SES_OK;
+}
+
 int ses_set_stamp(ses_handle *h, uint64_t *dst)
 {
     SES_REQUIRE(h, "ses_set_stamp: null handle");
diff --git a/simple-es_amd/csrc/ses_internal.h b/simple-es_amd/csrc/ses_internal.h
--- a/simple-es_amd/csrc/ses_internal.h
+++ b/simple-es_amd/csrc/ses_internal.h
@@ -96,6 +96,8 @@
     long long count_pair_rollouts;
     long long count_perturb_rollouts;
     long long count_apply_perturb;
+    int tune_rollout_tanh_banked;
+    long long count_tanh_banked;
     int tune_pendulum_generic;
     int tune_pgpe_fused_apply_perturb;
     int tune_spread_gru_wave_per_batch;
diff --git a/simple-es_amd/csrc/ses_perturb_prologue.h b/simple-es_amd/csrc/ses_perturb_prologue.h
--- a/simple-es_amd/csrc/ses_perturb_prologue.h
+++ b/simple-es_amd/csrc/ses_perturb_prologue.h
@@ -1,6 +1,7 @@
 #pragma once
 #include "ses_internal.h"
 #include "ses_rng.h"
+#include "ses_tanh_banked.h"
 
 namespace ses {
 
@@ -162,4 +163,51 @@
     __syncthreads();
 }
 
-}
+constexpr int TANH_IMAGE_PER_THREAD = 10;
+__device__ __forceinline__ void perturb_prologue_banked(const PerturbUpdate &u, RowSpan a, RowSpan b, float *mu_new, float *lds_rows,
+                                                        TanhEntry *tanh_lds)
+{
+    const int tid = (int)threadIdx.x, block = (int)blockDim.x;
+    const int items = (a.rows + b.rows) * u.quads;
+    UpdateOperands first{};
+    if (tid < u.P) first = es_update_load(u, tid);
+    const float4 *tanh_src = reinterpret_cast<const float4 *>(&SES_TANH_TABLE[0][0]);
+    constexpr int HALF = TANH_IMAGE_PER_THREAD / 2;
+    float4 tv[HALF];
+    const auto load_half = [&](int k0) {
+#pragma unroll
+        for (int k = 0; k < HALF; ++k) {
+            const int i = tid + (k0 + k) * block;
+            tv[k] = tanh_src[(i < TANH_IMAGE_ENTRIES ? i : TANH_IMAGE_ENTRIES - 1) / TANH_BANK_COPIES];
+        }
+    };
+    const auto store_half = [&](int k0) {
+#pragma unroll
+        for (int k = 0; k < HALF; ++k) {
+            const int i = tid + (k0 + k) * block;
+            if (i < TANH_IMAGE_ENTRIES) tanh_lds[i] = TanhEntry{tv[k].x, tv[k].y, tv[k].z, tv[k].w};
+        }
+    };
+    load_half(0);
+    PerturbItems it;
+    int n = perturb_batch_count(0, items);
+    perturb_draw_n(u, a, b, 0, items, n, it);
+    store_half(0);
+    load_half(HALF);
+    perturb_update_mean(u, mu_new, &first);
+    __syncthreads();
+    perturb_store(u, mu_new, lds_rows, 0, items, n, it);
+    store_half(HALF);
+    for (int i = tid + 2 * HALF * block; i < TANH_IMAGE_ENTRIES; i += block) {
+        const float4 v = tanh_src[i / TANH_BANK_COPIES];
+        tanh_lds[i] = TanhEntry{v.x, v.y, v.z, v.w};
+    }
+    for (int base = PERTURB_BATCH * block; base < items; base += PERTURB_BATCH * block) {
+        n = perturb_batch_count(base, items);
+        perturb_draw_n(u, a, b, base, items, n, it);
+        perturb_store(u, mu_new, lds_rows, base, items, n, it);
+    }
+    __syncthreads();
+}
+
+}
diff --git a/simple-es_amd/csrc/ses_policy.h b/simple-es_amd/csrc/ses_policy.h
--- a/simple-es_amd/csrc/ses_policy.h
+++ b/simple-es_amd/csrc/ses_policy.h
@@ -2,6 +2,7 @@
 #include <hip/hip_runtime.h>
 
 #include "ses_math.h"
+#include "ses_tanh_banked.h"
 
 namespace ses {
 
@@ -83,7 +84,8 @@
         TanhEntry ent[U];
     };
 
-    __device__ __forceinline__ void begin(const TanhEntry *tab, const float (&obs)[S], Pending &pd) const
+    template <class Tab>
+    __device__ __forceinline__ void begin(Tab tab, const float (&obs)[S], Pending &pd) const
     {
         int32_t idx[U];
 #pragma unroll
@@ -96,7 +98,7 @@
         }
         __builtin_amdgcn_sched_barrier(0);
 #pragma unroll
-        for (int u = 0; u < U; ++u) pd.ent[u] = tab[idx[u]];
+        for (int u = 0; u < U; ++u) pd.ent[u] = tanh_entry(tab, idx[u]);
     }
 
     __device__ __forceinline__ void finish(const Pending &pd, float (&logits)[A]) const
@@ -229,6 +231,16 @@
     __syncthreads();
 }
 
+__device__ __forceinline__ void stage_tanh_table_banked(TanhEntry *image)
+{
+    const float4 *src = reinterpret_cast<const float4 *>(&SES_TANH_TABLE[0][0]);
+    for (int i = threadIdx.x; i < TANH_IMAGE_ENTRIES; i += blockDim.x) {
+        const float4 v = src[i / TANH_BANK_COPIES];
+        image[i] = TanhEntry{v.x, v.y, v.z, v.w};
+    }
+    __syncthreads();
+}
+
 __device__ __forceinline__ int add_mask_bit(int v, unsigned long long mask)
 {
     asm("v_addc_co_u32_e64 %0, vcc, %0, 0, %1" : "+v"(v) : "s"(mask) : "vcc");
diff --git a/simple-es_amd/csrc/ses_policy_pk.h b/simple-es_amd/csrc/ses_policy_pk.h
--- a/simple-es_amd/csrc/ses_policy_pk.h
+++ b/simple-es_amd/csrc/ses_policy_pk.h
@@ -1,4 +1,6 @@
 #pragma once
+#include <type_traits>
+
 #include "ses_cartpole.h"
 #include "ses_policy.h"
 
@@ -45,7 +47,8 @@
         TanhEntry ent[U];
     };
 
-    __device__ __forceinline__ void begin(const TanhEntry *tab, const float (&obs)[S], Pending &pd) const
+    template <class Tab>
+    __device__ __forceinline__ void begin(Tab tab, const float (&obs)[S], Pending &pd) const
     {
         int32_t idx[U];
         pk2 acc[UP];
@@ -65,7 +68,7 @@
         }
         __builtin_amdgcn_sched_barrier(0);
 #pragma unroll
-        for (int u = 0; u < U; ++u) pd.ent[u] = tab[idx[u]];
+        for (int u = 0; u < U; ++u) pd.ent[u] = tanh_entry(tab, idx[u]);
     }
 
     __device__ __forceinline__ pk2 finish(const Pending &pd) const
@@ -121,8 +124,10 @@
     }
 };
 
-template <int LPE, bool FIXED_LENGTH, bool MASKED>
-__device__ __forceinline__ void rollout_cartpole_mlp_loop_pk(const TanhEntry *tanh_tab, const MlpSlicePk<LPE> &net,
+constexpr int HEAVY_LOOP_PAD_NOPS = 5;
+
+template <int LPE, bool FIXED_LENGTH, bool MASKED, class Tab>
+__device__ __forceinline__ void rollout_cartpole_mlp_loop_pk(Tab tanh_tab, const MlpSlicePk<LPE> &net,
                                                              CartPoleSimPk &sim, int max_step, uint32_t obs_mask, int &steps,
                                                              unsigned long long &alive_mask)
 {
@@ -135,6 +140,8 @@
     const pk2 k2 = {register_constant(4.166664568298827e-2f), register_constant(-1.6666654611e-1f)};
     asm volatile("" ::"v"(net.b2));
     bool alive = true;
+    if constexpr (LPE == 4 && FIXED_LENGTH && !MASKED && std::is_same_v<Tab, TanhBanked>)
+        asm volatile(".p2align 6\n\t.rept %0\n\ts_nop 0\n\t.endr" ::"n"(HEAVY_LOOP_PAD_NOPS));
     for (int t = 0; t < max_step; ++t) {
         if constexpr (!FIXED_LENGTH) {
             if (__ballot(alive) == 0ull) break;
diff --git a/simple-es_amd/csrc/ses_rollout.hip b/simple-es_amd/csrc/ses_rollout.hip
--- a/simple-es_amd/csrc/ses_rollout.hip
+++ b/simple-es_amd/csrc/ses_rollout.hip
@@ -1,3 +1,5 @@
+#include <atomic>
+
 #include "ses_cartpole.h"
 #include "ses_gru.h"
 #include "ses_gru_lockstep.h"
@@ -82,8 +84,8 @@
     }
 };
 
-template <int LPE, bool FIXED_LENGTH, bool PHYS64, bool MASKED, bool SMALL>
-__device__ __forceinline__ void rollout_cartpole_mlp_loop(const TanhEntry *tanh_tab, const MlpSlice<4, 2, LPE> &net,
+template <int LPE, bool FIXED_LENGTH, bool PHYS64, bool MASKED, bool SMALL, class Tab>
+__device__ __forceinline__ void rollout_cartpole_mlp_loop(Tab tanh_tab, const MlpSlice<4, 2, LPE> &net,
                                                           CartPoleSim<PHYS64> &sim, int max_step, uint32_t obs_mask,
                                                           int &steps, unsigned long long &alive_mask)
 {
@@ -115,8 +117,8 @@
     }
 }
 
-template <int LPE, bool FIXED_LENGTH, bool PHYS64>
-__device__ __forceinline__ void rollout_cartpole_mlp_run(const TanhEntry *tanh_tab, const MlpSlice<4, 2, LPE> &net,
+template <int LPE, bool FIXED_LENGTH, bool PHYS64, class Tab>
+__device__ __forceinline__ void rollout_cartpole_mlp_run(Tab tanh_tab, const MlpSlice<4, 2, LPE> &net,
                                                          CartPoleSim<PHYS64> &sim, int n_steps, uint32_t obs_mask, bool small,
                                                          int &steps, unsigned long long &alive_mask)
 {
@@ -128,8 +130,8 @@
         rollout_cartpole_mlp_loop<LPE, FIXED_LENGTH, PHYS64, true, false>(tanh_tab, net, sim, n_steps, obs_mask, steps, alive_mask);
 }
 
-template <int LPE, bool FIXED_LENGTH, bool PHYS64 = false, bool PK = false>
-__device__ __forceinline__ void rollout_cartpole_mlp_body(const TanhEntry *tanh_tab, long long lane_index, int env0,
+template <int LPE, bool FIXED_LENGTH, bool PHYS64 = false, bool PK = false, class Tab>
+__device__ __forceinline__ void rollout_cartpole_mlp_body(Tab tanh_tab, long long lane_index, int env0,
                                                           const float *__restrict__ theta,
                                                           const float *__restrict__ init, int init_per_offspring,
                                                           int n_env, int E, int P, int max_step, uint32_t obs_mask,
@@ -217,9 +219,9 @@
     float x, xd, th, thd;
     int steps, alive;
 };
-template <bool FIXED_LENGTH, bool OWN_ROWS, bool HEAVY_PK>
+template <bool FIXED_LENGTH, bool OWN_ROWS, bool HEAVY_PK, class Tab>
 __device__ __forceinline__ void rollout_cartpole_mlp_pairs(
-    const TanhEntry *tanh_tab, HandoverSlot (*slots)[64 / 4], int *small_of, const float *__restrict__ theta,
+    Tab tanh_tab, HandoverSlot (*slots)[64 / 4], int *small_of, const float *__restrict__ theta,
     const float *__restrict__ init, int init_per_offspring, int n_rows, int E, int P, int max_step, uint32_t obs_mask,
     int waves_light, int waves_heavy, int handover, int prio_steps, double *__restrict__ ep_return,
     int32_t *__restrict__ ep_steps, const float *rows_l = nullptr, int row0_l = 0, const float *rows_h = nullptr, int row0_h = 0)
@@ -325,42 +327,70 @@
     }
 }
 
-template <bool FIXED_LENGTH, bool HEAVY_PK = false>
+template <bool FIXED_LENGTH, bool HEAVY_PK = false, bool TANH_BANKED = false>
 __global__ __launch_bounds__(64 * 2 * HANDOVER_PAIRS) void k_rollout_cartpole_mlp_handover(
     const float *__restrict__ theta, const float *__restrict__ init, int init_per_offspring, int n_rows, int E, int P,
     int max_step, uint32_t obs_mask, int waves_light, int waves_heavy, int handover, int prio_steps,
     double *__restrict__ ep_return, int32_t *__restrict__ ep_steps)
 {
-    __shared__ TanhEntry tanh_tab[SES_TANH_N];
-    __shared__ HandoverSlot slots[HANDOVER_PAIRS][64 / 4];
-    __shared__ int small_of[HANDOVER_PAIRS];
-    stage_tanh_table(tanh_tab);
-    rollout_cartpole_mlp_pairs<FIXED_LENGTH, false, HEAVY_PK>(tanh_tab, slots, small_of, theta, init, init_per_offspring, n_rows, E, P,
-                                                              max_step, obs_mask, waves_light, waves_heavy, handover, prio_steps,
-                                                              ep_return, ep_steps);
-}
-
-template <bool FIXED_LENGTH, bool HEAVY_PK = false>
+    if constexpr (TANH_BANKED) {
+        __shared__ HandoverSlot slots[HANDOVER_PAIRS][64 / 4];
+        __shared__ int small_of[HANDOVER_PAIRS];
+        extern __shared__ TanhEntry tanh_image_lds[];
+        stage_tanh_table_banked(tanh_image_lds);
+        rollout_cartpole_mlp_pairs<FIXED_LENGTH, false, HEAVY_PK>(tanh_banked_view(tanh_image_lds), slots, small_of, theta, init,
+                                                                  init_per_offspring, n_rows, E, P, max_step, obs_mask, waves_light,
+                                                                  waves_heavy, handover, prio_steps, ep_return, ep_steps);
+    } else {
+        __shared__ TanhEntry tanh_tab[SES_TANH_N];
+        __shared__ HandoverSlot slots[HANDOVER_PAIRS][64 / 4];
+        __shared__ int small_of[HANDOVER_PAIRS];
+        stage_tanh_table(tanh_tab);
+        rollout_cartpole_mlp_pairs<FIXED_LENGTH, false, HEAVY_PK>(tanh_tab, slots, small_of, theta, init, init_per_offspring, n_rows, E, P,
+                                                                  max_step, obs_mask, waves_light, waves_heavy, handover, prio_steps,
+                                                                  ep_return, ep_steps);
+    }
+}
+
+template <bool FIXED_LENGTH, bool HEAVY_PK = false, bool TANH_BANKED = false>
 __global__ __launch_bounds__(64 * 2 * HANDOVER_PAIRS) void k_rollout_cartpole_mlp_handover_perturb(
     const float *__restrict__ init, int init_per_offspring, int n_rows, int E, int P, int max_step, uint32_t obs_mask,
     int waves_light, int waves_heavy, int handover, int prio_steps, double *__restrict__ ep_return,
     int32_t *__restrict__ ep_steps, PerturbUpdate u)
 {
-    __shared__ TanhEntry tanh_tab[SES_TANH_N];
-    __shared__ HandoverSlot slots[HANDOVER_PAIRS][64 / 4];
-    __shared__ int small_of[HANDOVER_PAIRS];
-    extern __shared__ float own_rows_lds[];
-    constexpr int ENVS_L = HANDOVER_PAIRS * (64 / 16), ENVS_H = HANDOVER_PAIRS * (64 / 4);
-    const int n_env = n_rows * E;
-    const int n_light = n_env < waves_light * (64 / 16) ? n_env : waves_light * (64 / 16);
-    const int l0 = (int)blockIdx.x * ENVS_L, h0 = waves_light * (64 / 16) + (int)blockIdx.x * ENVS_H;
-    const RowSpan span_l = rows_of_envs(l0, l0 + ENVS_L < n_light ? l0 + ENVS_L : n_light, E);
-    const RowSpan span_h = rows_of_envs(h0, h0 + ENVS_H < n_env ? h0 + ENVS_H : n_env, E);
-    float *const mu_new = own_rows_lds, *const rows = own_rows_lds + u.P4;
-    perturb_prologue(u, span_l, span_h, mu_new, rows, tanh_tab);
-    rollout_cartpole_mlp_pairs<FIXED_LENGTH, true, HEAVY_PK>(tanh_tab, slots, small_of, nullptr, init, init_per_offspring, n_rows, E, P,
-                                                             max_step, obs_mask, waves_light, waves_heavy, handover, prio_steps, ep_return,
-                                                             ep_steps, rows, span_l.row0, rows + (size_t)span_l.rows * P, span_h.row0);
+    if constexpr (TANH_BANKED) {
+        __shared__ HandoverSlot slots[HANDOVER_PAIRS][64 / 4];
+        __shared__ int small_of[HANDOVER_PAIRS];
+        extern __shared__ TanhEntry tanh_image_lds[];
+        constexpr int ENVS_L = HANDOVER_PAIRS * (64 / 16), ENVS_H = HANDOVER_PAIRS * (64 / 4);
+        const int n_env = n_rows * E;
+        const int n_light = n_env < waves_light * (64 / 16) ? n_env : waves_light * (64 / 16);
+        const int l0 = (int)blockIdx.x * ENVS_L, h0 = waves_light * (64 / 16) + (int)blockIdx.x * ENVS_H;
+        const RowSpan span_l = rows_of_envs(l0, l0 + ENVS_L < n_light ? l0 + ENVS_L : n_light, E);
+        const RowSpan span_h = rows_of_envs(h0, h0 + ENVS_H < n_env ? h0 + ENVS_H : n_env, E);
+        float *const mu_new = reinterpret_cast<float *>(tanh_image_lds + TANH_IMAGE_ENTRIES), *const rows = mu_new + u.P4;
+        perturb_prologue_banked(u, span_l, span_h, mu_new, rows, tanh_image_lds);
+        rollout_cartpole_mlp_pairs<FIXED_LENGTH, true, HEAVY_PK>(tanh_banked_view(tanh_image_lds), slots, small_of, nullptr, init,
+                                                                 init_per_offspring, n_rows, E, P, max_step, obs_mask, waves_light,
+                                                                 waves_heavy, handover, prio_steps, ep_return, ep_steps, rows,
+                                                                 span_l.row0, rows + (size_t)span_l.rows * P, span_h.row0);
+    } else {
+        __shared__ TanhEntry tanh_tab[SES_TANH_N];
+        __shared__ HandoverSlot slots[HANDOVER_PAIRS][64 / 4];
+        __shared__ int small_of[HANDOVER_PAIRS];
+        extern __shared__ float own_rows_lds[];
+        constexpr int ENVS_L = HANDOVER_PAIRS * (64 / 16), ENVS_H = HANDOVER_PAIRS * (64 / 4);
+        const int n_env = n_rows * E;
+        const int n_light = n_env < waves_light * (64 / 16) ? n_env : waves_light * (64 / 16);
+        const int l0 = (int)blockIdx.x * ENVS_L, h0 = waves_light * (64 / 16) + (int)blockIdx.x * ENVS_H;
+        const RowSpan span_l = rows_of_envs(l0, l0 + ENVS_L < n_light ? l0 + ENVS_L : n_light, E);
+        const RowSpan span_h = rows_of_envs(h0, h0 + ENVS_H < n_env ? h0 + ENVS_H : n_env, E);
+        float *const mu_new = own_rows_lds, *const rows = own_rows_lds + u.P4;
+        perturb_prologue(u, span_l, span_h, mu_new, rows, tanh_tab);
+        rollout_cartpole_mlp_pairs<FIXED_LENGTH, true, HEAVY_PK>(tanh_tab, slots, small_of, nullptr, init, init_per_offspring, n_rows, E, P,
+                                                                 max_step, obs_mask, waves_light, waves_heavy, handover, prio_steps, ep_return,
+                                                                 ep_steps, rows, span_l.row0, rows + (size_t)span_l.rows * P, span_h.row0);
+    }
 }
 inline int pair_own_rows(int E) { return max_rows_of_envs(HANDOVER_PAIRS * (64 / 16), E) + max_rows_of_envs(HANDOVER_PAIRS * (64 / 4), E); }
 
@@ -1080,6 +1110,8 @@
 
 static void launch_cartpole_mlp_pairs_perturb(ses_handle *h, const RolloutArgs &a, const PairShape &ps);
 static void launch_cartpole_mlp_pairs_packed(ses_handle *h, const RolloutArgs &a, const PairShape &ps);
+template <int FORM, class Launch>
+static bool launch_tanh_banked(ses_handle *h, size_t lds, const Launch &launch);
 
 static void launch_cartpole_mlp(ses_handle *h, const RolloutArgs &a, int mode)
 {
@@ -1419,19 +1451,55 @@
 {
     h->perturb_pending = 0;
     h->count_perturb_rollouts += 1;
-    const auto launch = [&](auto kernel) {
-        hipLaunchKernelGGL(kernel, dim3(ceil_div(ps.waves_light, HANDOVER_PAIRS)), dim3(64 * 2 * HANDOVER_PAIRS),
-                           perturb_rollout_lds(a.P, a.E), h->stream, a.init, a.per, a.n_rows, a.E, a.P, a.max_step, a.obs_mask,
-                           ps.waves_light, ps.waves_rest, ps.handover, h->tune_rollout_heavy_prio_steps, a.epr, a.ep_steps, h->pending);
+    const auto launch = [&](auto kernel, size_t lds) {
+        hipLaunchKernelGGL(kernel, dim3(ceil_div(ps.waves_light, HANDOVER_PAIRS)), dim3(64 * 2 * HANDOVER_PAIRS), lds, h->stream, a.init,
+                           a.per, a.n_rows, a.E, a.P, a.max_step, a.obs_mask, ps.waves_light, ps.waves_rest, ps.handover,
+                           h->tune_rollout_heavy_prio_steps, a.epr, a.ep_steps, h->pending);
     };
-    if (!cartpole_mlp_heavy_packed(h)) launch(k_rollout_cartpole_mlp_handover_perturb<true>);
-    else launch(k_rollout_cartpole_mlp_handover_perturb<true, true>);
+    if (!cartpole_mlp_heavy_packed(h)) launch(k_rollout_cartpole_mlp_handover_perturb<true>, perturb_rollout_lds(a.P, a.E));
+    else if (!launch_tanh_banked<1>(h, perturb_rollout_lds(a.P, a.E), launch))
+        launch(k_rollout_cartpole_mlp_handover_perturb<true, true>, perturb_rollout_lds(a.P, a.E));
 }
 
 static void launch_cartpole_mlp_pairs_packed(ses_handle *h, const RolloutArgs &a, const PairShape &ps)
 {
-    launch_rollout_kernel(h, k_rollout_cartpole_mlp_handover<true, true>, dim3(ceil_div(ps.waves_light, HANDOVER_PAIRS)),
-                          dim3(64 * 2 * HANDOVER_PAIRS), a, ps.waves_light, ps.waves_rest, ps.handover, h->tune_rollout_heavy_prio_steps);
+    const auto launch = [&](auto kernel, size_t lds) {
+        hipLaunchKernelGGL(kernel, dim3(ceil_div(ps.waves_light, HANDOVER_PAIRS)), dim3(64 * 2 * HANDOVER_PAIRS), lds, h->stream, a.theta,
+                           a.init, a.per, a.n_rows, a.E, a.P, a.max_step, a.obs_mask, ps.waves_light, ps.waves_rest, ps.handover,
+                           h->tune_rollout_heavy_prio_steps, a.epr, a.ep_steps);
+    };
+    if (!launch_tanh_banked<0>(h, 0, launch)) launch(k_rollout_cartpole_mlp_handover<true, true>, 0);
+}
+
+template <int FORM, class Launch>
+static bool launch_tanh_banked(ses_handle *h, size_t lds, const Launch &launch)
+{
+    constexpr int form = FORM;
+    constexpr int MAX_DEVICES = 64;
+    static std::atomic<int> allowed[2][MAX_DEVICES];
+    const int d = h->cfg.device;
+    if (h->tune_rollout_tanh_banked == 0 || d < 0 || d >= MAX_DEVICES) return false;
+    const void *kernel = form ? reinterpret_cast<const void *>(&k_rollout_cartpole_mlp_handover_perturb<true, true, true>)
+                              : reinterpret_cast<const void *>(&k_rollout_cartpole_mlp_handover<true, true, true>);
+    int st = allowed[form][d].load();
+    if (st == 0) {
+        hipFuncAttributes fa{};
+        st = -1;
+        if (hipFuncGetAttributes(&fa, kernel) == hipSuccess && fa.sharedSizeBytes + TANH_IMAGE_BYTES <= (size_t)h->lds_per_cu &&
+            hipFuncSetAttribute(kernel, hipFuncAttributeMaxDynamicSharedMemorySize, h->lds_per_cu - (int)fa.sharedSizeBytes) == hipSuccess)
+            st = 1 + (int)fa.sharedSizeBytes;
+        allowed[form][d].store(st);
+    }
+    if (st < 0 || (size_t)(st - 1) + lds + TANH_IMAGE_BYTES > (size_t)h->lds_per_cu) return false;
+    if (hipPeekAtLastError() != hipSuccess) return false;
+    if constexpr (form) launch(k_rollout_cartpole_mlp_handover_perturb<true, true, true>, TANH_IMAGE_BYTES + lds);
+    else launch(k_rollout_cartpole_mlp_handover<true, true, true>, TANH_IMAGE_BYTES + lds);
+    if (hipGetLastError() != hipSuccess) {
+        allowed[form][d].store(-1);
+        return false;
+    }
+    h->count_tanh_banked += 1;
+    return true;
 }
 
 }
diff --git a/simple-es_amd/csrc/ses_tanh_banked.h b/simple-es_amd/csrc/ses_tanh_banked.h
--- /dev/null
+++ b/simple-es_amd/csrc/ses_tanh_banked.h
@@ -0,0 +1,47 @@
+#pragma once
+#include <stddef.h>
+
+#include "ses_math.h"
+
+namespace ses {
+
+constexpr int TANH_BANK_COPIES = 16;
+constexpr int TANH_IMAGE_ENTRIES = SES_TANH_N * TANH_BANK_COPIES;
+constexpr size_t TANH_IMAGE_BYTES = (size_t)TANH_IMAGE_ENTRIES * 16;
+
+constexpr int tanh_bank_slot(int lane) { return lane & (TANH_BANK_COPIES - 1); }
+constexpr int tanh_bank_index(int entry, int slot) { return entry * TANH_BANK_COPIES + slot; }
+
+constexpr int LDS_B128_GROUPS[4][16] = {{0, 1, 2, 3, 12, 13, 14, 15, 20, 21, 22, 23, 24, 25, 26, 27},
+                                        {4, 5, 6, 7, 8, 9, 10, 11, 16, 17, 18, 19, 28, 29, 30, 31},
+                                        {32, 33, 34, 35, 44, 45, 46, 47, 52, 53, 54, 55, 56, 57, 58, 59},
+                                        {36, 37, 38, 39, 40, 41, 42, 43, 48, 49, 50, 51, 60, 61, 62, 63}};
+constexpr int tanh_bank_max_sharing()
+{
+    int worst = 0;
+    for (int g = 0; g < 4; ++g) {
+        int seen[TANH_BANK_COPIES] = {};
+        for (int k = 0; k < 16; ++k) {
+            const int n = ++seen[tanh_bank_slot(LDS_B128_GROUPS[g][k])];
+            worst = n > worst ? n : worst;
+        }
+    }
+    return worst;
+}
+static_assert((TANH_BANK_COPIES & (TANH_BANK_COPIES - 1)) == 0 && TANH_BANK_COPIES <= 16, "the copy of a lane is lane & (copies - 1)");
+static_assert(tanh_bank_max_sharing() == 16 / TANH_BANK_COPIES, "the lanes of a service group spread evenly over the copies");
+
+struct TanhBanked {
+    const TanhEntry *image;
+    int slot;
+};
+#if defined(__HIPCC__)
+__device__ __forceinline__ TanhBanked tanh_banked_view(const TanhEntry *image)
+{
+    return TanhBanked{image, tanh_bank_slot((int)threadIdx.x)};
+}
+#endif
+SES_DEV TanhEntry tanh_entry(const TanhEntry *tab, int32_t i) { return tab[i]; }
+SES_DEV TanhEntry tanh_entry(const TanhBanked &tab, int32_t i) { return tab.image[(i * TANH_BANK_COPIES) + tab.slot]; }
+
+}
diff --git a/simple-es_amd/ses/_lib.py b/simple-es_amd/ses/_lib.py
--- a/simple-es_amd/ses/_lib.py
+++ b/simple-es_amd/ses/_lib.py
@@ -101,6 +101,7 @@
     "ses_sync": [_vp],
     "ses_set_tuning": [_vp, ctypes.c_char_p, _i32],
     "ses_launch_counts": [_vp, _vp, _vp, _vp],
+    "ses_tanh_banked_count": [_vp, _vp],
     "ses_set_stamp": [_vp, _vp],
     "ses_last_error": [],
     "ses_version": [],
diff --git a/simple-es_amd/ses/device.py b/simple-es_amd/ses/device.py
--- a/simple-es_amd/ses/device.py
+++ b/simple-es_amd/ses/device.py
@@ -110,6 +110,11 @@
         check(self._lib.ses_launch_counts(self._h, *[ctypes.byref(o) for o in out]), "ses_launch_counts")
         return tuple(int(o.value) for o in out)
 
+    def tanh_banked_count(self):
+        out = ctypes.c_int64(0)
+        check(self._lib.ses_tanh_banked_count(self._h, ctypes.byref(out)), "ses_tanh_banked_count")
+        return int(out.value)
+
     def set_stamp(self, dst):
         if dst is not None and not (isinstance(dst, torch.Tensor) and dst.dtype == torch.int64 and dst.numel() >= 1 and
                                     (dst.is_pinned() if dst.device.type == "cpu" else dst.device == self.device)):
```

Result: no change. 57.99 billion (median of 6 runs) (+0.7%).
